# bmds-lab/Crackling

Hardware: AMD Instinct MI355X
Metric: guides/sec (whole node) + achieved HBM GB/s, 20bp/<=4mm ISSL scan (higher is better)
Workload: dtype u32

## Files before the change

crackling_amd/csrc/issl_bin.hip:

```cpp
#include <hip/hip_runtime.h>

#include <algorithm>
#include <type_traits>

#include "issl_kernels.hpp"

namespace issl {


__global__ __launch_bounds__(256) void k_pack_scan_stream(ImageView v, uint32_t *__restrict__ scan_out,
                                                          uint64_t *__restrict__ esig_out,
                                                          uint8_t *__restrict__ occ8_out,
                                                          uint32_t *__restrict__ error_flag, uint32_t *__restrict__ seen,
                                                          uint32_t tile_begin, uint32_t tile_end)
{
    for (uint32_t t = tile_begin + blockIdx.x; t < tile_end; t += gridDim.x) {
        uint32_t lo = 0, hi = v.n_buckets;
        while (hi - lo > 1) {
            const uint32_t mid = (lo + hi) >> 1;
            if (v.tile_first[mid] <= t) lo = mid; else hi = mid;
        }
        const uint32_t b = lo;
        const uint32_t slice = b >> v.slice_width;
        const uint64_t start = v.bucket_start[b];
// ... 71 lines not shown
    if (g < n) {
        const uint64_t sig = guides[g];
        const uint32_t low = (1u << slice_width) - 1u;
        for (uint32_t s = 0; s < n_slices; ++s) {
            const uint32_t key = static_cast<uint32_t>(sig >> (slice_width * s)) & low;
            atomicAdd(&hist[(s << slice_width) + key], 1u);
        }
    }
    const uint32_t stride = gridDim.x * 256;
    for (uint32_t k = g; k < n_slots; k += stride) { ws.gidx[k] = kNoGuide; ws.gword[k] = kPadGuideWord; }
    for (uint32_t k = g; k <= n; k += stride) ws.gcount[k] = 0;
    for (uint32_t k = g; k <= ws.cap_chunks; k += stride) ws.raw_used[k] = 0;
    if (g == 0) {
        Counters c{};
        c.raw_chunks = n_scan_waves;
        *ws.counters = c;
        ws.scan_span[2u * ws.span_slot] = ~0ull;
        ws.scan_span[2u * ws.span_slot + 1u] = 0ull;
    }
    __syncthreads();
    if (blockIdx.x * 256 < n)
        for (uint32_t b = threadIdx.x; b < n_buckets; b += 256)
            if (hist[b]) atomicAdd(&ws.ng[b], hist[b]);
}

template <bool COOP = false>
__device__ __forceinline__ RangeStart range_start_of(const ScanItem *__restrict__ items, uint32_t n_items, uint64_t total,
                                                     uint32_t n_ranges, uint32_t r)
{
    RangeStart out;
    out.item = n_items;
    out.tile = 0;
    out.goff = 0;
    out.pad = 0;
    if (r < n_ranges) {
        const uint64_t lo = total / n_ranges * r + (total % n_ranges) * r / n_ranges;
        uint32_t a = 0, z = n_items;
        if (COOP) {
            const uint32_t lane = threadIdx.x & 63u;
            while (z - a > 1) {
                const uint32_t step = (z - a + 63u) / 64u;
                const uint64_t pos = static_cast<uint64_t>(a) + static_cast<uint64_t>(lane + 1u) * step;
                const bool le = pos < z && items[pos].cost0 <= lo;
                const uint32_t k = static_cast<uint32_t>(__popcll(__ballot(le)));
                const uint64_t na = static_cast<uint64_t>(a) + static_cast<uint64_t>(k) * step, nz = na + step;
                a = static_cast<uint32_t>(na);
                if (nz < z) z = static_cast<uint32_t>(nz);
            }
        } else
        while (z - a > 1) {
            const uint32_t mid = (a + z) >> 1;
            if (items[mid].cost0 <= lo) a = mid; else z = mid;
        }
        const ScanItem it = items[a];
        const uint32_t len = it.g1 - it.g0;
        const uint32_t per_guide = it.shape >> 3;
        const uint64_t tile_cost = static_cast<uint64_t>(len) * per_guide + kTileFixedCost;
        const uint64_t rel = lo - it.cost0;
        uint64_t k = rel / tile_cost;
        const uint64_t rem = rel % tile_cost;
        uint32_t goff = 0;
        if (rem > kTileFixedCost) {
            goff = ((static_cast<uint32_t>(rem - kTileFixedCost) + per_guide - 1u) / per_guide + kGuideGroup - 1u) & ~(kGuideGroup - 1u);
            if (goff >= len) { goff = 0; ++k; }
        }
        if (k >= it.n_tiles) { out.item = a + 1; out.tile = 0; out.goff = 0; }
        else { out.item = a; out.tile = static_cast<uint32_t>(k); out.goff = goff; }
    }
    return out;
}

__device__ __forceinline__ uint32_t ranges_for(uint64_t units, uint32_t scan_blocks)
{
    const uint64_t want = units / 64u + 1u;
    const uint32_t floor_ = scan_blocks < 64u ? scan_blocks : 64u;
    return want >= scan_blocks ? scan_blocks : want < floor_ ? floor_ : static_cast<uint32_t>(want);
}

__global__ __launch_bounds__(256) void k_plan(ImageView v, uint32_t *__restrict__ ng, uint32_t *__restrict__ gfill,
                                              uint32_t *__restrict__ gstart, ScanItem *__restrict__ items,
                                              uint32_t cap_items, PlanInfo *__restrict__ plan, uint32_t item_guides,
                                              uint32_t scan_blocks, Counters *__restrict__ counters)
{
    short_kernel_priority();
    __shared__ uint64_t lds[256];
    const uint32_t nb = v.n_buckets;
    const uint32_t per = (nb + 255u) / 256u;
    const uint32_t b0 = threadIdx.x * per;
    const uint32_t b1 = (b0 + per < nb) ? b0 + per : nb;

    uint64_t slots = 0, n_it = 0, cost = 0, cand = 0, wtiles = 0;
    for (uint32_t b = b0; b < b1; ++b) {
        const uint32_t g = ng[b];
        const uint32_t nt = v.tile_first[b + 1] - v.tile_first[b];
        slots += (g + kGuideGroup - 1u) / kGuideGroup * kGuideGroup;
        if (g && nt) {
            const uint32_t k = (g + item_guides - 1u) / item_guides;
            n_it += k;
            cost += static_cast<uint64_t>(nt) * (static_cast<uint64_t>(g) * kGuideCost + static_cast<uint64_t>(k) * kTileFixedCost);
            cand += (v.bucket_start[b + 1] - v.bucket_start[b]) * g;
            wtiles += static_cast<uint64_t>(nt) * k;
        }
    }
    uint64_t tot_slots, tot_items, tot_cost, tot_cand, tot_tiles;
    uint64_t slot_at = block_exclusive_scan(slots, lds, &tot_slots);
    uint64_t item_at = block_exclusive_scan(n_it, lds, &tot_items);
    uint64_t cost_at = block_exclusive_scan(cost, lds, &tot_cost);
    (void)block_exclusive_scan(cand, lds, &tot_cand);
    uint64_t tile_at = block_exclusive_scan(wtiles, lds, &tot_tiles);

    const bool overflow = tot_items > cap_items;
    for (uint32_t b = b0; b < b1; ++b) {
        const uint32_t g = ng[b];
        const uint32_t nt = v.tile_first[b + 1] - v.tile_first[b];
        gstart[b] = static_cast<uint32_t>(slot_at);
        if (g && nt && !overflow) {
            const uint64_t blen = v.bucket_start[b + 1] - v.bucket_start[b];
            for (uint32_t done = 0; done < g; done += item_guides) {
                const uint32_t len = (g - done < item_guides) ? g - done : item_guides;
                ScanItem it;
                it.bucket = b;
                it.g0 = static_cast<uint32_t>(slot_at) + done;
                it.g1 = it.g0 + len;
                it.n_tiles = nt;
                it.cost0 = cost_at;
                it.tile0 = static_cast<uint32_t>(tile_at);
                it.last_cands = static_cast<uint32_t>(blen - static_cast<uint64_t>(nt - 1u) * kTileCands);
                it.group_abs = v.tile_first[b] * 64u;
                it.window = it.last_cands << 16;
                it.shape = 32; it.gmid = 0;
                items[item_at++] = it;
                cost_at += static_cast<uint64_t>(nt) * (len * kGuideCost + kTileFixedCost);
                tile_at += nt;
            }
        }
        slot_at += (g + kGuideGroup - 1u) / kGuideGroup * kGuideGroup;
        ng[b] = 0;
        gfill[b] = 0;
    }
    if (threadIdx.x == 255) {
        gstart[nb] = static_cast<uint32_t>(tot_slots);
        if (!overflow) {
            ScanItem end;
            end.bucket = 0; end.g0 = 0; end.g1 = 0; end.n_tiles = 0; end.cost0 = tot_cost;
            end.tile0 = static_cast<uint32_t>(tot_tiles); end.last_cands = 0; end.group_abs = 0; end.window = 0;
            end.shape = 32; end.gmid = 0;
            items[tot_items] = end;
        }
        plan->n_items = overflow ? 0u : static_cast<uint32_t>(tot_items);
        plan->total_cost = overflow ? 0ull : tot_cost;
        plan->candidates = tot_cand;
        plan->reference_candidates = tot_cand;
        plan->fine = 0;
        plan->tiles = tot_tiles;
        plan->n_ranges = (overflow || tot_tiles == 0) ? 0u : ranges_for(tot_tiles, scan_blocks);
        counters->raw_chunks = (plan->n_ranges ? plan->n_ranges : 1u) * 16u;
        plan->error = overflow ? 2u : 0u;
    }
}

__global__ __launch_bounds__(256) void k_guide_scatter(const uint64_t *__restrict__ guides, uint32_t n,
                                                       uint32_t slice_width, uint32_t n_slices, uint32_t sorted_layout,
                                                       uint32_t n_buckets, const uint32_t *__restrict__ gstart,
                                                       uint32_t *__restrict__ gfill, uint32_t *__restrict__ gword,
                                                       uint32_t *__restrict__ gidx, uint32_t *__restrict__ gbucket,
                                                       uint64_t *__restrict__ gsig,
                                                       uint32_t guide_blocks, const PlanInfo *__restrict__ plan,
                                                       const ScanItem *__restrict__ items,
                                                       RangeStart *__restrict__ starts)
{
    short_kernel_priority();
    if (blockIdx.x >= guide_blocks) {
        const uint32_t n_ranges = plan->n_ranges;
        const uint32_t r = (blockIdx.x - guide_blocks) * 256 + threadIdx.x;
        if (r <= n_ranges && n_ranges != 0) starts[r] = range_start_of(items, plan->n_items, plan->total_cost, n_ranges, r);
        return;
    }
    __shared__ uint32_t hist[kMaxBuckets];
    __shared__ uint32_t base[kMaxBuckets];
    for (uint32_t b = threadIdx.x; b < n_buckets; b += 256) hist[b] = 0;
    __syncthreads();
    const uint32_t g = blockIdx.x * 256 + threadIdx.x;
    const uint32_t low = (1u << slice_width) - 1u;
    uint64_t sig = 0;
    uint32_t rank[kMaxSlices];
    if (g < n) {
        sig = guides[g];
#pragma unroll
        for (uint32_t s = 0; s < kMaxSlices; ++s) {
            if (s < n_slices) {
                const uint32_t key = static_cast<uint32_t>(sig >> (slice_width * s)) & low;
                rank[s] = atomicAdd(&hist[(s << slice_width) + key], 1u);
            }
        }
    }
    __syncthreads();
    for (uint32_t b = threadIdx.x; b < n_buckets; b += 256)
        base[b] = hist[b] ? atomicAdd(&gfill[b], hist[b]) : 0u;
    __syncthreads();
    if (g < n) {
#pragma unroll
        for (uint32_t s = 0; s < kMaxSlices; ++s) {
            if (s < n_slices) {
                const uint32_t key = static_cast<uint32_t>(sig >> (slice_width * s)) & low;
                const uint32_t b = (s << slice_width) + key;
                const uint32_t slot = gstart[b] + base[b] + rank[s];
                gword[slot] = image_word(sig, s, slice_width, sorted_layout != 0u);
                gidx[slot] = g;
                gbucket[slot] = b;
                gsig[slot] = sig;
            }
        }
    }
}


struct GroupUnits {
    uint32_t s0a, n_full, rest, shape, units;
};
__device__ __forceinline__ GroupUnits group_units(uint32_t s0, uint32_t s1, uint32_t tail_shapes)
{
    GroupUnits u;
    u.s0a = s0 & ~31u;
    const uint32_t span = s1 - u.s0a;
    u.n_full = span / kTileCands;
    u.rest = span - u.n_full * kTileCands;
    u.shape = (!tail_shapes || u.rest > 1024u) ? 32u : u.rest > 512u ? 16u : 8u;
    u.units = u.n_full + (u.rest ? 1u : 0u);
    return u;
}
__device__ __forceinline__ uint64_t group_cost(const GroupUnits &u, uint32_t len)
{
    return static_cast<uint64_t>(u.n_full) * (static_cast<uint64_t>(len) * kGuideCost + kTileFixedCost) +
           (u.rest ? static_cast<uint64_t>(len) * (u.shape >> 3) + kTileFixedCost : 0ull);
}

__device__ __forceinline__ uint32_t fine_way(uint32_t gj, uint32_t way)
{
    if (way == 0) return gj;
    if (way < kFineWays) {
        const uint32_t q = (way - 1u) / 3u, d = (way - 1u) % 3u + 1u;
        return gj ^ (d << (2u * q));
    }
    const uint32_t w2 = way - kFineWays, pair = w2 / 9u, d1 = (w2 % 9u) / 3u + 1u, d2 = w2 % 3u + 1u;
    const uint32_t a = pair < 3u ? 0u : pair < 5u ? 1u : 2u;
    const uint32_t b = pair < 3u ? pair + 1u : pair < 5u ? pair - 1u : 3u;
    return gj ^ (d1 << (2u * a)) ^ (d2 << (2u * b));
}
__device__ __forceinline__ uint32_t fine_class(uint32_t way) { return way == 0u ? 0u : way < kFineWays ? 1u : 2u; }

__host__ __device__ __forceinline__ uint32_t fine_word(uint32_t word, uint32_t slice, uint32_t slice_width = 8u)
{
    const uint32_t lo = word & 0xFFFFu, hi = word >> 16;
    uint32_t lo12 = 0, hi12 = 0;
    for (uint32_t j = 0; j < 3u; ++j) {
        const uint32_t q = fine_order(slice, j, slice_width);
        lo12 |= ((lo >> (4u * q)) & 0xFu) << (4u * j);
        hi12 |= ((hi >> (4u * q)) & 0xFu) << (4u * j);
    }
    return lo12 | (hi12 << 12);
}

template <uint32_t WAYS>
__global__ __launch_bounds__(256) void k_fine_count(ImageView v, const uint64_t *__restrict__ gsig,
                                                    const uint32_t *__restrict__ gstart, const uint32_t *__restrict__ gfill,
                                                    uint32_t *__restrict__ fcount,
                                                    uint32_t *__restrict__ fcount0,
                                                    FineSum *__restrict__ fsum, uint32_t item_guides, uint32_t tail_shapes)
{
    constexpr uint32_t ways = WAYS;
    short_kernel_priority();
    __shared__ uint32_t cnt[256], cnt0[256];
    __shared__ uint64_t lds[256];
    const uint32_t b = blockIdx.x, slice = b >> v.slice_width;
    cnt[threadIdx.x] = 0;
    cnt0[threadIdx.x] = 0;
    __syncthreads();
    const uint32_t g0 = gstart[b], n = gfill[b];
    for (uint32_t i = threadIdx.x; i < n; i += 256) {
        const uint32_t gj = succ_byte(gsig[g0 + i], slice, v.slice_width);
        atomicAdd(&cnt0[gj], 1u);
#pragma unroll
        for (uint32_t way = 0; way < ways; ++way) atomicAdd(&cnt[fine_way(gj, way)], 1u);
    }
    __syncthreads();
    const uint32_t w = threadIdx.x, c = cnt[w];
    const uint32_t *ss = v.sub_start + static_cast<uint64_t>(b) * 257u;
    const uint32_t s0 = ss[w], s1 = ss[w + 1];
    fcount[static_cast<uint64_t>(b) * 256u + w] = (s1 > s0) ? c : 0u;
    fcount0[static_cast<uint64_t>(b) * 256u + w] = (s1 > s0) ? cnt0[w] : 0u;
    uint64_t cost = 0, cand = 0, slots = 0, items = 0, units = 0;
    if (c && s1 > s0) {
        const GroupUnits gu = group_units(s0, s1, tail_shapes);
        const uint32_t kk = (c + item_guides - 1u) / item_guides;
        slots = (c + kGuideGroup - 1u) / kGuideGroup * kGuideGroup;
        units = static_cast<uint64_t>(gu.units) * kk;
        items = units;
        for (uint32_t done = 0; done < c; done += item_guides) cost += group_cost(gu, c - done < item_guides ? c - done : item_guides);
        cand = static_cast<uint64_t>(s1 - s0) * c;
    }
    uint64_t t_cost, t_cand, t_slots, t_items, t_units, t_places;
    (void)block_exclusive_scan(cost, lds, &t_cost);
    (void)block_exclusive_scan(cand, lds, &t_cand);
    (void)block_exclusive_scan(slots, lds, &t_slots);
    (void)block_exclusive_scan(items, lds, &t_items);
    (void)block_exclusive_scan(units, lds, &t_units);
    (void)block_exclusive_scan((c && s1 > s0) ? c : 0u, lds, &t_places);
    if (threadIdx.x == 0) {
        FineSum f;
        f.cost = t_cost; f.cand = t_cand; f.slots = static_cast<uint32_t>(t_slots); f.items = static_cast<uint32_t>(t_items);
        f.units = static_cast<uint32_t>(t_units); f.places = static_cast<uint32_t>(t_places);
        fsum[b] = f;
    }
}

__global__ __launch_bounds__(256) void k_fine_plan(FineSum *__restrict__ fsum, uint32_t nb, ScanItem *__restrict__ fitems,
                                                   uint32_t cap_items, uint32_t cap_slots, PlanInfo *__restrict__ plan,
                                                   uint32_t scan_blocks, uint32_t prune_mode, uint32_t always,
                                                   uint32_t *__restrict__ sticky, Counters *__restrict__ counters)
{
    short_kernel_priority();
    __shared__ uint64_t lds[256];
    const uint32_t per = (nb + 255u) / 256u;
    const uint32_t b0 = threadIdx.x * per, b1 = (b0 + per < nb) ? b0 + per : nb;
    uint64_t cost = 0, cand = 0, slots = 0, items = 0, units = 0, places = 0;
    for (uint32_t b = b0; b < b1; ++b) {
        cost += fsum[b].cost; cand += fsum[b].cand; slots += fsum[b].slots; items += fsum[b].items; units += fsum[b].units;
        places += fsum[b].places;
    }
    uint64_t t_cost, t_cand, t_slots, t_items, t_units, t_places;
    (void)block_exclusive_scan(places, lds, &t_places);
    uint64_t cost_at = block_exclusive_scan(cost, lds, &t_cost);
    (void)block_exclusive_scan(cand, lds, &t_cand);
    uint64_t slot_at = block_exclusive_scan(slots, lds, &t_slots);
    uint64_t item_at = block_exclusive_scan(items, lds, &t_items);
    uint64_t unit_at = block_exclusive_scan(units, lds, &t_units);
    for (uint32_t b = b0; b < b1; ++b) {
        const FineSum f = fsum[b];
        FineSum at;
        at.cost = cost_at; at.cand = 0; at.slots = static_cast<uint32_t>(slot_at); at.items = static_cast<uint32_t>(item_at);
        at.units = static_cast<uint32_t>(unit_at); at.places = 0;
        fsum[b] = at;
        cost_at += f.cost; slot_at += f.slots; item_at += f.items; unit_at += f.units;
    }
    if (threadIdx.x == 255) {
        const uint64_t fetch_cost = static_cast<uint64_t>(kFetchPairs) * kGuideCost;
        const uint64_t full_fetch = plan->tiles, full_pairs = plan->total_cost - kTileFixedCost * full_fetch;
        const uint64_t fine_pairs = t_cost - kTileFixedCost * t_units;
        const uint64_t est_full = full_pairs > fetch_cost * full_fetch ? full_pairs : fetch_cost * full_fetch;
        const uint64_t est_fine = (fine_pairs > fetch_cost * t_units ? fine_pairs : fetch_cost * t_units) + t_places * kGuideCost;
        const bool fits = t_items <= cap_items && t_slots <= cap_slots;
        if (t_items > cap_items)
            atomicMax(&sticky[3], static_cast<uint32_t>(t_items < 0xFFFFFFFFull ? t_items : 0xFFFFFFFFull));
        if (fits && plan->error == 0 && (always || est_fine < est_full)) {
            ScanItem end;
            end.bucket = 0; end.g0 = 0; end.g1 = 0; end.n_tiles = 0; end.cost0 = t_cost;
            end.tile0 = static_cast<uint32_t>(t_units); end.last_cands = 0; end.group_abs = 0; end.window = 0;
            end.shape = 32; end.gmid = 0;
            fitems[t_items] = end;
            plan->n_items = static_cast<uint32_t>(t_items);
            plan->total_cost = t_cost;
            plan->candidates = t_cand;
            plan->tiles = t_units;
            plan->n_ranges = t_units == 0 ? 0u : ranges_for(t_units, scan_blocks);
            counters->raw_chunks = (plan->n_ranges ? plan->n_ranges : 1u) * 16u;
            plan->fine = prune_mode;
            plan->fine_slots = static_cast<uint32_t>(t_slots);
        }
    }
}


struct alignas(16) FineGroup {
    uint64_t cost0, chunk_cost;
    uint32_t s0, s1, n_full, units;
    uint32_t shape, c, slot, slot0;
};
template <uint32_t THREADS> struct FineItemLds {
    uint64_t scan[THREADS / 64u];
    uint32_t item0_of[257];
    FineGroup group[256];
    alignas(16) ScanItem stage[THREADS];
};
template <uint32_t THREADS> struct FineGuideLds {
    uint64_t scan[THREADS / 64u];
    uint32_t slot_of[256], slot0_of[256], cursor[256], cursor0[256], has_cands[256];
};
static_assert(sizeof(FineItemLds<512u>) <= 40u * 1024u, "four workgroups of k_fine_scatter per CU");

template <uint32_t THREADS>
__device__ __forceinline__ void fine_scatter_items(const ImageView &v, uint32_t b, const uint32_t *__restrict__ fcount,
                                                   const uint32_t *__restrict__ fcount0, const FineSum *__restrict__ fbase,
                                                   ScanItem *__restrict__ fitems, uint32_t item_guides, uint32_t tail_shapes,
                                                   FineItemLds<THREADS> &l)
{
    const uint32_t w = threadIdx.x;
    const FineSum base = fbase[b];
    const uint64_t blen = v.bucket_start[b + 1] - v.bucket_start[b];
    const uint32_t tile_first_b = v.tile_first[b];
    uint32_t c = 0, c1 = 0, s0 = 0, s1 = 0;
    if (w < 256u) {
        c = fcount[static_cast<uint64_t>(b) * 256u + w];
        c1 = c - fcount0[static_cast<uint64_t>(b) * 256u + w];
        const uint32_t *ss = v.sub_start + static_cast<uint64_t>(b) * 257u;
        s0 = ss[w];
        s1 = ss[w + 1];
    }
    uint64_t cost = 0, slots = 0, items = 0;
    GroupUnits gu{};
    if (c) {
        gu = group_units(s0, s1, tail_shapes);
        const uint32_t kk = (c + item_guides - 1u) / item_guides;
        slots = (c + kGuideGroup - 1u) / kGuideGroup * kGuideGroup;
        items = static_cast<uint64_t>(gu.units) * kk;
        for (uint32_t done = 0; done < c; done += item_guides) cost += group_cost(gu, c - done < item_guides ? c - done : item_guides);
    }
    const uint64_t cost_at = base.cost + block_exclusive_scan(cost, l.scan, nullptr);
    const uint32_t slot_at = base.slots + static_cast<uint32_t>(block_exclusive_scan(slots, l.scan, nullptr));
    const uint32_t item_at = static_cast<uint32_t>(block_exclusive_scan(items, l.scan, nullptr));
    if (w < 256u) {
        l.item0_of[w] = item_at;
        if (w == 255u) l.item0_of[256] = item_at + static_cast<uint32_t>(items);
        FineGroup g;
        g.cost0 = cost_at; g.chunk_cost = group_cost(gu, item_guides);
        g.s0 = s0; g.s1 = s1; g.n_full = gu.n_full; g.units = gu.units;
        g.shape = gu.shape; g.c = c; g.slot = slot_at; g.slot0 = slot_at + c1;
        l.group[w] = g;
    }
    __syncthreads();
    const uint32_t total = l.item0_of[256];
    for (uint32_t i0 = 0; i0 < total; i0 += THREADS) {
        const uint32_t i = i0 + w;
        if (i < total) {
            uint32_t lo = 0, hi = 256;
            while (hi - lo > 1u) {
                const uint32_t mid = (lo + hi) >> 1;
                if (l.item0_of[mid] <= i) lo = mid; else hi = mid;
            }
            const uint32_t gw = lo;
            const FineGroup g = l.group[gw];
            const uint32_t s0a = g.s0 & ~31u;
            const uint32_t j = i - l.item0_of[gw];
            const uint32_t chunk = j / g.units, t = j - chunk * g.units;
            const uint32_t done = chunk * item_guides;
            const uint32_t len = (g.c - done < item_guides) ? g.c - done : item_guides;
            const bool full = t < g.n_full;
            const uint32_t shape = full ? 32u : g.shape, cap = 64u * shape;
            const uint32_t wstart = s0a + t * kTileCands;
            const uint64_t after = blen - wstart;
            ScanItem it;
            it.bucket = (b << 8) | gw;
            it.g0 = g.slot + done;
            it.g1 = it.g0 + len;
            it.n_tiles = 1;
            it.cost0 = g.cost0 + static_cast<uint64_t>(chunk) * g.chunk_cost +
                       static_cast<uint64_t>(t) * (static_cast<uint64_t>(len) * kGuideCost + kTileFixedCost);
            it.tile0 = base.items + i;
            it.last_cands = after < cap ? static_cast<uint32_t>(after) : cap;
            it.group_abs = tile_first_b * 64u + (wstart >> 5);
            it.window = (t == 0 ? g.s0 - s0a : 0u) | ((g.s1 - wstart < cap ? g.s1 - wstart : cap) << 16);
            it.shape = shape; it.gmid = g.slot0;
            l.stage[w] = it;
        }
        __syncthreads();
        const uint32_t n_here = total - i0 < THREADS ? total - i0 : THREADS;
        const uint4 *src4 = reinterpret_cast<const uint4 *>(l.stage);
        uint4 *dst4 = reinterpret_cast<uint4 *>(fitems + base.items + i0);
        for (uint32_t q = w; q < n_here * 3u; q += THREADS) dst4[q] = src4[q];
        __syncthreads();
    }
}

template <uint32_t WAYS, uint32_t THREADS>
__device__ __forceinline__ void fine_scatter_guides(const ImageView &v, uint32_t b, const uint32_t *__restrict__ gstart,
                                                    const uint32_t *__restrict__ gfill, const uint32_t *__restrict__ gword,
                                                    const uint32_t *__restrict__ gidx, const uint64_t *__restrict__ gsig,
                                                    const uint32_t *__restrict__ fcount, const uint32_t *__restrict__ fcount0,
                                                    const FineSum *__restrict__ fbase, FineSlot *__restrict__ fword,
                                                    FineGuideLds<THREADS> &l)
{
    constexpr uint32_t ways = WAYS;
    const uint32_t w = threadIdx.x, slice = b >> v.slice_width;
    const uint32_t g0 = gstart[b], n = gfill[b];
    const uint32_t base_slots = fbase[b].slots;
    uint32_t c = 0, c1 = 0;
    if (w < 256u) {
        c = fcount[static_cast<uint64_t>(b) * 256u + w];
        c1 = c - fcount0[static_cast<uint64_t>(b) * 256u + w];
    }
    uint32_t i = w, guide = 0, word = 0;
    uint64_t sig = 0;
    if (i < n) { guide = gidx[g0 + i]; word = gword[g0 + i]; sig = gsig[g0 + i]; }
    const uint32_t slots = (c + kGuideGroup - 1u) / kGuideGroup * kGuideGroup;
    const uint32_t slot_at = base_slots + static_cast<uint32_t>(block_exclusive_scan(slots, l.scan, nullptr));
    if (w < 256u) {
        l.slot_of[w] = slot_at;
        l.slot0_of[w] = slot_at + c1;
        l.cursor[w] = 0;
        l.cursor0[w] = 0;
        l.has_cands[w] = c ? 1u : 0u;
        for (uint32_t k2 = c; k2 < slots; ++k2) fword[slot_at + k2] = FineSlot{kPadGuideWord, kPadSlotId};
    }
    __syncthreads();
    while (i < n) {
        const uint32_t gj = succ_byte(sig, slice, v.slice_width);
        const uint32_t word12 = fine_word(word, slice, v.slice_width), id = slot_id(slice, guide);
#pragma unroll
        for (uint32_t way = 0; way < ways; ++way) {
            const uint32_t ww = fine_way(gj, way);
            if (!l.has_cands[ww]) continue;
            const uint32_t slot = way ? l.slot_of[ww] + atomicAdd(&l.cursor[ww], 1u) : l.slot0_of[ww] + atomicAdd(&l.cursor0[ww], 1u);
            fword[slot] = FineSlot{word12 | (fine_class(way) << 24), id};
        }
        i += THREADS;
        if (i < n) { guide = gidx[g0 + i]; word = gword[g0 + i]; sig = gsig[g0 + i]; }
    }
}

template <uint32_t WAYS, uint32_t THREADS>
__global__ __launch_bounds__(THREADS) void k_fine_scatter(ImageView v, const uint32_t *__restrict__ gstart,
// ... 231 lines not shown
```

crackling_amd/csrc/issl_capi.cpp:

```cpp
#include <algorithm>
#include <cerrno>
#include <cstdio>
#include <cstdlib>
#include <cstring>

#include "issl_index.hpp"

using namespace issl;

namespace issl {

int build_from_device_sites(const uint64_t *d_sigs, const uint32_t *d_occ, size_t n_sites, size_t n_lines, size_t seq_len,
                            size_t slice_width, int device, const char *options, issl_index **out)
{
    int rc = select_device(device, "the ISSL scorer");
    if (rc) return rc;
    const uint32_t n_slices = static_cast<uint32_t>((seq_len * 2) / slice_width);
    std::vector<uint64_t> sizes(size_t(n_slices) << slice_width);
    rc = launch_bucket_sizes(d_sigs, n_sites, static_cast<uint32_t>(slice_width), n_slices, sizes.data());
    if (rc) return rc;
    std::unique_ptr<HostIndex> h(new HostIndex());
    rc = h->init_from_bucket_sizes(sizes.data(), n_sites, n_lines, seq_len, slice_width);
    if (rc) return rc;
    return build_on_device(std::move(h), d_sigs, d_occ, true, device, options, out);
// ... 1 lines not shown

}

extern "C" {

const char *issl_last_error(void) { return get_error(); }
int issl_abi_version(void) { return ISSL_ABI_VERSION; }

int issl_index_open(const char *path, issl_index **out)
{
    if (!path || !out) return issl::fail(ISSL_E_ARG, "null argument");
    return abi_call([&] { return new_index([&](HostIndex &h) { return h.open_file(path); }, out); });
}

int issl_index_from_memory(const void *image, size_t len, issl_index **out)
{
    if (!image || !out) return issl::fail(ISSL_E_ARG, "null argument");
    return abi_call([&] { return new_index([&](HostIndex &h) { return h.from_memory(image, len); }, out); });
}

int issl_index_build_from_text(const char *text, size_t n_lines, size_t seq_len, size_t slice_width,
                               issl_index **out)
{
    if (!text || !out) return issl::fail(ISSL_E_ARG, "null argument");
    return abi_call([&] { return new_index([&](HostIndex &h) { return h.build_from_text(text, n_lines, seq_len, slice_width); }, out); });
}

int issl_index_build_from_sites(const uint64_t *sigs, const uint32_t *occ, size_t n_sites, size_t n_lines,
                                size_t seq_len, size_t slice_width, issl_index **out)
{
    if (!sigs || !occ || !out) return issl::fail(ISSL_E_ARG, "null argument");
    return abi_call([&] { return new_index([&](HostIndex &h) { return h.build_from_sites(sigs, occ, n_sites, n_lines, seq_len, slice_width); }, out); });
}

int issl_index_write(const issl_index *idx, const char *path)
{
    if (!idx || !path) return issl::fail(ISSL_E_ARG, "null argument");
    return abi_call([&]() -> int {
        if (!idx->host) { set_error("index was attached from a device image and has no host arrays"); return ISSL_E_STATE; }
        if (idx->host->has_arrays()) return idx->host->write_file(path);
        if (!idx->d_image) { set_error("index has neither host arrays nor a device image"); return ISSL_E_STATE; }
        HIP_TRY(hipSetDevice(idx->device));
        FILE *fp = std::fopen(path, "wb");
        if (!fp) {
            set_error(std::string("cannot write index file '") + path + "': " + std::strerror(errno));
            return ISSL_E_IO;
        }
        bool ok = idx->host->write_leading_sections(fp) == ISSL_OK;
        const uint8_t *base = static_cast<const uint8_t *>(idx->d_image);
        const uint8_t *cold = static_cast<const uint8_t *>(idx->h_cold);
        std::vector<uint8_t> stage;
        bool sig_words = false;
        auto stream_dev = [&](const uint8_t *src, uint64_t bytes) {
            stage.resize(size_t(64) << 20);
            for (uint64_t at = 0; ok && at < bytes; at += stage.size()) {
                const size_t len = static_cast<size_t>(std::min<uint64_t>(stage.size(), bytes - at));
                ok = hipMemcpy(stage.data(), src + at, len, hipMemcpyDeviceToHost) == hipSuccess;
                if (ok && sig_words) {
                    uint64_t *w = reinterpret_cast<uint64_t *>(stage.data());
                    for (size_t i = 0; i < len / 8; ++i) w[i] &= kSigMask;
                }
                ok = ok && std::fwrite(stage.data(), 1, len, fp) == len;
            }
        };
        auto stream_out = [&](uint64_t off, uint64_t bytes, bool in_host) {
            if (in_host) {
                ok = ok && std::fwrite(cold + off, 1, bytes, fp) == bytes;
                return;
            }
            stream_dev(base + off, bytes);
        };
        sig_words = idx->hdr.off_sub_start != 0;
        stream_out(idx->hdr.off_sites, 8 * idx->geo.n_sites, (idx->hdr.cold_on_host & 2u) != 0);
        sig_words = false;
        ok = ok && std::fwrite(idx->host->sizes, 8, idx->geo.n_buckets(), fp) == idx->geo.n_buckets();
        if (idx->hdr.lists_absent) {
            std::unique_ptr<void, hipError_t (*)(void *)> list_mem(nullptr, hipFree);
            const uint64_t n = idx->geo.n_sites;
            void *p = nullptr;
            if (hipMalloc(&p, std::max<uint64_t>(8 * n, 8)) != hipSuccess) {
                (void)hipGetLastError();
                std::fclose(fp);
                set_error("no device memory to rebuild the slice lists of this image (8 B per site)");
                return ISSL_E_DEVICE;
            }
            list_mem.reset(p);
            for (uint64_t sl = 0; ok && sl < idx->geo.n_slices; ++sl) {
                int brc = launch_build_entries(reinterpret_cast<const uint64_t *>(base + idx->hdr.off_sites),
                                               reinterpret_cast<const uint32_t *>(base + idx->hdr.off_site_occ), n, static_cast<uint32_t>(sl),
                                               static_cast<uint32_t>(sl + 1), static_cast<uint32_t>(idx->geo.slice_width),
                                               static_cast<uint64_t *>(list_mem.get()));
                if (brc) { std::fclose(fp); return brc; }
                stream_dev(static_cast<const uint8_t *>(list_mem.get()), 8 * n);
            }
        } else {
            stream_out(idx->hdr.off_entries, 8 * idx->geo.n_sites * idx->geo.n_slices, (idx->hdr.cold_on_host & 1u) != 0);
        }
        ok = (std::fclose(fp) == 0) && ok;
        if (!ok) {
            set_error(std::string("could not write '") + path + "' from the device image");
            return ISSL_E_IO;
        }
        return ISSL_OK;
    });
}

int issl_index_header(const issl_index *idx, issl_header *out)
{
    if (!idx || !out) return issl::fail(ISSL_E_ARG, "null argument");
    out->n_sites = idx->geo.n_sites;
    out->seq_len = idx->geo.seq_len;
    out->n_lines = idx->geo.n_lines;
    out->slice_width = idx->geo.slice_width;
    out->n_slices = idx->geo.n_slices;
    out->n_scores = idx->geo.n_scores;
    return ISSL_OK;
}

int issl_index_bucket_sizes(const issl_index *idx, uint64_t *out, size_t n)
{
    if (!idx || !out) return issl::fail(ISSL_E_ARG, "null argument");
    if (n < idx->bucket_sizes.size()) { set_error("bucket size buffer too small"); return ISSL_E_ARG; }
    std::copy(idx->bucket_sizes.begin(), idx->bucket_sizes.end(), out);
    return ISSL_OK;
}

int issl_index_close(issl_index *idx)
{
    if (!idx) return ISSL_OK;
    release_device(idx);
    delete idx;
    return ISSL_OK;
}

int issl_index_device_bytes(const issl_index *idx, size_t *out)
{
    if (!idx || !out) return issl::fail(ISSL_E_ARG, "null argument");
    if (idx->d_image) { *out = idx->hdr.total_bytes; return ISSL_OK; }
    if (!idx->host) { set_error("index has neither host arrays nor a device image"); return ISSL_E_STATE; }
    return abi_call([&] { return planned_image_bytes(idx, out); });
}

static bool workspace_option(const issl_index *idx, const char *key, long long *value)
{
    const Workspace &w = idx->lane.ws;
    const bool used = w.cap_guides != 0;
    const struct { const char *key; long long v; } keys[] = {
        {"ws_cap_guides", static_cast<long long>(w.cap_guides)},
        {"ws_slot_width", used ? static_cast<long long>(w.slot_width) : 0},
        {"ws_fine_ways", static_cast<long long>(w.fine_ways)},
        {"ws_cap_chunks", static_cast<long long>(w.cap_chunks)},
        {"ws_cap_fitems", static_cast<long long>(w.cap_fitems)},
        {"ws_lean", idx->lane.lean ? 1 : 0},
    };
    for (const auto &k : keys)
        if (std::strcmp(k.key, key) == 0) {
            if (value) *value = k.v;
            return true;
        }
    return false;
}

int issl_index_set_option(issl_index *idx, const char *key, const char *value)
{
    if (!idx || !key || !value) return issl::fail(ISSL_E_ARG, "null argument");
    if (workspace_option(idx, key, nullptr)) {
        return abi_call([&]() -> int {
            set_error(std::string("read-only option: ") + key);
            return ISSL_E_ARG;
        });
    }
    if (idx->n_pending) { set_error("issl_index_set_option: batches are in flight, call issl_score_finish first"); return ISSL_E_STATE; }
    return abi_call([&]() -> int {
        Tuning t = idx->tuning;
        if (!t.set(key, value)) {
            set_error(std::string("unknown option or value out of range: ") + key + "=" + value);
            return ISSL_E_ARG;
        }
        if (idx->d_image && t.scan_blocks != idx->tuning.scan_blocks) {
            HIP_TRY(hipSetDevice(idx->device));
            for (Lane *lp : {&idx->lane, &idx->lane2})
                if (lp->ws.cap_chunks && lp->ws.cap_chunks < size_t(scan_waves(t)) * 2) {
                    int rc = ensure_raw_capacity(lp->ws, size_t(scan_waves(t)) * 4);
                    if (rc) return rc;
                }
        }
        idx->tuning = t;
        return ISSL_OK;
    });
}

int issl_index_get_option(const issl_index *idx, const char *key, long long *value)
{
    if (!idx || !key || !value) return issl::fail(ISSL_E_ARG, "null argument");
    if (idx->tuning.get(key, value) || image_option(idx->d_image ? &idx->hdr : nullptr, key, value) || workspace_option(idx, key, value)) return ISSL_OK;
    return abi_call([&]() -> int {
        set_error(std::string("unknown option: ") + key);
        return ISSL_E_ARG;
    });
}

int issl_index_build_on_device_opt(const uint64_t *sigs, const uint32_t *occ, size_t n_sites, size_t n_lines,
                                   size_t seq_len, size_t slice_width, int device, const char *options, issl_index **out)
{
    if (!sigs || !occ || !out) return issl::fail(ISSL_E_ARG, "null argument");
    return abi_call([&]() -> int {
        std::unique_ptr<HostIndex> h(new HostIndex());
        int rc = h->init_without_arrays(sigs, n_sites, n_lines, seq_len, slice_width);
        if (rc) return rc;
        return build_on_device(std::move(h), sigs, occ, false, device, options, out);
    });
}


int issl_index_build_from_device_sites(const uint64_t *d_sigs, const uint32_t *d_occ, size_t n_sites, size_t n_lines,
                                       size_t seq_len, size_t slice_width, int device, const char *options, issl_index **out)
{
    if (!d_sigs || !d_occ || !out) return issl::fail(ISSL_E_ARG, "null argument");
    if (seq_len == 0 || seq_len > 32 || slice_width < 2 || slice_width > 8 || (seq_len * 2) / slice_width == 0 ||
        (seq_len * 2) / slice_width > kMaxSlices) {
        set_error("bad sequence length or slice width");
        return ISSL_E_ARG;
    }
    return abi_call([&] { return build_from_device_sites(d_sigs, d_occ, n_sites, n_lines, seq_len, slice_width, device, options, out); });
}

int issl_index_build_on_device(const uint64_t *sigs, const uint32_t *occ, size_t n_sites, size_t n_lines,
                               size_t seq_len, size_t slice_width, int device, issl_index **out)
{
    return issl_index_build_on_device_opt(sigs, occ, n_sites, n_lines, seq_len, slice_width, device, nullptr, out);
}

int issl_device_memory(int device, size_t *free_bytes, size_t *total_bytes)
{
    if (!free_bytes || !total_bytes) return issl::fail(ISSL_E_ARG, "null argument");
    int rc = select_device(device, "the ISSL scorer");
    if (rc) return rc;
    HIP_TRY(hipMemGetInfo(free_bytes, total_bytes));
    return ISSL_OK;
}

int issl_index_upload(issl_index *idx, int device)
{
    if (!idx) return issl::fail(ISSL_E_ARG, "null argument");
    return abi_call([&] { return upload_common(idx, device, nullptr, 0); });
}

int issl_index_upload_into(issl_index *idx, int device, void *dev_buf, size_t bytes)
{
    if (!dev_buf) { set_error("null device buffer"); return ISSL_E_ARG; }
    if (!idx) return issl::fail(ISSL_E_ARG, "null argument");
    return abi_call([&] { return upload_common(idx, device, dev_buf, bytes); });
}


int issl_index_attach_image(int device, void *dev_buf, size_t bytes, issl_index **out)
{
    return abi_call([&] { return attach_common(device, dev_buf, bytes, nullptr, 0, out); });
}

int issl_index_attach_image_cold(int device, void *dev_buf, size_t bytes, void *cold_host, size_t cold_bytes,
                                 issl_index **out)
{
    return abi_call([&] { return attach_common(device, dev_buf, bytes, cold_host, cold_bytes, out); });
}

int issl_index_cold(const issl_index *idx, void **host_ptr, size_t *bytes)
{
    if (!idx || !host_ptr || !bytes) return issl::fail(ISSL_E_ARG, "null argument");
    if (!idx->d_image) { set_error("index has no device image"); return ISSL_E_STATE; }
    *host_ptr = idx->hdr.cold_on_host ? idx->h_cold : nullptr;
    *bytes = idx->hdr.cold_on_host ? idx->hdr.cold_bytes : 0;
    return ISSL_OK;
}

int issl_index_image(const issl_index *idx, void **dev_ptr, size_t *bytes)
{
    if (!idx || !dev_ptr || !bytes) return issl::fail(ISSL_E_ARG, "null argument");
    if (!idx->d_image) { set_error("index has no device image"); return ISSL_E_STATE; }
    *dev_ptr = idx->d_image;
    *bytes = idx->hdr.total_bytes;
    return ISSL_OK;
}

int issl_index_copy_image_to(const issl_index *idx, void *dev_dst, size_t bytes)
{
    if (!idx || !dev_dst) return issl::fail(ISSL_E_ARG, "null argument");
    if (!idx->d_image) { set_error("index has no device image"); return ISSL_E_STATE; }
    if (bytes < idx->hdr.total_bytes || (reinterpret_cast<uintptr_t>(dev_dst) & 255u)) {
        set_error("destination too small or not 256-byte aligned");
        return ISSL_E_ARG;
    }
    HIP_TRY(hipSetDevice(idx->device));
    HIP_TRY(hipMemcpy(dev_dst, idx->d_image, idx->hdr.total_bytes, hipMemcpyDeviceToDevice));
    return ISSL_OK;
}


void issl_free(void *p) { std::free(p); }

int issl_score_device(issl_index *idx, const uint64_t *d_guides, size_t n, int max_dist, double threshold,
                      int method, double *d_mit, double *d_cfd, void *stream)
{
    if (!idx || (n && (!d_guides || !d_mit || !d_cfd))) return issl::fail(ISSL_E_ARG, "null argument");
    return abi_call([&]() -> int {
        return score_core(idx, d_guides, n, max_dist, threshold, method, d_mit, d_cfd, static_cast<hipStream_t>(stream), false);
// ... 109 lines not shown
```

crackling_amd/csrc/issl_device.hpp:

```cpp
#pragma once
#include <cstddef>
#include <cstdint>
#include <string>

#include "issl_host.hpp"

namespace issl {

constexpr uint64_t kImageMagic = 0x314C535349444D41ull;
constexpr uint32_t kImageVersion = 9;
constexpr uint32_t kTileCands = 2048;
constexpr uint32_t kHeaderBytes = 4096;

struct ImageHeader {
    uint64_t magic;
    uint32_t version;
    uint32_t kind;
    uint64_t n_sites, seq_len, n_lines, slice_width, n_slices, n_scores_file;
    uint64_t n_buckets;
    uint64_t n_scores_unique;
    uint64_t n_tiles;
    uint64_t tile_cands;
    uint64_t total_bytes;
    uint64_t off_bucket_start, off_tile_first, off_score_mask, off_score_val, off_sites, off_entries,
        off_scan;
    uint64_t off_mit_dense;
    uint64_t off_esig;
    uint64_t cold_on_host;
    uint64_t cold_bytes;
    uint64_t off_occ8;
    uint64_t off_sub_start;
    uint64_t off_srec;
    uint64_t off_sid;
    uint64_t off_site_occ;
    uint64_t lists_absent;
};
static_assert(sizeof(ImageHeader) <= kHeaderBytes, "header must fit its block");

constexpr uint32_t kOccSaturated = 0xFFFFFFu;
constexpr uint64_t kSigMask = (1ull << 40) - 1ull;

#if defined(__HIPCC__)
__host__ __device__
#endif
inline uint32_t succ_byte(uint64_t sig, uint32_t s, uint32_t slice_width)
{
    const uint32_t sh = (slice_width * (s + 1u)) % 40u;
    const uint64_t x = sig & kSigMask;
    return static_cast<uint32_t>(sh ? (x >> sh) | (x << (40u - sh)) : x) & 0xFFu;
}
struct alignas(16) StreamRec {
    uint64_t sig;
    uint32_t id;
    uint32_t pos;
};

struct ImageView {
    const uint64_t *bucket_start;
    const uint32_t *tile_first;
    const uint64_t *score_mask;
    const double *score_val;
    const double *mit_dense;
    const uint64_t *sites;
    const uint64_t *entries;
    const uint64_t *esig;
    const uint8_t *occ8;
    const uint32_t *sub_start;
    const StreamRec *srec;
    const uint32_t *sid;
    const uint32_t *site_occ;
    const uint32_t *scan;
    uint64_t n_sites;
    uint32_t n_buckets;
    uint32_t n_scores;
    uint32_t slice_width;
    uint32_t n_slices;
    uint32_t n_tiles;
};

struct LayoutSpec {
    bool inline_sigs = false;
    uint32_t cold = 0;
    uint32_t sorted = 0;
    bool no_lists = false;
};
void layout_image(ImageHeader &h, const Geometry &g, uint64_t n_scores_unique, uint64_t n_tiles, bool dense_mit,
                  const LayoutSpec &spec);
ImageView make_view(const ImageHeader &h, void *base, void *cold);

struct Tuning {
    uint32_t scan_blocks;
    uint32_t scan_threads;
    int upload_threads;
    size_t upload_chunk_kib, upload_ring_min_kib;
    uint32_t item_guides;
    bool scan_generic;
    int scan_events;
    bool stage_timing;
    bool upload_timing;
    size_t raw_chunks;
    int inline_sigs;
    int sorted_layout;
    int compact;
    int prune;
    int tail_shapes;
    int hit_slots;
    size_t fine_items;
    size_t expect_guides;
    int small_bin;
    int lean_tail;
    int lanes;
    int host_cold;
    int keep_lists;
    std::string stamps_path;
    static Tuning from_env();
    bool set(const char *key, const char *value);
    bool get(const char *key, long long *value) const;
    int set_list(const char *options);
};
bool image_option(const ImageHeader *h, const char *key, long long *value);

int launch_build_entries(const uint64_t *d_sites, const uint32_t *d_occ, uint64_t n_sites, uint32_t slice_begin,
                         uint32_t slice_end, uint32_t slice_width, uint64_t *d_entries);
int launch_bucket_sizes(const uint64_t *d_sites, uint64_t n_sites, uint32_t slice_width, uint32_t n_slices, uint64_t *h_sizes);

constexpr int kSortNeedsListOrder = -1000;
constexpr int kSortNoRoom = -1001;
struct SortTemp {
    uint64_t *keys = nullptr, *tmp = nullptr;
    uint32_t *hist = nullptr;
    bool keys_borrowed = false;
    int alloc(uint64_t n_sites, void *borrowed_keys = nullptr);
    void release();
    ~SortTemp() { release(); }
};
int launch_sort_slice(SortTemp &t, const uint64_t *d_sites, const uint64_t *d_list, const uint64_t *d_bucket_start,
                      const uint32_t *d_tile_first, uint64_t n_sites, uint32_t n_slices, uint32_t n_buckets, uint32_t slice_width, uint32_t slice, uint32_t *d_sub_start,
                      StreamRec *d_srec, uint32_t *d_sid, uint32_t *d_site_occ, uint32_t *d_flag);
int finish_sort(uint32_t *d_flag);
void launch_tag_sites(uint64_t *d_sites, const uint32_t *d_site_occ, uint64_t n_sites);

constexpr uint32_t kGuideGroup = 8;
constexpr uint32_t kItemGuides = 512;
constexpr uint32_t kGuideCost = 4;
constexpr uint32_t kTileFixedCost = 8 * kGuideCost;
constexpr uint32_t kNoGuide = 0xFFFFFFFFu;
constexpr uint32_t kPadGuideWord = 0xFFFFFFFFu;
constexpr uint32_t kScanGridBlocks = 256u * 4u;
constexpr uint32_t kScanMaxBlocks = 8192u;
constexpr uint32_t kScanWaves = kScanMaxBlocks * 16u;
constexpr uint32_t kMaxRanges = kScanMaxBlocks;
constexpr uint32_t kStampsScanWords = 4u * kScanWaves, kStampsPerReplay = 16u * 4096u;
constexpr uint32_t kStampsMid = kStampsScanWords, kStampsBig256 = kStampsMid + kStampsPerReplay, kStampsBig1024 = kStampsBig256 + kStampsPerReplay;
constexpr uint32_t kStampsWords = kStampsBig1024 + kStampsPerReplay;
constexpr uint32_t kSpanRing = 64;
constexpr uint32_t kChunkRecs = 128;
constexpr uint64_t kDeadKey = ~0ull;
constexpr uint32_t kKeySliceShift = 32, kKeyGuideShift = 37, kKeySliceMask = 31, kMaxSlices = 20;

struct ScanItem {
    uint32_t bucket;
    uint32_t g0, g1;
    uint32_t n_tiles;
    uint64_t cost0;
    uint32_t tile0;
    uint32_t last_cands;
    uint32_t group_abs;
    uint32_t window;
    uint32_t shape;
    uint32_t gmid;
};
static_assert(sizeof(ScanItem) == 48, "scan items are fetched with scalar loads");

struct RangeStart {
    uint32_t item;
    uint32_t tile;
    uint32_t goff;
    uint32_t pad;
};

struct PlanInfo {
    uint32_t n_items;
    uint32_t error;
    uint32_t n_ranges;
    uint32_t fine;
    uint64_t total_cost;
    uint64_t candidates;
    uint64_t reference_candidates;
    uint64_t tiles;
    uint32_t fine_slots;
    uint32_t pad;
};

struct Counters {
    uint32_t next_range;
    uint32_t n_big;
    uint32_t n_big2;
    uint32_t n_big3;
    uint32_t raw_chunks;
    uint32_t raw_overflow;
    uint32_t overflowed;
    uint32_t replay_next[3];
};

struct FineSum {
    uint64_t cost, cand;
    uint32_t slots, items, units;
    uint32_t places;
};

constexpr uint32_t kSlotHits = 512;
constexpr uint32_t kSlotHitsWide = 2048;
struct alignas(32) SlotRec {
    double mit, cfd;
    uint64_t key, pad;
};
#if defined(__HIPCC__)
__host__ __device__
#endif
inline uint64_t slot_pad(uint32_t occ, uint32_t dist) { return static_cast<uint64_t>(occ) | (static_cast<uint64_t>(dist) << 32); }
constexpr uint32_t kFineWays = 13;
constexpr uint32_t kFineWays2 = 67;
constexpr uint32_t kFetchPairs = 8;
constexpr uint32_t kPruneMaxGuides = 1u << 20;
constexpr uint32_t kPruneMaxGuides2 = 1u << 18;
inline uint32_t prune_max_guides(uint32_t prune_mode, uint32_t n_slices)
{
    const uint32_t m = prune_mode == 3 ? kPruneMaxGuides2 : kPruneMaxGuides;
    return n_slices > 10 ? m >> 2 : n_slices > 5 ? m >> 1 : m;
}

constexpr uint32_t kSlotIdBits = 27, kSlotGuideBits = 22;
constexpr uint32_t kPadSlotId = (1u << kSlotIdBits) - 1u;
#if defined(__HIPCC__)
__host__ __device__
#endif
inline uint32_t slot_id(uint32_t slice, uint32_t guide) { return (slice << kSlotGuideBits) | guide; }
#if defined(__HIPCC__)
__host__ __device__
#endif
inline void slot_id_unpack(uint32_t id, uint32_t &slice, uint32_t &guide)
{
    slice = id >> kSlotGuideBits;
    guide = id & ((1u << kSlotGuideBits) - 1u);
}
static_assert(kPruneMaxGuides <= (1u << kSlotGuideBits), "a pruned launch's guides fit the id's guide field");
static_assert(kMaxSlices <= (1u << (kSlotIdBits - kSlotGuideBits)), "an index's slices fit the id's slice field");
static_assert(((kMaxSlices - 1u) << kSlotGuideBits | (kPruneMaxGuides - 1u)) < kPadSlotId, "no slot's id is the padding id");
static_assert(kSlotIdBits + 26u + 11u == 64u, "raw record: slot id, tile, offset in tile");

struct alignas(8) FineSlot {
    uint32_t word;
    uint32_t id;
};

struct Workspace {
    uint32_t *ng = nullptr;
    uint32_t *gfill = nullptr;
    uint32_t *gstart = nullptr;
    uint32_t *gword = nullptr;
    uint32_t *gidx = nullptr;
    uint32_t *gbucket = nullptr;
    uint64_t *gsig = nullptr;
    ScanItem *items = nullptr;
    FineSlot *fword = nullptr;
    ScanItem *fitems = nullptr;
    uint32_t *fcount = nullptr;
    uint32_t *fcount0 = nullptr;
    FineSum *fsum = nullptr;
    size_t cap_fslots = 0, cap_fitems = 0;
    uint32_t fine_ways = 0;
    PlanInfo *plan = nullptr;
    RangeStart *range_start = nullptr;
    uint64_t *raw = nullptr;
    uint32_t *raw_used = nullptr;
    size_t cap_chunks = 0;
    Counters *counters = nullptr;
    unsigned long long *scan_span = nullptr;
    uint32_t span_slot = 0;
    uint64_t *scan_count = nullptr;
    unsigned long long *stamps = nullptr;
    uint32_t *sticky = nullptr;
    uint64_t *sorted = nullptr;
    uint32_t *gcount = nullptr;
    uint32_t *goff = nullptr;
    uint32_t *gcur_big = nullptr;
    uint32_t *gcur_big2 = nullptr;
    double *terms = nullptr;
    double *pay = nullptr;
    uint32_t *rank = nullptr;
    SlotRec *slots = nullptr;
    uint32_t slot_hits = 0;
    uint32_t slot_width = kSlotHits;
    uint32_t lean_tail = 0;
    size_t cap_slot_guides = 0;
    uint32_t *blocksum = nullptr;
    uint64_t *d_guides = nullptr;
    void *h_stage = nullptr;
    size_t h_stage_bytes = 0;
    double *d_mit = nullptr, *d_cfd = nullptr;
    uint32_t *d_kept = nullptr;
    issl_hit *d_hitrec = nullptr;
    size_t cap_hitrec = 0;
    size_t cap_guides = 0;
    size_t cap_hits = 0;
    size_t cap_items = 0;
    size_t cap_gslots = 0;
    uint32_t n_buckets = 0;
};

struct ScoreParams {
    int max_dist;
    int method;
    double maximum_sum;
};

void launch_pack_scan_stream(const ImageView &v, uint32_t *scan_out, uint64_t *esig_out, uint8_t *occ8_out,
                             uint32_t *error_flag, uint32_t *seen, void *stream);
void launch_pack_scan_range(const ImageView &v, uint32_t *scan_out, uint64_t *esig_out, uint8_t *occ8_out,
                            uint32_t *error_flag, uint32_t *seen, uint32_t tile_begin, uint32_t tile_end, void *stream);
inline uint32_t fine_ways_of(uint32_t prune_mode) { return prune_mode == 1 ? 1u : prune_mode == 3 ? kFineWays2 : kFineWays; }
uint32_t prune_mode_for(const ImageView &v, const Tuning &tn, uint32_t n_guides, int max_dist);
void launch_bin_guides(const ImageView &v, const Workspace &ws, const Tuning &tn, const uint64_t *d_guides, uint32_t n,
                       uint32_t prune_mode, void *stream);
void launch_scan(const ImageView &v, const Workspace &ws, const Tuning &tn, const uint64_t *d_guides, uint32_t n,
                 int max_dist, uint32_t prune_mode, void *stream);
void launch_verify(const ImageView &v, const Workspace &ws, const uint64_t *d_guides, uint32_t n, const ScoreParams &p, void *stream);
void launch_group_hits(const Workspace &ws, uint32_t n, void *stream);
void launch_replay(const ImageView &v, const Workspace &ws, const uint64_t *d_guides, uint32_t n,
                   const ScoreParams &p, double *d_mit, double *d_cfd, uint32_t *d_kept, issl_hit *d_hitrec,
                   void *stream);
void launch_profile(const ImageView &v, const Workspace &ws, const uint64_t *d_guides, uint32_t n, issl_profile *d_out,
                    void *stream);
void launch_report_offsets(const Workspace &ws, uint32_t n, uint64_t base, uint64_t *d_offsets, void *stream);
void launch_report_emit(const ImageView &v, const Workspace &ws, const uint64_t *d_guides, uint32_t n_records,
                        uint32_t guide_base, issl_offtarget *d_out, void *stream);

}
```

crackling_amd/csrc/issl_group.hip:

```cpp
#include <hip/hip_runtime.h>

#include "issl_kernels.hpp"

namespace issl {


__global__ __launch_bounds__(256) void k_prefix_block_sums(const uint32_t *__restrict__ in, uint32_t n,
                                                           uint32_t *__restrict__ sums, uint32_t slot_hits)
{
    short_kernel_priority();
    __shared__ uint64_t lds[256];
    const uint32_t base = blockIdx.x * kScanChunk + threadIdx.x * 8u;
    uint64_t s = 0;
    for (uint32_t i = 0; i < 8; ++i)
        if (base + i < n) s += grouped_hits(in[base + i], slot_hits);
    uint64_t total;
    (void)block_exclusive_scan(s, lds, &total);
    if (threadIdx.x == 0) sums[blockIdx.x] = static_cast<uint32_t>(total);
}

__global__ __launch_bounds__(256) void k_prefix_of_sums(uint32_t *__restrict__ sums, uint32_t n_blocks)
{
    short_kernel_priority();
    __shared__ uint64_t lds[256];
    uint64_t carry = 0;
    for (uint32_t base = 0; base < n_blocks; base += 256) {
        const uint32_t i = base + threadIdx.x;
        const uint64_t val = i < n_blocks ? sums[i] : 0;
        uint64_t total;
        const uint64_t ex = block_exclusive_scan(val, lds, &total);
        if (i < n_blocks) sums[i] = static_cast<uint32_t>(carry + ex);
        carry += total;
    }
}

__global__ __launch_bounds__(256) void k_prefix_apply(const uint32_t *__restrict__ in, uint32_t n,
                                                      const uint32_t *__restrict__ sums, uint32_t *__restrict__ out,
                                                      uint32_t *__restrict__ big, Counters *__restrict__ counters,
                                                      uint32_t slot_hits)
{
    short_kernel_priority();
    __shared__ uint64_t lds[256];
    const uint32_t base = blockIdx.x * kScanChunk + threadIdx.x * 8u;
    uint32_t val[8];
    uint64_t s = 0;
    uint32_t nb = 0;
    for (uint32_t i = 0; i < 8; ++i) {
        const uint32_t c = (base + i < n) ? in[base + i] : 0u;
        nb += c > kReplayLds;
        val[i] = grouped_hits(c, slot_hits);
        s += val[i];
    }
    if (nb != 0u) {
        uint32_t at = atomicAdd(&counters->n_big, nb);
        for (uint32_t i = 0; i < 8; ++i)
            if (base + i < n && in[base + i] > kReplayLds) big[at++] = base + i;
    }
    uint64_t run = block_exclusive_scan(s, lds, nullptr) + sums[blockIdx.x];
    for (uint32_t i = 0; i < 8; ++i) {
        if (base + i < n) out[base + i] = static_cast<uint32_t>(run);
        run += val[i];
    }
}

__global__ __launch_bounds__(1024) void k_prefix_single(const uint32_t *__restrict__ in, uint32_t n,
                                                        uint32_t *__restrict__ out, uint32_t *__restrict__ big,
                                                        Counters *__restrict__ counters, uint32_t slot_hits)
{
    short_kernel_priority();
    if (slot_hits >= kReplayLds && counters->overflowed == 0u) return;
    __shared__ uint32_t wave_sum[16], wave_big[16];
    const uint32_t lane = threadIdx.x & 63u, wave = threadIdx.x >> 6;
    const uint32_t per = ((n + 1023u) / 1024u + 3u) & ~3u;
    const uint32_t i0 = threadIdx.x * per;
    uint32_t s = 0, b = 0;
    for (uint32_t k = 0; k < per; k += 4) {
        const uint32_t i = i0 + k;
        uint4 q = make_uint4(0, 0, 0, 0);
        if (i + 3 < n) q = *reinterpret_cast<const uint4 *>(in + i);
        else { if (i < n) q.x = in[i]; if (i + 1 < n) q.y = in[i + 1]; if (i + 2 < n) q.z = in[i + 2]; }
        s += grouped_hits(q.x, slot_hits) + grouped_hits(q.y, slot_hits) + grouped_hits(q.z, slot_hits) + grouped_hits(q.w, slot_hits);
        b += (q.x > kReplayLds) + (q.y > kReplayLds) + (q.z > kReplayLds) + (q.w > kReplayLds);
    }
    uint32_t x = s, xb = b;
    for (uint32_t d = 1; d < 64; d <<= 1) {
        const uint32_t y = __shfl_up(x, d, 64), yb = __shfl_up(xb, d, 64);
        if (lane >= d) { x += y; xb += yb; }
    }
    if (lane == 63) { wave_sum[wave] = x; wave_big[wave] = xb; }
    __syncthreads();
    uint32_t run = x - s, brun = xb - b;
    for (uint32_t wv = 0; wv < wave; ++wv) { run += wave_sum[wv]; brun += wave_big[wv]; }
    if (threadIdx.x == 1023u) counters->n_big = brun + b;
    for (uint32_t k = 0; k < per; k += 4) {
        const uint32_t i = i0 + k;
        if (i >= n) break;
        uint4 q = make_uint4(0, 0, 0, 0);
        if (i + 3 < n) q = *reinterpret_cast<const uint4 *>(in + i);
        else { q.x = in[i]; if (i + 1 < n) q.y = in[i + 1]; if (i + 2 < n) q.z = in[i + 2]; }
        const uint32_t ex = grouped_hits(q.x, slot_hits), ey = grouped_hits(q.y, slot_hits), ez = grouped_hits(q.z, slot_hits),
                       ew = grouped_hits(q.w, slot_hits);
        const uint4 o = make_uint4(run, run + ex, run + ex + ey, run + ex + ey + ez);
        if (i + 3 < n) *reinterpret_cast<uint4 *>(out + i) = o;
        else { out[i] = o.x; if (i + 1 < n) out[i + 1] = o.y; if (i + 2 < n) out[i + 2] = o.z; }
        run += ex + ey + ez + ew;
        if (q.x > kReplayLds) big[brun++] = i;
        if (q.y > kReplayLds) big[brun++] = i + 1;
        if (q.z > kReplayLds) big[brun++] = i + 2;
        if (q.w > kReplayLds) big[brun++] = i + 3;
    }
}

__global__ __launch_bounds__(kChunkRecs) void k_group_scatter(const uint64_t *__restrict__ raw,
                                                              const uint32_t *__restrict__ raw_used,
                                                              const Counters *__restrict__ counters, uint32_t cap_chunks,
                                                              const uint32_t *__restrict__ gcount,
                                                              const uint32_t *__restrict__ goff,
                                                              const uint32_t *__restrict__ rank,
                                                              const double2 *__restrict__ pay,
                                                              uint64_t *__restrict__ sorted, double2 *__restrict__ terms,
                                                              uint32_t slot_hits)
{
    short_kernel_priority();
    if (slot_hits >= kReplayLds && counters->n_big == 0u) return;
    uint32_t n_chunks = counters->raw_chunks;
    if (n_chunks > cap_chunks) n_chunks = cap_chunks;
    for (uint32_t chunk = blockIdx.x; chunk < n_chunks; chunk += gridDim.x) {
        const uint64_t *recs = raw + static_cast<uint64_t>(chunk) * kChunkRecs;
        const uint32_t t = threadIdx.x + 1u;
        const uint64_t slot = static_cast<uint64_t>(chunk) * (kChunkRecs - 1u) + (threadIdx.x < kChunkRecs - 1u ? threadIdx.x : kChunkRecs - 2u);
        const uint64_t key = recs[t < kChunkRecs ? t : 0u];
        const uint32_t my_rank = rank[slot];
        const double2 my_pay = pay[slot];
        const uint32_t used = raw_used[chunk];
        if (t >= used || t >= kChunkRecs || key == kDeadKey) continue;
        const uint32_t guide = static_cast<uint32_t>(key >> kKeyGuideShift);
        const uint32_t to = goff[guide] + my_rank;
        sorted[to] = key;
        if (gcount[guide] <= kMidHits) terms[to] = my_pay;
    }
}

void launch_group_hits(const Workspace &ws, uint32_t n, void *stream_)
{
    if (ws.lean_tail) return;
    hipStream_t stream = static_cast<hipStream_t>(stream_);
    const uint32_t m = n + 1;
    if (m <= (1u << 18)) {
        hipLaunchKernelGGL(k_prefix_single, dim3(1), dim3(1024), 0, stream, ws.gcount, m, ws.goff, ws.gcur_big,
                           ws.counters, ws.slot_hits);
    } else {
        const uint32_t blocks = (m + kScanChunk - 1) / kScanChunk;
        hipLaunchKernelGGL(k_prefix_block_sums, dim3(blocks), dim3(256), 0, stream, ws.gcount, m, ws.blocksum, ws.slot_hits);
        hipLaunchKernelGGL(k_prefix_of_sums, dim3(1), dim3(256), 0, stream, ws.blocksum, blocks);
        hipLaunchKernelGGL(k_prefix_apply, dim3(blocks), dim3(256), 0, stream, ws.gcount, m, ws.blocksum, ws.goff,
                           ws.gcur_big, ws.counters, ws.slot_hits);
    }
    hipLaunchKernelGGL(k_group_scatter, dim3(kTailGrid), dim3(kChunkRecs), 0, stream, ws.raw, ws.raw_used, ws.counters,
                       static_cast<uint32_t>(ws.cap_chunks), ws.gcount, ws.goff, ws.rank, reinterpret_cast<const double2 *>(ws.pay),
                       ws.sorted, reinterpret_cast<double2 *>(ws.terms), ws.slot_hits);
}

}
```

crackling_amd/csrc/issl_index.hpp:

```cpp
#pragma once
#include <hip/hip_runtime_api.h>

#include <functional>
#include <memory>
#include <string>
#include <vector>

#include "issl_device.hpp"
#include "issl_hiputil.hpp"

namespace issl {

constexpr uint32_t kRing = 64;
constexpr size_t kMaxBatch = size_t(1) << 24;
constexpr size_t kSlotBytesMax = size_t(8) << 30;

struct Lane {
    Workspace ws;
    hipEvent_t ev[6] = {};
    hipEvent_t done = nullptr;
    hipStream_t stream = nullptr;
    hipStream_t tail_stream = nullptr;
    bool ready = false;
    uint32_t last_n = 0;
    uint32_t pending = 0;
    bool staged = true;
    bool done_recorded = false;
    hipStream_t last_tail = nullptr;
    int last_max_dist = 0;
    uint32_t last_prune = 0;
    bool lean = false;
};

}

struct issl_index {
    uint64_t worst_per_guide = 0;
    std::unique_ptr<issl::HostIndex> host;
    issl::Geometry geo;
    std::vector<uint64_t> bucket_sizes;
    issl::Tuning tuning = issl::Tuning::from_env();
    int device = -1;
    void *d_image = nullptr;
    bool owns_image = false;
    void *h_cold = nullptr;
    void *d_cold = nullptr;
    bool owns_cold = false;
    issl::ImageHeader hdr{};
    issl::ImageView view{};
    issl::Lane lane;
    issl::Lane lane2;
    uint32_t n_async = 0;
    issl::Lane *last_lane = nullptr;
    hipEvent_t ring[2 * issl::kRing] = {};
    uint32_t n_ring = 0;
    bool have_events = false;
    issl_stats stats{};
    uint32_t n_pending = 0;
    hipEvent_t prev_scan_end = nullptr;
    hipEvent_t prev_batch_end = nullptr;
    bool list_order_only = false;
    size_t proven_guides = 0, proven_chunks = 0;
    int proven_dist = -1;
};

namespace issl {

int new_index_from_host(std::unique_ptr<HostIndex> h, issl_index **out);
template <class Init> int new_index(Init &&init, issl_index **out)
{
    std::unique_ptr<HostIndex> h(new HostIndex());
    if (int rc = init(*h)) return rc;
    return new_index_from_host(std::move(h), out);
}
int build_on_device(std::unique_ptr<HostIndex> h, const uint64_t *sigs, const uint32_t *occ, bool on_device, int device,
                    const char *options, issl_index **out);
int build_from_device_sites(const uint64_t *d_sigs, const uint32_t *d_occ, size_t n_sites, size_t n_lines, size_t seq_len,
                            size_t slice_width, int device, const char *options, issl_index **out);
int upload_common(issl_index *idx, int device, void *buf, size_t bytes);
int attach_common(int device, void *dev_buf, size_t bytes, void *cold_host, size_t cold_bytes, issl_index **out);
int planned_image_bytes(const issl_index *idx, size_t *out);
void release_device(issl_index *ix);

int supported_geometry(const Geometry &g);
void release_lanes(issl_index *ix);
inline uint32_t scan_waves(const Tuning &tn) { return tn.scan_blocks * 16u; }
int ensure_workspace(issl_index *ix, size_t n, Lane &lane, uint32_t fine_ways = kFineWays);
int ensure_raw_capacity(Workspace &w, size_t chunks);
int finish_batches(issl_index *ix, hipStream_t stream);
int score_core(issl_index *ix, const uint64_t *d_guides, size_t n, int max_dist, double threshold, int method,
               double *d_mit, double *d_cfd, hipStream_t stream, bool dump, issl_profile *d_profile = nullptr);
int score_async(issl_index *idx, const uint64_t *d_guides, size_t n, int max_dist, double threshold, int method,
                double *d_mit, double *d_cfd, hipStream_t stream);
int wait_batches(issl_index *idx, hipStream_t stream);
int score_host(issl_index *idx, const uint64_t *guides, size_t n, int max_dist, double threshold, int method,
               double *mit, double *cfd);
int dump_hits(issl_index *idx, const uint64_t *guides, size_t n, int max_dist, double threshold, int method,
              issl_hit *hits, size_t cap, size_t *n_hits);
int profile_host(issl_index *idx, const uint64_t *guides, size_t n, int max_dist, issl_profile *out);
int profile_device(issl_index *idx, const uint64_t *d_guides, size_t n, int max_dist, issl_profile *d_out, hipStream_t stream);
int offtargets_host(issl_index *idx, const uint64_t *guides, size_t n, int max_dist, uint64_t *offsets, issl_offtarget *recs,
                    size_t cap, size_t *n_total);
int offtargets_device(issl_index *idx, const uint64_t *d_guides, size_t n, int max_dist, uint64_t *d_offsets,
                      issl_offtarget *d_recs, size_t cap, size_t *n_total, hipStream_t stream);

struct CallBuffer : DevBuf {
    size_t bytes = 0;
    int reserve(size_t want)
    {
        if (want <= bytes) return ISSL_OK;
        release();
        bytes = 0;
        HIP_TRY(hipMalloc(&p, want));
        bytes = want;
        return ISSL_OK;
    }
};

struct RecordBatch {
    const uint64_t *d_guides = nullptr;
    size_t n_guides = 0, guide_base = 0;
    const issl_offtarget *d_recs = nullptr;
    uint32_t n_recs = 0;
    const uint32_t *d_rec_off = nullptr;
};
int records_device(issl_index *idx, const uint64_t *d_guides, size_t n, int max_dist, CallBuffer &buf, RecordBatch &out, hipStream_t stream);
int records_host(issl_index *idx, const uint64_t *guides, size_t n, int max_dist, CallBuffer &buf,
                 const std::function<int(const RecordBatch &)> &use);

}
```

crackling_amd/csrc/issl_kernels.hip:

```cpp
#include <hip/hip_runtime.h>

#include <type_traits>

#include "issl_kernels.hpp"

namespace issl {


struct alignas(4 * kGuideGroup) GuideGroup {
    uint32_t w[kGuideGroup];
};


__device__ __forceinline__ uint64_t raw_record(uint32_t gslot, uint32_t tile, uint32_t offset)
{
    return (static_cast<uint64_t>(gslot) << 37) | (static_cast<uint64_t>(tile) << 11) | offset;
}

struct RawWriter {
    uint64_t *chunk;
    uint32_t fill;
    uint32_t left;
    uint32_t reserve;
};

__device__ __forceinline__ void raw_retire(const RawWriter &w, uint32_t lane, const uint64_t *raw, uint32_t *raw_used)
{
    if (lane == 0) raw_used[(w.chunk - raw) / kChunkRecs] = w.fill;
}

__device__ __forceinline__ void raw_acquire(RawWriter &w, uint64_t *raw, uint32_t max_chunks, Counters *counters,
                                            uint32_t lane)
{
    w.fill = 1;
    if (w.left != 0u) {
        w.chunk += kChunkRecs;
        w.left -= 1u;
        return;
    }
    const uint32_t take = w.reserve;
    uint32_t idx = 0;
    if (lane == 0) idx = atomicAdd(&counters->raw_chunks, take);
    idx = __builtin_amdgcn_readfirstlane(idx);
    if (idx + take > max_chunks) {
        idx = max_chunks;
        if (lane == 0) counters->raw_overflow = 1u;
        w.chunk = raw + static_cast<uint64_t>(idx) * kChunkRecs;
        return;
    }
    w.chunk = raw + static_cast<uint64_t>(idx) * kChunkRecs;
    w.left = take - 1u;
    if (take < 16u) w.reserve = take * 2u;
}

__device__ __forceinline__ void full_add(uint32_t a, uint32_t b, uint32_t c, uint32_t &sum, uint32_t &carry)
{
    sum = __builtin_amdgcn_bitop3_b32(a, b, c, 0x96);
    carry = __builtin_amdgcn_bitop3_b32(a, b, c, 0xE8);
}
__device__ __forceinline__ void half_add(uint32_t a, uint32_t b, uint32_t &sum, uint32_t &carry)
{
    sum = a ^ b;
    carry = a & b;
}

template <int THR>
__device__ __forceinline__ uint32_t count_near(const uint32_t (&m)[16], uint32_t thr, uint32_t keep);

template <int THR>
__device__ __forceinline__ uint32_t near_plane(const uint32_t (&c)[kPlanes], uint32_t gw, uint32_t thr, uint32_t keep)
{
    uint32_t m[16];
#pragma unroll
    for (int p = 0; p < 16; ++p) {
        const uint32_t g0 = 0u - ((gw >> p) & 1u);
        const uint32_t g1 = 0u - ((gw >> (16 + p)) & 1u);
        m[p] = (c[p] ^ g0) | (c[16 + p] ^ g1);
    }
    return count_near<THR>(m, thr, keep);
}

template <int THR>
__device__ __forceinline__ uint32_t near_plane_masks(const uint32_t (&c)[kPlanes], const uint4 *gm ,
                                                     uint32_t thr, uint32_t keep)
{
    uint32_t m[16];
#pragma unroll
    for (int q = 0; q < 4; ++q) {
        const uint4 lo = gm[q], hi = gm[4 + q];
        asm volatile("" ::: "memory");
        m[4 * q + 0] = (c[4 * q + 0] ^ lo.x) | (c[16 + 4 * q + 0] ^ hi.x);
        m[4 * q + 1] = (c[4 * q + 1] ^ lo.y) | (c[16 + 4 * q + 1] ^ hi.y);
        m[4 * q + 2] = (c[4 * q + 2] ^ lo.z) | (c[16 + 4 * q + 2] ^ hi.z);
        m[4 * q + 3] = (c[4 * q + 3] ^ lo.w) | (c[16 + 4 * q + 3] ^ hi.w);
    }
    return count_near<THR>(m, thr, keep);
}

constexpr uint32_t kPassIds = 28;
typedef uint32_t SlotPair __attribute__((ext_vector_type(4)));
__device__ __forceinline__ void short_unit_masks(const FineSlot *__restrict__ slots, uint32_t g0, bool wide,
                                                 uint32_t lane, uint4 *lds_masks)
{
    const uint32_t i = lane >> 3, q = lane & 7u;
    uint32_t m[4];
    if (wide) {
        const SlotPair gw = *reinterpret_cast<const SlotPair *>(slots + g0 + 2u * i);
        const uint32_t a = gw.x >> (4u * q), b = gw.z >> (4u * q);
#pragma unroll
        for (uint32_t r = 0; r < 4; ++r)
            m[r] = ((0u - ((a >> r) & 1u)) & 0xFFFFu) | ((0u - ((b >> r) & 1u)) << 16);
        if (q == 7u) { m[0] = gw.y; m[1] = gw.w; }
    } else {
        const SlotPair *src = reinterpret_cast<const SlotPair *>(slots + g0 + 4u * i);
        const SlotPair ga = src[0], gb = src[1];
        const uint32_t t[4] = {ga.x >> (4u * q), ga.z >> (4u * q), gb.x >> (4u * q), gb.z >> (4u * q)};
#pragma unroll
        for (uint32_t r = 0; r < 4; ++r) {
            const uint32_t bits = ((t[0] >> r) & 1u) | (((t[1] >> r) & 1u) << 8) | (((t[2] >> r) & 1u) << 16) | (((t[3] >> r) & 1u) << 24);
            m[r] = bits * 255u;
        }
        if (q == 7u) { m[0] = ga.y; m[1] = ga.w; m[2] = gb.y; m[3] = gb.w; }
    }
    lds_masks[i * 8u + q] = make_uint4(m[0], m[1], m[2], m[3]);
}

template <int THR>
__device__ __forceinline__ uint32_t count_near(const uint32_t (&m)[16], uint32_t thr, uint32_t keep)
{
    uint32_t s0, s1, s2, s3, s4, t, u, n0, n1, n2;
    uint32_t k2[8], k4[4], k8a, k8b;
    full_add(m[0], m[1], m[2], s0, k2[0]);
    full_add(m[3], m[4], m[5], s1, k2[1]);
    full_add(m[6], m[7], m[8], s2, k2[2]);
    full_add(m[9], m[10], m[11], s3, k2[3]);
    full_add(m[12], m[13], m[14], s4, k2[4]);
    full_add(s0, s1, s2, t, k2[5]);
    full_add(s3, s4, m[15], u, k2[6]);
    half_add(t, u, n0, k2[7]);
    uint32_t a2, b2, c2;
    full_add(k2[0], k2[1], k2[2], a2, k4[0]);
    full_add(k2[3], k2[4], k2[5], b2, k4[1]);
    full_add(k2[6], k2[7], a2, c2, k4[2]);
    half_add(b2, c2, n1, k4[3]);
    if (THR >= 0 && THR <= 4) {
        const uint32_t o = __builtin_amdgcn_bitop3_b32(k4[0], k4[1], k4[2], 0xFE);
        if (THR == 0) return __builtin_amdgcn_bitop3_b32(o, __builtin_amdgcn_bitop3_b32(k4[3], n1, n0, 0xFE), keep, 0x02);
        if (THR == 1) return __builtin_amdgcn_bitop3_b32(o, k4[3], n1, 0x01) & keep;
        if (THR == 2) return __builtin_amdgcn_bitop3_b32(o, __builtin_amdgcn_bitop3_b32(k4[3], n1, n0, 0xF8), keep, 0x02);
        if (THR == 3) return __builtin_amdgcn_bitop3_b32(o, k4[3], keep, 0x02);
        const uint32_t p = __builtin_amdgcn_bitop3_b32(k4[0], k4[1], k4[2], 0xE8);
        const uint32_t z = __builtin_amdgcn_bitop3_b32(o, k4[3], n1 | n0, 0xE8);
        return __builtin_amdgcn_bitop3_b32(p, z, keep, 0x02);
    }
    uint32_t a4;
    full_add(k4[0], k4[1], k4[2], a4, k8a);
    half_add(a4, k4[3], n2, k8b);
    const uint32_t n[5] = {n0, n1, n2, k8a ^ k8b, k8a & k8b};
    uint32_t gt = 0u, eq = ~0u;
#pragma unroll
    for (int b = 4; b >= 0; --b) {
        if ((thr >> b) & 1u) {
            eq &= n[b];
        } else {
            gt |= eq & n[b];
            eq &= ~n[b];
        }
    }
    return keep & ~gt;
}

struct PrevSlice {
    uint32_t a, b, c;
};
template <int B, bool EXTRA>
__device__ __forceinline__ uint32_t count_near12(const uint32_t (&m)[12], uint32_t f, uint32_t thr, uint32_t keep, PrevSlice &prev)
{
    uint32_t s0, s1, s2, s3, t, n0, a2, b2, k2[6], k40, k41;
    full_add(m[0], m[1], m[2], s0, k2[0]);
    prev.a = s0; prev.b = k2[0]; prev.c = m[3];
    full_add(m[3], m[4], m[5], s1, k2[1]);
    full_add(m[6], m[7], m[8], s2, k2[2]);
    full_add(m[9], m[10], m[11], s3, k2[3]);
    full_add(s0, s1, s2, t, k2[4]);
    if (EXTRA) full_add(t, s3, f, n0, k2[5]);
    else half_add(t, s3, n0, k2[5]);
    full_add(k2[0], k2[1], k2[2], a2, k40);
    full_add(k2[3], k2[4], k2[5], b2, k41);
    if (B >= 0 && B <= 3) {
        const uint32_t r1 = __builtin_amdgcn_bitop3_b32(k40, k41, keep, 0x02);
        if (B == 3) return __builtin_amdgcn_bitop3_b32(r1, a2, b2, 0x70);
        if (B == 1) return __builtin_amdgcn_bitop3_b32(r1, a2, b2, 0x10);
        if (B == 0) return __builtin_amdgcn_bitop3_b32(__builtin_amdgcn_bitop3_b32(r1, a2, b2, 0x10), n0, n0, 0x30);
        const uint32_t r2 = __builtin_amdgcn_bitop3_b32(r1, a2, b2, 0x70);
        return __builtin_amdgcn_bitop3_b32(r2, a2 ^ b2, n0, 0x70);
    }
    const uint32_t k42 = a2 & b2;
    if (B == 4) {
        const uint32_t w = __builtin_amdgcn_bitop3_b32(a2, b2, n0, 0xBE);
        const uint32_t p = __builtin_amdgcn_bitop3_b32(k40, k41, k42, 0xE8);
        const uint32_t o = __builtin_amdgcn_bitop3_b32(k40, k41, k42, 0xFE);
        const uint32_t x = __builtin_amdgcn_bitop3_b32(o, w, keep, 0x2A);
        return __builtin_amdgcn_bitop3_b32(x, p, p, 0x30);
    }
    uint32_t n2, n3;
    full_add(k40, k41, k42, n2, n3);
    const uint32_t n[4] = {n0, a2 ^ b2, n2, n3};
    uint32_t gt = 0u, eq = ~0u;
#pragma unroll
    for (int b = 3; b >= 0; --b) {
        if ((thr >> b) & 1u) {
            eq &= n[b];
        } else {
            gt |= eq & n[b];
            eq &= ~n[b];
        }
    }
    return keep & ~gt;
}

template <int B>
__device__ __forceinline__ uint32_t near_plane12(const uint32_t (&c)[24], uint32_t gw, uint32_t thr, uint32_t keep, PrevSlice &prev)
{
    uint32_t m[12];
#pragma unroll
    for (int p = 0; p < 12; ++p) {
        const uint32_t g0 = 0u - ((gw >> p) & 1u);
        const uint32_t g1 = 0u - ((gw >> (12 + p)) & 1u);
        m[p] = (c[p] ^ g0) | (c[12 + p] ^ g1);
    }
    return count_near12<B, false>(m, 0u, thr, keep, prev);
}

template <int B>
__device__ __forceinline__ uint32_t near_plane12_masks(const uint32_t (&c)[24], const uint4 *gm ,
                                                       uint32_t thr, uint32_t keep, PrevSlice &prev)
{
    uint32_t m[12];
#pragma unroll
    for (int q = 0; q < 3; ++q) {
        const uint4 lo = gm[q], hi = gm[3 + q];
        asm volatile("" ::: "memory");
        m[4 * q + 0] = (c[4 * q + 0] ^ lo.x) | (c[12 + 4 * q + 0] ^ hi.x);
        m[4 * q + 1] = (c[4 * q + 1] ^ lo.y) | (c[12 + 4 * q + 1] ^ hi.y);
        m[4 * q + 2] = (c[4 * q + 2] ^ lo.z) | (c[12 + 4 * q + 2] ^ hi.z);
        m[4 * q + 3] = (c[4 * q + 3] ^ lo.w) | (c[12 + 4 * q + 3] ^ hi.w);
    }
    const uint32_t f = reinterpret_cast<const uint32_t *>(gm)[24];
    return count_near12<B, true>(m, f, thr, keep, prev);
}

__device__ __forceinline__ uint32_t fine_dup(uint32_t ok, const PrevSlice &prev, uint32_t dup_filter)
{
    const uint32_t prev_mismatch = __builtin_amdgcn_bitop3_b32(prev.a, prev.b, prev.c, 0xFE);
    return ok & (prev_mismatch | ~dup_filter);
}

struct alignas(4) GuideGroupAny {
    uint32_t w[kGuideGroup];
};
struct alignas(8) FineSlotGroup {
    FineSlot s[kGuideGroup];
};

constexpr uint32_t fine_order_code(uint32_t slice, uint32_t slice_width)
{
    return fine_order(slice, 0u, slice_width) | (fine_order(slice, 1u, slice_width) << 2) | (fine_order(slice, 2u, slice_width) << 4);
}
constexpr uint32_t kFineOrders = fine_order_code(0u, 8u) | (fine_order_code(1u, 8u) << 6) | (fine_order_code(2u, 8u) << 12) |
                                 (fine_order_code(3u, 8u) << 18) | (fine_order_code(4u, 8u) << 24);
constexpr uint32_t kFineOrderNarrow = fine_order_code(0u, 4u);
static_assert(fine_order_code(0u, 2u) == kFineOrderNarrow && fine_order_code(7u, 4u) == kFineOrderNarrow && (kFineOrders & 63u) == kFineOrderNarrow,
              "narrow slices: one order, that of slice 0 of the 8-bit ones");

struct RecLane {
    uint32_t lo, hi;
};
__device__ __forceinline__ RecLane rec_lane(uint32_t tile, uint32_t off0)
{
    return {(tile << 11) | off0, tile >> 21};
}
__device__ __forceinline__ RecLane rec_lane_at(uint32_t group_abs, uint32_t cand)
{
    const uint64_t at = (static_cast<uint64_t>(group_abs) << 5) + cand;
    return {static_cast<uint32_t>(at), static_cast<uint32_t>(at >> 32)};
}

__device__ __forceinline__ void note_candidates(uint32_t ok, uint32_t gslot, const uint32_t *pass_ids, uint32_t w_log, const RecLane &rl,
                                                uint32_t lane, RawWriter &w, uint64_t *raw, uint32_t *raw_used,
                                                uint32_t max_chunks, Counters *counters)
{
    uint64_t who = __ballot(ok != 0u);
    if (who == 0ull) return;
    do {
        const uint32_t n = static_cast<uint32_t>(__builtin_popcountll(who));
        if (__builtin_expect(w.fill + n > kChunkRecs, 0)) {
            raw_retire(w, lane, raw, raw_used);
            raw_acquire(w, raw, max_chunks, counters, lane);
        }
        if (ok != 0u) {
            const uint32_t q = static_cast<uint32_t>(__builtin_ctz(ok));
            ok &= ok - 1u;
            const uint32_t rank = __builtin_amdgcn_mbcnt_hi(static_cast<uint32_t>(who >> 32),
                                                            __builtin_amdgcn_mbcnt_lo(static_cast<uint32_t>(who), 0u));
            const uint32_t slot = pass_ids ? pass_ids[q >> w_log] : gslot + (q >> w_log);
            const uint32_t lo = rl.lo | (q & ((1u << w_log) - 1u)), hi = rl.hi | (slot << 5);
            w.chunk[w.fill + rank] = (static_cast<uint64_t>(hi) << 32) | lo;
        }
        w.fill += n;
        who = __ballot(ok != 0u);
    } while (__builtin_expect(who != 0ull, 0));
}

template <int THR, bool FINE>
__device__ __forceinline__ void scan_range(const uint32_t *__restrict__ scan_stream, const ScanItem *__restrict__ items,
                                           const PlanInfo *__restrict__ plan, const RangeStart *__restrict__ range_start,
                                           const std::conditional_t<FINE, FineSlot, uint32_t> *__restrict__ gword_stream, uint4 *wave_masks,
                                           uint64_t *raw, uint32_t *raw_used, uint32_t max_chunks,
                                           Counters *counters, uint32_t thr, unsigned long long *stamps,
                                           uint64_t *__restrict__ scan_count, uint32_t *next_unit_p, uint32_t *waves_done_p,
                                           unsigned long long *wg_compared_p, unsigned long long t_start,
                                           unsigned long long *span, uint32_t n_tiles, uint32_t slice_bits)
{
    uint32_t &next_unit = *next_unit_p;
    uint32_t &waves_done = *waves_done_p;
    unsigned long long &wg_compared = *wg_compared_p;
    constexpr bool fine = FINE;
    uint32_t units_done = 0;
    unsigned long long plane_wait = 0ull;
    const uint32_t lane = threadIdx.x & 63u;
    const uint32_t wave_id = __builtin_amdgcn_readfirstlane(blockIdx.x * (blockDim.x >> 6) + (threadIdx.x >> 6));
    RawWriter w;
    const bool no_own_chunk = wave_id >= max_chunks;
    w.chunk = raw + static_cast<uint64_t>(no_own_chunk ? max_chunks : wave_id) * kChunkRecs;
    w.fill = 1;
    w.left = 0;
    w.reserve = 1;
    bool own_chunk = false;
    unsigned long long compared = 0ull;

    const RangeStart first = range_start[blockIdx.x];
    const RangeStart last = range_start[blockIdx.x + 1];
    const uint32_t tile_begin = items[first.item].tile0 + first.tile;
    const uint32_t tile_last = items[last.item].tile0 + last.tile;
    const uint32_t n_units = tile_last - tile_begin + (last.goff ? 1u : 0u);
    uint32_t it = first.item;
    ScanItem cur = items[it];

    const uint32_t order_step = slice_bits == 8u ? 6u : 0u;
    while (true) {
        uint32_t u = 0;
        if (lane == 0) u = atomicAdd(&next_unit, 1u);
        u = __builtin_amdgcn_readfirstlane(u);
        if (u >= n_units) break;
        ++units_done;
        const uint32_t gt = tile_begin + u;
        if (fine) { it = gt; cur = items[gt]; }
        else while (gt >= cur.tile0 + cur.n_tiles) cur = items[++it];
        const uint32_t k = gt - cur.tile0;
        const uint32_t g_begin = cur.g0 + (u == 0 ? first.goff : 0u);
        const uint32_t g_end = (gt == tile_last) ? cur.g0 + last.goff : cur.g1;

        if constexpr (FINE) {
            const uint32_t slice_of = cur.bucket >> (8u + slice_bits);
            const uint32_t order = (kFineOrders >> (slice_of * order_step)) & 63u;
            const uint32_t dup_filter = slice_of != 0u ? ~0u : 0u;
            const uint32_t t0 = cur.group_abs >> 6, g0 = cur.group_abs & 63u;
            const uint32_t next_tile = t0 + 1u < n_tiles ? 64u * 16u : 0u;
            const char *planes = reinterpret_cast<const char *>(scan_stream) + static_cast<uint64_t>(t0) * (4u * kTileCands) + 4096u;
            const char *plane0 = planes + ((order & 3u) << 10), *plane1 = planes + (((order >> 2) & 3u) << 10), *plane2 = planes + ((order >> 4) << 10);
            const uint32_t lo = cur.window & 0xFFFFu, hi = cur.window >> 16;
            compared += static_cast<unsigned long long>(cur.last_cands) * (g_end - g_begin);
            if (cur.shape != 32u) {
                const bool wide = cur.shape == 16u;
                const uint32_t shape = wide ? 16u : 8u, w_log = wide ? 4u : 3u, per_log = wide ? 1u : 2u, per = wide ? 2u : 4u;
                const uint32_t at16 = (g0 + (lane >> per_log)) << 4, sub = lane & (per - 1u);
                const uint32_t off = (at16 & 0x3F0u) + ((at16 & next_tile) << 3);
                const uint32_t sel = (wide ? 0x01000100u : 0u) + sub * (wide ? 0x02020202u : 0x01010101u);
                uint32_t c[24];
                {
                    const uint4 a0 = *reinterpret_cast<const uint4 *>(plane0 - 4096 + off), a1 = *reinterpret_cast<const uint4 *>(plane1 - 4096 + off);
                    const uint4 a2 = *reinterpret_cast<const uint4 *>(plane2 - 4096 + off);
                    const uint4 b0 = *reinterpret_cast<const uint4 *>(plane0 + off), b1 = *reinterpret_cast<const uint4 *>(plane1 + off);
                    const uint4 b2 = *reinterpret_cast<const uint4 *>(plane2 + off);
                    const uint4 t6[6] = {a0, a1, a2, b0, b1, b2};
#pragma unroll
                    for (int q = 0; q < 6; ++q) {
                        c[4 * q + 0] = __builtin_amdgcn_perm(0u, t6[q].x, sel); c[4 * q + 1] = __builtin_amdgcn_perm(0u, t6[q].y, sel);
                        c[4 * q + 2] = __builtin_amdgcn_perm(0u, t6[q].z, sel); c[4 * q + 3] = __builtin_amdgcn_perm(0u, t6[q].w, sel);
                    }
                }
                const int mine0 = static_cast<int>(lane << w_log), width = static_cast<int>(shape);
                const int from = min(max(static_cast<int>(lo) - mine0, 0), width), to = min(max(static_cast<int>(hi) - mine0, 0), width);
                const uint32_t keep = ((1u << to) - (1u << from)) * (wide ? 0x00010001u : 0x01010101u);
                const RecLane rl = rec_lane_at(cur.group_abs, lane << w_log);
                for (uint32_t gb = g_begin; gb < g_end; gb += 8u * per) {
                    __builtin_amdgcn_wave_barrier();
                    short_unit_masks(gword_stream, gb, wide, lane, wave_masks);
                    __builtin_amdgcn_fence(__ATOMIC_RELEASE, "wavefront");
                    __builtin_amdgcn_wave_barrier();
                    const uint32_t passes = (g_end - gb + per - 1u) >> per_log;
                    for (uint32_t i = 0; i < (passes < 8u ? passes : 8u); ++i) {
                        PrevSlice prev;
                        const uint32_t ok = near_plane12_masks<THR>(c, wave_masks + i * 8u, thr, keep, prev);
                        if (__ballot(ok != 0u) != 0ull) {
                            note_candidates(fine_dup(ok, prev, dup_filter), 0u, reinterpret_cast<const uint32_t *>(wave_masks + i * 8u) + kPassIds, w_log, rl, lane, w, raw,
                                            raw_used, max_chunks, counters);
                            own_chunk = true;
                        }
                    }
                }
                continue;
            }
            const uint32_t at16 = (g0 + lane) << 4;
            const uint32_t off = (at16 & 0x3F0u) + ((at16 & next_tile) << 3);
            uint32_t c[24];
            {
                const uint4 a0 = *reinterpret_cast<const uint4 *>(plane0 - 4096 + off), a1 = *reinterpret_cast<const uint4 *>(plane1 - 4096 + off);
                const uint4 a2 = *reinterpret_cast<const uint4 *>(plane2 - 4096 + off);
                const uint4 b0 = *reinterpret_cast<const uint4 *>(plane0 + off), b1 = *reinterpret_cast<const uint4 *>(plane1 + off);
                const uint4 b2 = *reinterpret_cast<const uint4 *>(plane2 + off);
                c[0] = a0.x; c[1] = a0.y; c[2] = a0.z; c[3] = a0.w; c[4] = a1.x; c[5] = a1.y; c[6] = a1.z; c[7] = a1.w;
                c[8] = a2.x; c[9] = a2.y; c[10] = a2.z; c[11] = a2.w;
                c[12] = b0.x; c[13] = b0.y; c[14] = b0.z; c[15] = b0.w; c[16] = b1.x; c[17] = b1.y; c[18] = b1.z; c[19] = b1.w;
                c[20] = b2.x; c[21] = b2.y; c[22] = b2.z; c[23] = b2.w;
            }
            const int to = min(max(static_cast<int>(hi) - static_cast<int>(lane << 5), 0), 32);
            const uint32_t keep = static_cast<uint32_t>((0xFFFFFFFFull << to) >> 32) & (lane == 0u ? ~0u << lo : ~0u);
            const RecLane rl = rec_lane_at(cur.group_abs, lane << 5);
            if (stamps) {
                const unsigned long long t1 = __builtin_amdgcn_s_memrealtime();
                asm volatile("s_waitcnt vmcnt(0)" ::: "memory");
                plane_wait += __builtin_amdgcn_s_memrealtime() - t1;
            }
            if constexpr (THR < 0) {
                for (uint32_t g = g_begin; g < g_end; g += kGuideGroup) {
                    const FineSlotGroup gg = *reinterpret_cast<const FineSlotGroup *>(gword_stream + g);
#pragma unroll
                    for (uint32_t uu = 0; uu < kGuideGroup; ++uu) {
                        if (g + uu >= g_end) break;
                        const uint32_t cls = (gg.s[uu].word >> 24) & 3u;
                        if (cls > thr) continue;
                        PrevSlice prev;
                        const uint32_t ok = near_plane12<-1>(c, gg.s[uu].word, thr - cls, keep, prev);
                        if (__ballot(ok != 0u) != 0ull) {
                            note_candidates(fine_dup(ok, prev, dup_filter), gg.s[uu].id, nullptr, 5u, rl, lane, w, raw, raw_used, max_chunks, counters);
                            own_chunk = true;
                        }
                    }
                }
                continue;
            }
            const uint32_t gmid = cur.gmid < g_begin ? g_begin : cur.gmid > g_end ? g_end : cur.gmid;
            if constexpr (THR >= 1) {
                {
                    for (uint32_t g = g_begin; g < gmid; g += kGuideGroup) {
                        const FineSlotGroup gg = *reinterpret_cast<const FineSlotGroup *>(gword_stream + g);
#pragma unroll
                        for (uint32_t uu = 0; uu < kGuideGroup; ++uu) {
                            if (g + uu >= gmid) break;
                            PrevSlice prev;
                            const uint32_t ok = near_plane12<(THR < 1 ? 0 : THR - 1)>(c, gg.s[uu].word, thr - 1u, keep, prev);
                            if (__ballot(ok != 0u) != 0ull) {
                                note_candidates(fine_dup(ok, prev, dup_filter), gg.s[uu].id, nullptr, 5u, rl, lane, w, raw, raw_used, max_chunks, counters);
                                own_chunk = true;
                            }
                        }
                    }
                }
            }
            for (uint32_t g = gmid; g < g_end; g += kGuideGroup) {
                const FineSlotGroup gg = *reinterpret_cast<const FineSlotGroup *>(gword_stream + g);
#pragma unroll
                for (uint32_t uu = 0; uu < kGuideGroup; ++uu) {
                    if (g + uu >= g_end) break;
                    PrevSlice prev;
                    const uint32_t ok = near_plane12<THR>(c, gg.s[uu].word, thr, keep, prev);
                    if (__ballot(ok != 0u) != 0ull) {
                        note_candidates(fine_dup(ok, prev, dup_filter), gg.s[uu].id, nullptr, 5u, rl, lane, w, raw, raw_used, max_chunks, counters);
                        own_chunk = true;
                    }
                }
            }
            continue;
        }

        const uint32_t glane = cur.group_abs + (k << 6) + lane;
        const uint32_t tile = __builtin_amdgcn_readfirstlane(glane >> 6), grp = lane;
        compared += static_cast<unsigned long long>((k + 1u == cur.n_tiles) ? cur.last_cands : kTileCands) * (g_end - g_begin);
        const uint4 *__restrict__ src =
            reinterpret_cast<const uint4 *>(scan_stream + static_cast<uint64_t>(tile) * kTileCands) + grp;
        uint32_t c[kPlanes];
#pragma unroll
        for (int q = 0; q < kPlanes / 4; ++q) {
            const uint4 t4 = src[q * 64];
            c[4 * q + 0] = t4.x; c[4 * q + 1] = t4.y; c[4 * q + 2] = t4.z; c[4 * q + 3] = t4.w;
        }
        const int lo = (k == 0u) ? static_cast<int>(cur.window & 0xFFFFu) : 0;
        const int hi = (k + 1u == cur.n_tiles) ? static_cast<int>(cur.window >> 16) : static_cast<int>(kTileCands);
        const int below = lo - static_cast<int>(lane * 32u), upto = hi - static_cast<int>(lane * 32u);
        const uint32_t keep = (below <= 0 ? ~0u : below >= 32 ? 0u : ~0u << below) &
                              (upto >= 32 ? ~0u : upto <= 0 ? 0u : ~0u >> (32 - upto));
        const RecLane rl = rec_lane(tile, grp * 32u);
        if (stamps) {
            const unsigned long long t1 = __builtin_amdgcn_s_memrealtime();
            asm volatile("s_waitcnt vmcnt(0)" ::: "memory");
            plane_wait += __builtin_amdgcn_s_memrealtime() - t1;
        }
        for (uint32_t g = g_begin; g < g_end; g += kGuideGroup) {
            const GuideGroup gg = *reinterpret_cast<const GuideGroup *>(gword_stream + g);
#pragma unroll
            for (uint32_t uu = 0; uu < kGuideGroup; ++uu) {
                if (g + uu >= g_end) break;
                const uint32_t ok = near_plane<THR>(c, gg.w[uu], thr, keep);
                if (__ballot(ok != 0u) != 0ull) {
                    note_candidates(ok, g + uu, nullptr, 5u, rl, lane, w, raw, raw_used, max_chunks, counters);
                    own_chunk = true;
                }
            }
        }
    }
    if (own_chunk) {
        raw_retire(w, lane, raw, raw_used);
        if (no_own_chunk && lane == 0) counters->raw_overflow = 1u;
    }
    if (lane == 0) {
        atomicAdd(&wg_compared, compared);
        if (atomicAdd(&waves_done, 1u) == (blockDim.x >> 6) - 1u) {
            scan_count[blockIdx.x] = atomicAdd(&wg_compared, 0ull);
            atomicMax(span + 1, static_cast<unsigned long long>(__builtin_amdgcn_s_memrealtime()));
        }
    }
    if (stamps && lane == 0) {
        stamps[4 * wave_id] = t_start;
        stamps[4 * wave_id + 1] = __builtin_amdgcn_s_memrealtime();
        stamps[4 * wave_id + 2] = (static_cast<unsigned long long>(__builtin_amdgcn_s_getreg((20 << 0) | (0 << 6) | (31 << 11))) << 32) |
                                  __builtin_amdgcn_s_getreg((4 << 0) | (0 << 6) | (31 << 11));
        stamps[4 * wave_id + 3] = units_done | (plane_wait << 32);
    }
}

template <int THR>
__global__ __launch_bounds__(1024, 8) void k_scan(const uint32_t *__restrict__ scan_stream,
                                                  const ScanItem *__restrict__ items_full,
                                                  const ScanItem *__restrict__ items_fine,
                                                  const PlanInfo *__restrict__ plan,
                                                  const RangeStart *__restrict__ range_start,
                                                  const uint32_t *__restrict__ gword_full,
                                                  const FineSlot *__restrict__ gword_fine, uint64_t *raw,
                                                  uint32_t *raw_used, uint32_t max_chunks, Counters *counters, uint32_t thr,
                                                  unsigned long long *stamps, uint64_t *__restrict__ scan_count,
                                                  unsigned long long *span, uint32_t n_tiles, uint32_t slice_bits)
{
    __shared__ uint32_t next_unit;
    __shared__ uint32_t waves_done;
    __shared__ unsigned long long wg_compared;
    __shared__ uint4 tail_masks[16][64];
    const unsigned long long t_start = __builtin_amdgcn_s_memrealtime();
    if (threadIdx.x == 0) { next_unit = 0; waves_done = 0; wg_compared = 0ull; }
    __syncthreads();
    if (blockIdx.x >= plan->n_ranges) {
        if (threadIdx.x == 0) scan_count[blockIdx.x] = 0ull;
        return;
    }
    if (threadIdx.x == 0) atomicMin(span, t_start);
    if (plan->fine != 0u)
        scan_range<THR, true>(scan_stream, items_fine, plan, range_start, gword_fine, tail_masks[threadIdx.x >> 6], raw, raw_used, max_chunks, counters, thr, stamps,
                              scan_count, &next_unit, &waves_done, &wg_compared, t_start, span, n_tiles, slice_bits);
    else
        scan_range<THR, false>(scan_stream, items_full, plan, range_start, gword_full, tail_masks[threadIdx.x >> 6], raw, raw_used, max_chunks, counters, thr, stamps,
                               scan_count, &next_unit, &waves_done, &wg_compared, t_start, span, n_tiles, slice_bits);
}

template <int THR>
static void launch_scan_thr(const ImageView &v, const Workspace &ws, const Tuning &tn, uint32_t thr, uint32_t prune_mode,
                            hipStream_t stream)
{
    hipLaunchKernelGGL(k_scan<THR>, dim3(tn.scan_blocks), dim3(tn.scan_threads), 0, stream, v.scan, ws.items,
                       prune_mode ? ws.fitems : ws.items, ws.plan, ws.range_start, ws.gword, ws.fword,
                       ws.raw, ws.raw_used, static_cast<uint32_t>(ws.cap_chunks), ws.counters, thr, ws.stamps, ws.scan_count,
                       ws.scan_span + 2u * ws.span_slot, v.n_tiles, v.slice_width);
}

void launch_scan(const ImageView &v, const Workspace &ws, const Tuning &tn, const uint64_t *d_guides, uint32_t n,
                 int max_dist, uint32_t prune_mode, void *stream_)
{
    (void)n;
    (void)d_guides;
    hipStream_t stream = static_cast<hipStream_t>(stream_);
    if (max_dist < 0) {
        (void)hipMemsetAsync(ws.scan_count, 0, 8ull * tn.scan_blocks, stream);
        return;
    }
    const uint32_t thr = max_dist > 31 ? 31u : static_cast<uint32_t>(max_dist);
    if (tn.scan_generic || thr > 4) launch_scan_thr<-1>(v, ws, tn, thr, prune_mode, stream);
    else if (thr == 0) launch_scan_thr<0>(v, ws, tn, thr, prune_mode, stream);
    else if (thr == 1) launch_scan_thr<1>(v, ws, tn, thr, prune_mode, stream);
    else if (thr == 2) launch_scan_thr<2>(v, ws, tn, thr, prune_mode, stream);
    else if (thr == 3) launch_scan_thr<3>(v, ws, tn, thr, prune_mode, stream);
    else launch_scan_thr<4>(v, ws, tn, thr, prune_mode, stream);
}

}
```

crackling_amd/csrc/issl_kernels.hpp:

```cpp
#pragma once
#include <hip/hip_runtime.h>

#include "issl_device.hpp"

namespace issl {


__device__ __forceinline__ void short_kernel_priority() { __builtin_amdgcn_s_setprio(3); }

__host__ __device__ inline uint32_t gather_even16(uint32_t x)
{
    x &= 0x55555555u;
    x = (x | (x >> 1)) & 0x33333333u;
    x = (x | (x >> 2)) & 0x0F0F0F0Fu;
    x = (x | (x >> 4)) & 0x00FF00FFu;
    x = (x | (x >> 8)) & 0x0000FFFFu;
    return x;
}

__host__ __device__ inline uint32_t scan_word(uint64_t sig, uint32_t s, uint32_t width = 8u)
{
    const uint32_t sh = width * s;
    const uint64_t low = sig & ((1ull << sh) - 1ull);
    const uint64_t high = (sig >> (sh + width)) << sh;
    const uint32_t rem = static_cast<uint32_t>(low | high);
    return gather_even16(rem) | (gather_even16(rem >> 1) << 16);
}

__host__ __device__ inline uint32_t scan_word_sorted_narrow(uint64_t sig, uint32_t s, uint32_t width)
{
    const uint32_t sh = (width * (s + 1u)) % 40u;
    const uint64_t x = sig & kSigMask;
    const uint64_t a = (sh ? (x >> sh) | (x << (40u - sh)) : x) & kSigMask;
    const uint64_t prev = (a >> (40u - 2u * width)) & ((1ull << width) - 1ull);
    const uint64_t mid = (a >> 8) & ((1ull << (24u - width)) - 1ull);
    const uint32_t rem = static_cast<uint32_t>((a & 0xFFull) | (prev << 8) | (mid << (8u + width)));
    return gather_even16(rem) | (gather_even16(rem >> 1) << 16);
}
__host__ __device__ inline uint32_t image_word(uint64_t sig, uint32_t s, uint32_t width, bool sorted_layout)
{
    return (sorted_layout && width < 8u) ? scan_word_sorted_narrow(sig, s, width) : scan_word(sig, s, width);
}

__host__ __device__ inline uint64_t mismatch_mask(uint64_t a, uint64_t b)
{
    const uint64_t x = a ^ b;
    return ((x & 0xAAAAAAAAAAAAAAAAull) >> 1) | (x & 0x5555555555555555ull);
}

constexpr int kPlanes = 32;

__host__ __device__ inline uint32_t plane_word(uint32_t r, uint32_t group)
{
    return ((r >> 2) * 64u + group) * 4u + (r & 3u);
}

__device__ inline uint64_t candidate_signature(const ImageView &v, uint32_t bucket, uint32_t tile, uint32_t offset)
{
    const uint4 *src = reinterpret_cast<const uint4 *>(v.scan + static_cast<uint64_t>(tile) * kTileCands);
    const uint32_t group = offset >> 5, bit = offset & 31u;
    uint32_t w = 0;
#pragma unroll
    for (uint32_t q = 0; q < kPlanes / 4; ++q) {
        const uint4 t4 = src[q * 64u + group];
        w |= ((t4.x >> bit) & 1u) << (4 * q) | ((t4.y >> bit) & 1u) << (4 * q + 1) | ((t4.z >> bit) & 1u) << (4 * q + 2) |
             ((t4.w >> bit) & 1u) << (4 * q + 3);
    }
    uint64_t rem = 0;
#pragma unroll
    for (uint32_t p = 0; p < 16; ++p)
        rem |= static_cast<uint64_t>(((w >> p) & 1u) | (((w >> (16 + p)) & 1u) << 1)) << (2 * p);
    const uint32_t slice = bucket >> v.slice_width;
    const uint32_t sh = v.slice_width * slice;
    const uint64_t key = bucket & ((1u << v.slice_width) - 1u);
    return (rem & ((1ull << sh) - 1ull)) | (key << sh) | ((rem >> sh) << (sh + v.slice_width));
}

__device__ inline uint64_t wave_inclusive_scan_u64(uint64_t x)
{
    const uint32_t lane = threadIdx.x & 63u;
    for (uint32_t d = 1; d < 64; d <<= 1) {
        const uint32_t lo = __shfl_up(static_cast<uint32_t>(x), d, 64);
        const uint32_t hi = __shfl_up(static_cast<uint32_t>(x >> 32), d, 64);
        if (lane >= d) x += (static_cast<uint64_t>(hi) << 32) | lo;
    }
    return x;
}

__device__ inline uint64_t block_exclusive_scan(uint64_t v, uint64_t *lds , uint64_t *total)
{
    const uint32_t lane = threadIdx.x & 63u, wave = threadIdx.x >> 6;
    const uint64_t incl = wave_inclusive_scan_u64(v);
    if (lane == 63) lds[wave] = incl;
    __syncthreads();
    uint64_t before = 0, all = 0;
    for (uint32_t w = 0; w < 4; ++w) {
        const uint64_t s = lds[w];
        if (w < wave) before += s;
        all += s;
    }
    if (total) *total = all;
    __syncthreads();
    return before + incl - v;
}

__host__ __device__ __forceinline__ constexpr uint32_t fine_quad(uint32_t slice) { return slice < 4u ? slice : 0u; }
__host__ __device__ __forceinline__ constexpr uint32_t fine_order(uint32_t slice, uint32_t j, uint32_t slice_width = 8u)
{
    if (slice_width != 8u) return j + 1u;
    const uint32_t sq = fine_quad(slice);
    if (slice == 0u) return j + 1u;
    const uint32_t prev = slice - 1u;
    if (j == 0u) return prev;
    uint32_t q = 0, seen = 0;
    for (; q < 4u; ++q) {
        if (q == sq || q == prev) continue;
        if (++seen == j) break;
    }
    return q;
}

constexpr uint32_t kTailGrid = 16384;
constexpr uint32_t kReplayLds = 512;
static_assert(kReplayLds <= 512, "k_replay sorts (key, 9-bit index) pairs");
constexpr uint32_t kMidHits = 2048;

constexpr uint32_t kScanChunk = 2048;
constexpr uint32_t kBigLds = 7680;

__device__ __forceinline__ uint32_t grouped_hits(uint32_t count, uint32_t slot_hits)
{
    return count <= (slot_hits ? kSlotHits : 0u) ? 0u : count;
}

#define ISSL_CFD_QUAL inline __constant__
#include "cfd_tables.inc"

__device__ inline double mit_lookup(const ImageView &v, uint64_t mask)
{
    if (v.mit_dense) {
        if (mask >> 40) return 0.0;
        const uint32_t idx = gather_even16(static_cast<uint32_t>(mask)) |
                             (gather_even16(static_cast<uint32_t>(mask >> 32)) << 16);
        return v.mit_dense[idx];
    }
    uint32_t lo = 0, hi = v.n_scores;
    while (lo < hi) {
        const uint32_t mid = (lo + hi) >> 1;
        const uint64_t m = v.score_mask[mid];
        if (m == mask) return v.score_val[mid];
        if (m < mask) lo = mid + 1; else hi = mid;
    }
    return 0.0;
}

__device__ inline void score_terms(const ImageView &v, uint64_t gsig, uint64_t ot, uint32_t occ, bool calc_mit, bool calc_cfd,
                                   double &mit_term, double &cfd_term, int &dist_out)
{
    mit_term = 0.0;
    cfd_term = 0.0;
    const uint64_t mm = mismatch_mask(gsig, ot);
    const int dist = __builtin_popcountll(mm);
    dist_out = dist;
    if (calc_mit && dist > 0) mit_term = mit_lookup(v, mm) * static_cast<double>(occ);
    if (calc_cfd) {
        double cfd;
        if (dist == 0) {
            cfd = 1.0;
        } else {
            cfd = issl_cfd_pam[10];
            for (uint64_t left = mm; left != 0ull; left &= left - 1ull) {
                const uint32_t q = static_cast<uint32_t>(__builtin_ctzll(left)) >> 1;
                const uint32_t gb = static_cast<uint32_t>(gsig >> (2 * q)) & 3u;
                const uint32_t ob = static_cast<uint32_t>(ot >> (2 * q)) & 3u;
                cfd *= issl_cfd_pos[(q << 4) | (gb << 2) | (ob ^ 3u)];
            }
        }
        cfd_term = cfd * static_cast<double>(occ);
    }
}

struct HitTerms {
    double mit, cfd;
    issl_hit rec;
};

__device__ inline HitTerms hit_terms(const ImageView &v, uint64_t gsig, uint32_t g, uint64_t key, bool calc_mit,
                                     bool calc_cfd, bool want_id)
{
    HitTerms t;
    t.mit = 0.0;
    t.cfd = 0.0;
    const uint64_t low = (1ull << v.slice_width) - 1ull;
    const uint32_t slice = static_cast<uint32_t>(key >> kKeySliceShift) & kKeySliceMask;
    uint32_t pos = static_cast<uint32_t>(key);
    const uint32_t bucket = (slice << v.slice_width) + static_cast<uint32_t>((gsig >> (v.slice_width * slice)) & low);
    const uint64_t at = v.bucket_start[bucket] + pos;
    uint32_t id = 0, occ;
    uint64_t ot;
    if (v.srec || v.sid) {
        id = pos;
        const uint64_t site = v.sites[id];
        ot = site & kSigMask;
        occ = static_cast<uint32_t>(site >> 40);
        if (occ == kOccSaturated) occ = v.site_occ[id];
        pos = 0;
        if (want_id && v.entries) {
            const uint64_t *list = v.entries + v.bucket_start[bucket];
            uint64_t lo = 0, hi = v.bucket_start[bucket + 1] - v.bucket_start[bucket];
            while (lo < hi) {
                const uint64_t mid = (lo + hi) >> 1;
                if (static_cast<uint32_t>(list[mid]) < id) lo = mid + 1; else hi = mid;
            }
            pos = static_cast<uint32_t>(lo);
        } else if (want_id) {
            const uint32_t *ss = v.sub_start + static_cast<uint64_t>(bucket) * 257u;
            const uint64_t first = static_cast<uint64_t>(v.tile_first[bucket]) * kTileCands;
            for (uint32_t w = 0; w < 256u; ++w) {
                uint32_t lo = ss[w], hi = ss[w + 1];
                const uint32_t s0 = lo;
                while (lo < hi) {
                    const uint32_t mid = (lo + hi) >> 1;
                    const uint32_t there = v.srec ? v.srec[first + mid].id : v.sid[first + mid];
                    if (there < id) lo = mid + 1; else hi = mid;
                }
                pos += lo - s0;
            }
        }
    } else if (v.occ8) {
        ot = candidate_signature(v, bucket, v.tile_first[bucket] + (pos >> 11), pos & (kTileCands - 1u));
        occ = v.occ8[at];
        if (occ == 255u || want_id) {
            const uint64_t e = v.entries[at];
            id = static_cast<uint32_t>(e);
            occ = static_cast<uint32_t>(e >> 32);
        }
    } else {
        const uint64_t e = v.entries[at];
        id = static_cast<uint32_t>(e);
        occ = static_cast<uint32_t>(e >> 32);
        ot = v.esig ? v.esig[at] : v.sites[id];
    }
    int dist;
    score_terms(v, gsig, ot, occ, calc_mit, calc_cfd, t.mit, t.cfd, dist);
    t.rec.guide = g; t.rec.slice = slice; t.rec.pos = pos; t.rec.id = id;
    t.rec.dist = static_cast<uint32_t>(dist); t.rec.occ = occ;
    return t;
}

}
```

crackling_amd/csrc/issl_options.cpp:

```cpp
#include <climits>
#include <cstdlib>
#include <cstring>
#include <string>

#include "issl_device.hpp"

namespace issl {

namespace {

enum Kind { kInt, kFlag, kTri, kPath };

template <class T, T Tuning::*M> void put(Tuning &t, long long v) { t.*M = static_cast<T>(v); }
template <class T, T Tuning::*M> long long get(const Tuning &t) { return static_cast<long long>(t.*M); }
#define MEMBER(m) put<decltype(Tuning::m), &Tuning::m>, get<decltype(Tuning::m), &Tuning::m>

struct Option {
    const char *key, *env;
    Kind kind;
    long long lo, hi, def;
    void (*put)(Tuning &, long long);
    long long (*get)(const Tuning &);
    long long multiple = 1;
    long long round = 1;
};

constexpr long long kNoMax = LLONG_MAX;

const Option kOptions[] = {
    {"scan_blocks", "ISSL_SCAN_BLOCKS", kInt, 1, kScanMaxBlocks, kScanGridBlocks, MEMBER(scan_blocks)},
    {"scan_threads", "ISSL_SCAN_THREADS", kInt, 64, 1024, 1024, MEMBER(scan_threads), 64},
    {"upload_chunk_kib", "ISSL_UPLOAD_CHUNK_KIB", kInt, 4, 1 << 20, 16384, MEMBER(upload_chunk_kib)},
    {"upload_ring_min_kib", "ISSL_UPLOAD_RING_MIN_KIB", kInt, 0, kNoMax, 65536, MEMBER(upload_ring_min_kib)},
    {"upload_threads", "ISSL_UPLOAD_THREADS", kInt, 1, 32, 8, MEMBER(upload_threads)},
    {"item_guides", "ISSL_ITEM_GUIDES", kInt, 8, kItemGuides, kItemGuides, MEMBER(item_guides), 1, 8},
    {"scan_generic", "ISSL_SCAN_GENERIC", kFlag, 0, 1, 0, MEMBER(scan_generic)},
    {"stage_timing", "ISSL_STAGE_TIMING", kFlag, 0, 1, 0, MEMBER(stage_timing)},
    {"scan_events", "ISSL_SCAN_EVENTS", kInt, 0, 2, 2, MEMBER(scan_events)},
    {"raw_chunks", "ISSL_RAW_CHUNKS", kInt, 0, kNoMax, 0, MEMBER(raw_chunks)},
    {"inline_sigs", "ISSL_INLINE_SIGS", kTri, -1, 1, -1, MEMBER(inline_sigs)},
    {"host_cold", "ISSL_FORCE_HOST_COLD", kTri, -1, 1, -1, MEMBER(host_cold)},
    {"scan_stamps", "ISSL_SCAN_STAMPS", kPath, 0, 0, 0, nullptr, nullptr},
    {"sorted_layout", "ISSL_SORTED_LAYOUT", kTri, -1, 1, -1, MEMBER(sorted_layout)},
    {"prune", "ISSL_PRUNE", kTri, -1, 1, -1, MEMBER(prune)},
    {"lanes", "ISSL_LANES", kInt, 1, 3, 1, MEMBER(lanes)},
    {"compact", "ISSL_COMPACT", kTri, -1, 1, -1, MEMBER(compact)},
    {"tail_shapes", "ISSL_TAIL_SHAPES", kFlag, 0, 1, 1, MEMBER(tail_shapes)},
    {"hit_slots", "ISSL_HIT_SLOTS", kInt, 0, 2, 1, MEMBER(hit_slots)},
    {"lean_tail", "ISSL_LEAN_TAIL", kFlag, 0, 1, 1, MEMBER(lean_tail)},
    {"small_bin", "ISSL_SMALL_BIN", kFlag, 0, 1, 1, MEMBER(small_bin)},
    {"expect_guides", "ISSL_EXPECT_GUIDES", kInt, 0, kNoMax, 0, MEMBER(expect_guides)},
    {"fine_items", "ISSL_FINE_ITEMS", kInt, 0, kNoMax, 0, MEMBER(fine_items)},
    {"keep_lists", "ISSL_KEEP_LISTS", kTri, -1, 1, -1, MEMBER(keep_lists)},
};
#undef MEMBER

const Option *find(const char *key)
{
    for (const Option &o : kOptions)
        if (std::strcmp(o.key, key) == 0) return &o;
    return nullptr;
}

struct ImageKey {
    const char *key;
    long long (*get)(const ImageHeader &h);
};

const ImageKey kImageKeys[] = {
    {"is_sorted", [](const ImageHeader &h) -> long long { return (h.off_srec || h.off_sid) ? 1 : 0; }},
    {"is_compact", [](const ImageHeader &h) -> long long { return h.off_sid ? 1 : 0; }},
    {"cold_on_host", [](const ImageHeader &h) -> long long { return h.cold_on_host ? 1 : 0; }},
    {"cold_sections", [](const ImageHeader &h) -> long long { return h.cold_on_host; }},
    {"lists_absent", [](const ImageHeader &h) -> long long { return h.lists_absent; }},
    {"dense_mit", [](const ImageHeader &h) -> long long { return h.off_mit_dense ? 1 : 0; }},
    {"has_inline_sigs", [](const ImageHeader &h) -> long long { return h.off_esig ? 1 : 0; }},
};

}

Tuning Tuning::from_env()
{
    Tuning t;
    for (const Option &o : kOptions)
        if (o.put) o.put(t, o.def);
    const char *timing = std::getenv("ISSL_UPLOAD_TIMING");
    t.upload_timing = timing && timing[0] == '1';
    for (const Option &o : kOptions)
        if (const char *e = std::getenv(o.env)) (void)t.set(o.key, e);
    return t;
}

bool Tuning::set(const char *key, const char *value)
{
    const Option *o = key && value ? find(key) : nullptr;
    if (!o) return false;
    if (o->kind == kPath) {
        stamps_path = value;
        return true;
    }
    char *end = nullptr;
    const long long n = std::strtoll(value, &end, 10);
    if (end == value || *end != 0 || n < o->lo || n > o->hi || n % o->multiple) return false;
    o->put(*this, n / o->round * o->round);
    return true;
}

bool Tuning::get(const char *key, long long *value) const
{
    const Option *o = find(key);
    if (!o || o->kind == kPath) return false;
    *value = o->get(*this);
    return true;
}

int Tuning::set_list(const char *options)
{
    for (std::string rest = options ? options : ""; !rest.empty();) {
        const size_t comma = rest.find(',');
        const std::string item = rest.substr(0, comma);
        rest = comma == std::string::npos ? std::string() : rest.substr(comma + 1);
        const size_t eq = item.find('=');
        if (eq == std::string::npos || !set(item.substr(0, eq).c_str(), item.substr(eq + 1).c_str())) {
            set_error("unknown option or value out of range: " + item);
            return ISSL_E_ARG;
        }
    }
    return ISSL_OK;
}

bool image_option(const ImageHeader *h, const char *key, long long *value)
{
    for (const ImageKey &k : kImageKeys)
        if (std::strcmp(k.key, key) == 0) {
            *value = h ? k.get(*h) : -1;
            return true;
        }
    return false;
}

}
```

crackling_amd/csrc/issl_pipeline.cpp:

```cpp
#include <algorithm>
#include <cstdio>
#include <cstring>
#include <vector>

#include "issl_index.hpp"

namespace issl {

int supported_geometry(const Geometry &g)
{
    if (g.seq_len == 20 && (g.slice_width == 8 || g.slice_width == 4 || g.slice_width == 2) && g.n_slices * g.slice_width == 40) return ISSL_OK;
    set_error("unsupported index geometry: the gfx950 scan kernels implement 20 bp sequences in slices of 8, 4 or 2 bits "
              "(got seq_len=" + std::to_string(g.seq_len) + " slice_width=" +
              std::to_string(g.slice_width) + " slices=" + std::to_string(g.n_slices) + ")");
    return ISSL_E_UNSUPPORTED;
}

static void free_workspace(Workspace &w)
{
    void *ptrs[] = {w.ng, w.gfill, w.gstart, w.gword, w.gidx, w.gbucket, w.gsig, w.items, w.plan, w.range_start, w.counters, w.scan_count, w.scan_span, w.sticky, w.stamps, w.gcur_big, w.gcur_big2, w.terms, w.sorted, w.gcount,
                    w.goff, w.blocksum, w.d_guides, w.d_mit, w.d_cfd, w.d_kept, w.d_hitrec, w.pay, w.rank, w.fword,
                    w.fitems, w.fcount, w.fcount0, w.fsum, w.slots};
    for (void *p : ptrs)
        if (p) (void)hipFree(p);
    if (w.raw) (void)hipFree(w.raw);
    if (w.raw_used) (void)hipFree(w.raw_used);
    if (w.h_stage) (void)hipHostFree(w.h_stage);
    w = Workspace{};
}

void release_lanes(issl_index *ix)
{
    for (Lane *lp : {&ix->lane, &ix->lane2}) {
        Lane &lane = *lp;
        if (lane.ready) {
            (void)hipStreamSynchronize(lane.stream);
            (void)hipStreamSynchronize(lane.tail_stream);
            for (auto &e : lane.ev) (void)hipEventDestroy(e);
            (void)hipEventDestroy(lane.done);
            (void)hipStreamDestroy(lane.stream);
            (void)hipStreamDestroy(lane.tail_stream);
            lane.ready = false;
        }
        free_workspace(lane.ws);
        lane.lean = false;
        lane.last_n = 0;
        lane.pending = 0;
    }
    ix->last_lane = nullptr;
    if (ix->have_events) {
        for (auto &e : ix->ring) (void)hipEventDestroy(e);
        ix->have_events = false;
    }
    ix->n_pending = 0;
    ix->n_ring = 0;
    ix->proven_guides = 0;
    ix->proven_chunks = 0;
    ix->proven_dist = -1;
    ix->prev_scan_end = nullptr;
    ix->prev_batch_end = nullptr;
}

static bool ensure_stage(Workspace &w, size_t bytes)
{
    if (w.h_stage_bytes >= bytes) return true;
    if (w.h_stage) (void)hipHostFree(w.h_stage);
    w.h_stage = nullptr;
    w.h_stage_bytes = 0;
    const size_t want = bytes + bytes / 4;
    if (hipHostMalloc(&w.h_stage, want, hipHostMallocDefault) != hipSuccess) { (void)hipGetLastError(); w.h_stage = nullptr; return false; }
    w.h_stage_bytes = want;
    return true;
}

template <typename T> static int dev_alloc(T *&p, size_t count)
{
    if (p) {
        (void)hipFree(p);
        p = nullptr;
    }
    HIP_TRY(hipMalloc(reinterpret_cast<void **>(&p), std::max<size_t>(count, 1) * sizeof(T)));
    return ISSL_OK;
}

static int ensure_hit_capacity(Workspace &w, size_t want)
{
    if (want <= w.cap_hits) return ISSL_OK;
    int rc;
    if ((rc = dev_alloc(w.sorted, want))) return rc;
    if ((rc = dev_alloc(w.terms, 2 * want))) return rc;
    if ((rc = dev_alloc(w.pay, 2 * want))) return rc;
    if ((rc = dev_alloc(w.rank, want))) return rc;
    w.cap_hits = want;
    return ISSL_OK;
}

int ensure_raw_capacity(Workspace &w, size_t chunks)
{
    if (chunks <= w.cap_chunks) return ISSL_OK;
    int rc = dev_alloc(w.raw, (chunks + 1) * kChunkRecs);
    if (rc) return rc;
    if ((rc = dev_alloc(w.raw_used, chunks + 1))) return rc;
    w.cap_chunks = chunks;
    return ISSL_OK;
}

int ensure_workspace(issl_index *ix, size_t n, Lane &lane, uint32_t fine_ways)
{
    Workspace &w = lane.ws;
    const Tuning &tn = ix->tuning;
    const size_t nb = ix->hdr.n_buckets;
    int rc;
    if (w.n_buckets != nb) {
        if ((rc = dev_alloc(w.ng, nb))) return rc;
        if ((rc = dev_alloc(w.gfill, nb))) return rc;
        HIP_TRY(hipMemset(w.ng, 0, 4 * nb));
        HIP_TRY(hipMemset(w.gfill, 0, 4 * nb));
        if ((rc = dev_alloc(w.gstart, nb + 1))) return rc;
        if ((rc = dev_alloc(w.counters, 1))) return rc;
        if ((rc = dev_alloc(w.plan, 1))) return rc;
        if ((rc = dev_alloc(w.range_start, kMaxRanges + 2))) return rc;
        if ((rc = dev_alloc(w.scan_count, kScanMaxBlocks))) return rc;
        if ((rc = dev_alloc(w.scan_span, 2 * kSpanRing))) return rc;
        HIP_TRY(hipMemset(w.scan_span, 0, 16 * kSpanRing));
        HIP_TRY(hipMemset(w.scan_count, 0, 8 * kScanMaxBlocks));
        w.n_buckets = static_cast<uint32_t>(nb);
    }
    bool grew = false;
    const bool force_wide = tn.hit_slots == 2 && w.slot_width != kSlotHitsWide &&
                            std::max<size_t>(std::max<size_t>(n, w.cap_guides), 1024) * kSlotHitsWide * sizeof(SlotRec) <= kSlotBytesMax;
    if (force_wide) w.slot_width = kSlotHitsWide;
    if (n > w.cap_guides || (force_wide && w.slots)) {
        grew = true;
        const size_t cap = std::max<size_t>(std::max<size_t>(n, w.cap_guides), 1024);
        const size_t slots = cap * ix->hdr.n_slices + kGuideGroup * nb;
        const size_t items = nb + cap * ix->hdr.n_slices / 8 + 2;
        if ((rc = dev_alloc(w.gword, slots))) return rc;
        if ((rc = dev_alloc(w.gidx, slots))) return rc;
        if ((rc = dev_alloc(w.gbucket, slots))) return rc;
        if ((rc = dev_alloc(w.gsig, slots))) return rc;
        if ((rc = dev_alloc(w.items, items + 1))) return rc;
        if ((rc = dev_alloc(w.gcount, cap + 1))) return rc;
        if ((rc = dev_alloc(w.goff, cap + 1))) return rc;
        if ((rc = dev_alloc(w.gcur_big, cap + 1))) return rc;
        if ((rc = dev_alloc(w.gcur_big2, cap + 1))) return rc;
        if ((rc = dev_alloc(w.blocksum, (cap + 1) / 2048 + 2))) return rc;
        if ((rc = dev_alloc(w.d_guides, cap))) return rc;
        if ((rc = dev_alloc(w.d_mit, cap))) return rc;
        if ((rc = dev_alloc(w.d_cfd, cap))) return rc;
        if ((rc = dev_alloc(w.d_kept, cap))) return rc;
        if (w.slots) { (void)hipFree(w.slots); w.slots = nullptr; }
        w.cap_slot_guides = 0;
        if (cap * w.slot_width * sizeof(SlotRec) > kSlotBytesMax) w.slot_width = kSlotHits;
        if (cap * w.slot_width * sizeof(SlotRec) <= kSlotBytesMax) {
            if (hipMalloc(reinterpret_cast<void **>(&w.slots), cap * w.slot_width * sizeof(SlotRec)) == hipSuccess) w.cap_slot_guides = cap;
            else { (void)hipGetLastError(); w.slots = nullptr; }
        }
        w.cap_guides = cap;
        w.cap_gslots = slots;
        w.cap_items = items;
    }
    if (ix->hdr.off_sub_start && (grew || fine_ways > w.fine_ways)) {
        const size_t cap = w.cap_guides;
        const uint32_t ways = std::max(fine_ways, w.fine_ways);
        const size_t m = std::min<size_t>(cap, prune_max_guides(ways > kFineWays ? 3u : 2u, ix->hdr.n_slices));
        const size_t places = m * ix->hdr.n_slices * ways;
        const size_t groups = std::min<size_t>(nb * 256, places);
        const size_t fslots = places + kGuideGroup * groups;
        const size_t tiles_per_group = static_cast<size_t>(ix->hdr.n_sites * ix->hdr.n_slices / (static_cast<uint64_t>(nb) * 256ull * kTileCands)) + 4;
        const size_t fitems = std::max<size_t>(tn.fine_items ? tn.fine_items : tiles_per_group * (groups + places / 64) + 2, w.cap_fitems);
        if ((rc = dev_alloc(w.fword, fslots + 64))) return rc;
        if ((rc = dev_alloc(w.fitems, fitems + 1))) return rc;
        if ((rc = dev_alloc(w.fcount, nb * 256))) return rc;
        if ((rc = dev_alloc(w.fcount0, nb * 256))) return rc;
        if ((rc = dev_alloc(w.fsum, nb))) return rc;
        w.cap_fslots = fslots;
        w.cap_fitems = fitems;
        w.fine_ways = ways;
    }

    if (w.cap_chunks == 0) {
        const size_t want = tn.raw_chunks ? tn.raw_chunks : std::max<size_t>(size_t(scan_waves(tn)) * 6, n);
        if ((rc = ensure_raw_capacity(w, want))) return rc;
    }
    if (!ix->have_events) {
        for (auto &e : ix->ring) HIP_TRY(hipEventCreate(&e));
        ix->have_events = true;
    }
    if (!lane.ready) {
        for (auto &e : lane.ev) HIP_TRY(hipEventCreate(&e));
        HIP_TRY(hipEventCreate(&lane.done));
        int prio_low = 0, prio_high = 0;
        HIP_TRY(hipDeviceGetStreamPriorityRange(&prio_low, &prio_high));
        HIP_TRY(hipStreamCreateWithPriority(&lane.stream, hipStreamNonBlocking, prio_low));
        HIP_TRY(hipStreamCreateWithPriority(&lane.tail_stream, hipStreamNonBlocking, prio_high));
        lane.ready = true;
    }
    if (!w.stamps && !tn.stamps_path.empty()) {
        if ((rc = dev_alloc(w.stamps, kStampsWords))) return rc;
        HIP_TRY(hipMemset(w.stamps, 0, 8ull * kStampsWords));
    }
    if (!w.sticky) {
        if ((rc = dev_alloc(w.sticky, 4))) return rc;
        HIP_TRY(hipMemset(w.sticky, 0, 16));
    }
    return ISSL_OK;
}

static int enqueue_batch(issl_index *ix, Lane &lane, hipStream_t stream, const uint64_t *d_guides, size_t n, int max_dist,
                         double threshold, int method, double *d_mit, double *d_cfd, bool dump, bool staged,
                         int lanes_mode = 1, issl_profile *d_profile = nullptr)
{
    const bool pipelined = lanes_mode == 2, bin_ahead = lanes_mode == 3;
    if (!ix->d_image) {
        set_error("index has no device image: call issl_index_upload first");
        return ISSL_E_STATE;
    }
    const size_t max_batch = std::min<size_t>(kMaxBatch, ((size_t(1) << 27) - kGuideGroup * ix->hdr.n_buckets) / std::max<uint64_t>(ix->hdr.n_slices, 1));
    if (n > max_batch) {
        set_error("at most " + std::to_string(max_batch) + " guides per device batch on this index (issl_score splits larger batches itself)");
        return ISSL_E_ARG;
    }
    HIP_TRY(hipSetDevice(ix->device));
    if (n == 0) return ISSL_OK;
    const uint32_t prune_mode = prune_mode_for(ix->view, ix->tuning, static_cast<uint32_t>(n), max_dist);
    int rc = ensure_workspace(ix, n, lane, fine_ways_of(prune_mode ? prune_mode : 2u));
    if (rc) return rc;
    Workspace &ws = lane.ws;
    const Tuning &tn = ix->tuning;
    rc = ensure_hit_capacity(ws, ws.cap_chunks * (kChunkRecs - 1));
    if (rc) return rc;
    if (dump && ws.cap_hitrec < ws.cap_hits) {
        rc = dev_alloc(ws.d_hitrec, ws.cap_hits);
        if (rc) return rc;
        ws.cap_hitrec = ws.cap_hits;
    }
    ws.slot_hits = (!dump && tn.hit_slots && ws.cap_slot_guides >= n) ? ws.slot_width : 0u;
    ws.lean_tail = (lane.lean && ws.slot_hits >= kSlotHits && tn.lean_tail) ? 1u : 0u;
    ScoreParams p;
    p.max_dist = max_dist;
    p.method = method;
    p.maximum_sum = (10000.0 - threshold * 100) / threshold;
    const uint32_t n32 = static_cast<uint32_t>(n);
    const bool scan_pair = staged || pipelined || tn.scan_events == 1 || (tn.scan_events == 2 && ix->n_ring == 0);
    const uint32_t slot = ix->n_ring % kRing;
    lane.staged = staged;
    if (pipelined && lane.pending) HIP_TRY(hipStreamWaitEvent(stream, lane.done, 0));
    if (staged) HIP_TRY(hipEventRecord(lane.ev[0], stream));
    ws.span_slot = lane.pending % kSpanRing;
    launch_bin_guides(ix->view, ws, tn, d_guides, n32, prune_mode, stream);
    if (staged) HIP_TRY(hipEventRecord(lane.ev[1], stream));
    if (pipelined && ix->prev_scan_end) HIP_TRY(hipStreamWaitEvent(stream, ix->prev_scan_end, 0));
    if (bin_ahead && ix->prev_batch_end) HIP_TRY(hipStreamWaitEvent(stream, ix->prev_batch_end, 0));
    if (scan_pair) HIP_TRY(hipEventRecord(ix->ring[2 * slot], stream));
    launch_scan(ix->view, ws, tn, d_guides, n32, max_dist, prune_mode, stream);
    if (scan_pair) HIP_TRY(hipEventRecord(ix->ring[2 * slot + 1], stream));
    if (scan_pair) ix->n_ring += 1;
    if (staged) HIP_TRY(hipEventRecord(lane.ev[2], stream));
    hipStream_t tail = stream;
    if (pipelined) {
        tail = lane.tail_stream;
        HIP_TRY(hipStreamWaitEvent(tail, ix->ring[2 * slot + 1], 0));
        ix->prev_scan_end = ix->ring[2 * slot + 1];
    }
    launch_verify(ix->view, ws, d_guides, static_cast<uint32_t>(n), p, tail);
    if (staged) HIP_TRY(hipEventRecord(lane.ev[3], tail));
    launch_group_hits(ws, n32, tail);
    if (staged) HIP_TRY(hipEventRecord(lane.ev[4], tail));
    if (d_profile) launch_profile(ix->view, ws, d_guides, n32, d_profile, tail);
    else launch_replay(ix->view, ws, d_guides, n32, p, d_mit, d_cfd, dump ? ws.d_kept : nullptr,
                       dump ? ws.d_hitrec : nullptr, tail);
    if (staged) HIP_TRY(hipEventRecord(lane.ev[5], tail));
    if (pipelined || bin_ahead) HIP_TRY(hipEventRecord(lane.done, tail));
    lane.done_recorded = pipelined || bin_ahead;
    lane.last_tail = tail;
    if (bin_ahead) ix->prev_batch_end = lane.done;
    ix->n_pending += 1;
    lane.pending += 1;
    lane.last_n = n32;
    lane.last_max_dist = max_dist;
    lane.last_prune = prune_mode;
    ix->last_lane = &lane;
    return ISSL_OK;
}

int finish_batches(issl_index *ix, hipStream_t stream)
{
    if (!ix->d_image || ix->n_pending == 0) return ISSL_OK;
    HIP_TRY(hipSetDevice(ix->device));
    HIP_TRY(hipStreamSynchronize(stream));
    for (Lane *lp : {&ix->lane, &ix->lane2})
        if (lp->ready && lp->pending) {
            HIP_TRY(hipStreamSynchronize(lp->stream));
            HIP_TRY(hipStreamSynchronize(lp->tail_stream));
        }
    ix->prev_scan_end = nullptr;
    ix->prev_batch_end = nullptr;
    HIP_TRY(hipGetLastError());
    const uint32_t batches = ix->n_pending;
    const uint32_t ring_pairs = ix->n_ring;
    ix->n_pending = 0;
    ix->n_ring = 0;
    bool retry = false;
    uint32_t max_chunks = 0;
    Lane &lane = ix->last_lane ? *ix->last_lane : ix->lane;
    double span_sum = 0.0;
    uint32_t span_count = 0;
    for (Lane *lp : {&ix->lane, &ix->lane2}) {
        if (!lp->pending) continue;
        {
            const uint32_t have = lp->pending < kSpanRing ? lp->pending : kSpanRing;
            unsigned long long spans[2 * kSpanRing];
            HIP_TRY(hipMemcpy(spans, lp->ws.scan_span, 16 * have, hipMemcpyDeviceToHost));
            for (uint32_t i = 0; i < have; ++i)
                if (spans[2 * i + 1] > spans[2 * i]) { span_sum += static_cast<double>(spans[2 * i + 1] - spans[2 * i]); ++span_count; }
        }
        lp->pending = 0;
        uint32_t sticky[4] = {0, 0, 0, 0};
        HIP_TRY(hipMemcpy(sticky, lp->ws.sticky, sizeof sticky, hipMemcpyDeviceToHost));
        if (lp == &lane) max_chunks = sticky[1];
        if (sticky[2] & 2u) {
            HIP_TRY(hipMemset(lp->ws.sticky, 0, 16));
            set_error("internal error: scan item list overflow");
            return ISSL_E_DEVICE;
        }
        if (sticky[3] > lp->ws.cap_fitems && lp->ws.fitems) {
            const size_t want = static_cast<size_t>(sticky[3]) + sticky[3] / 4 + 2;
            uint32_t zero = 0;
            HIP_TRY(hipMemcpy(lp->ws.sticky + 3, &zero, 4, hipMemcpyHostToDevice));
            int rc = dev_alloc(lp->ws.fitems, want + 1);
            if (rc) return rc;
            lp->ws.cap_fitems = want;
        }
        if (lp->ws.slots && lp->ws.slot_width == kSlotHits && ix->tuning.hit_slots && lp->last_n) {
            Counters c{};
            HIP_TRY(hipMemcpy(&c, lp->ws.counters, sizeof c, hipMemcpyDeviceToHost));
            const size_t want = lp->ws.cap_slot_guides * size_t(kSlotHitsWide) * sizeof(SlotRec);
            size_t free_b = 0, total_b = 0;
            if (c.overflowed > lp->last_n / 8 && want <= kSlotBytesMax && hipMemGetInfo(&free_b, &total_b) == hipSuccess &&
                free_b > want + (size_t(4) << 30)) {
                SlotRec *wide = nullptr;
                if (hipMalloc(reinterpret_cast<void **>(&wide), want) == hipSuccess) {
                    (void)hipFree(lp->ws.slots);
                    lp->ws.slots = wide;
                    lp->ws.slot_width = kSlotHitsWide;
                } else {
                    (void)hipGetLastError();
                }
            }
        }
        lp->lean = (sticky[0] & 6u) == 0u && lp->ws.slot_hits >= kSlotHits;
        if (sticky[0] & 2u) retry = true;
        if (sticky[0] & 1u) {
            int rc = ensure_raw_capacity(lp->ws, static_cast<size_t>(sticky[1]) + sticky[1] / 8 + 1024);
            if (rc) return rc;
            retry = true;
        }
        if (sticky[0]) HIP_TRY(hipMemset(lp->ws.sticky, 0, 16));
    }
    if (retry) {
        ix->lane.lean = false;
        ix->lane2.lean = false;
        set_error("a batch has to be scored again: its raw record buffer was too small (it has been enlarged), or it was enqueued "
                  "without the many-hit part of the pipeline and met a guide that needs it");
        return ISSL_E_RETRY;
    }
    PlanInfo pl{};
    uint32_t total_hits = 0;
    HIP_TRY(hipMemcpy(&pl, lane.ws.plan, sizeof pl, hipMemcpyDeviceToHost));
    {
        std::vector<uint32_t> counts(lane.last_n);
        if (lane.last_n) HIP_TRY(hipMemcpy(counts.data(), lane.ws.gcount, 4 * counts.size(), hipMemcpyDeviceToHost));
        for (uint32_t c : counts) total_hits += c;
    }
    std::vector<uint64_t> counted(ix->tuning.scan_blocks);
    HIP_TRY(hipMemcpy(counted.data(), lane.ws.scan_count, 8 * counted.size(), hipMemcpyDeviceToHost));
    uint64_t compared = 0;
    for (uint64_t c : counted) compared += c;
    float ms[5] = {0, 0, 0, 0, 0};
    if (lane.staged)
        for (int i = 0; i < 5; ++i) (void)hipEventElapsedTime(&ms[i], lane.ev[i], lane.ev[i + 1]);
    double scan_sum = 0.0;
    const uint32_t have = ring_pairs < kRing ? ring_pairs : kRing;
    for (uint32_t i = 0; i < have; ++i) {
        float t = 0;
        (void)hipEventElapsedTime(&t, ix->ring[2 * i], ix->ring[2 * i + 1]);
        scan_sum += t;
    }
    ix->stats = issl_stats{};
    ix->stats.n_guides = lane.last_n;
    ix->stats.ms_bin = ms[0];
    ix->stats.ms_scan_events = have ? scan_sum / have : ms[1];
    ix->stats.ms_scan = span_count ? span_sum / span_count * 1e-5 : 0.0;
    ix->stats.ms_verify = ms[2];
    ix->stats.ms_group = ms[3];
    ix->stats.ms_replay = ms[4];
    ix->stats.ms_total = ms[0] + ms[1] + ms[2] + ms[3] + ms[4];
    ix->stats.raw_records = static_cast<uint64_t>(max_chunks) * (kChunkRecs - 1);
    ix->stats.candidates = compared;
    ix->stats.planned_comparisons = lane.last_max_dist < 0 ? 0 : pl.candidates;
    ix->stats.reference_comparisons = pl.reference_candidates;
    ix->stats.pruned = lane.last_prune ? pl.fine : 0;
    ix->stats.hits = total_hits;
    ix->stats.scan_tiles = pl.tiles;
    ix->stats.n_batches = batches;
    if (lane.ws.stamps) {
        std::vector<unsigned long long> st(kStampsWords);
        HIP_TRY(hipMemcpy(st.data(), lane.ws.stamps, 8ull * kStampsWords, hipMemcpyDeviceToHost));
        if (FILE *f = std::fopen(ix->tuning.stamps_path.c_str(), "wb")) {
            std::fwrite(st.data(), 8, st.size(), f);
            std::fclose(f);
        }
    }
    return ISSL_OK;
}

int score_core(issl_index *ix, const uint64_t *d_guides, size_t n, int max_dist, double threshold, int method,
               double *d_mit, double *d_cfd, hipStream_t stream, bool dump, issl_profile *d_profile)
{
    int rc = finish_batches(ix, stream);
    if (rc) return rc;
    ix->stats = issl_stats{};
    ix->stats.n_guides = n;
    if (n == 0) return ISSL_OK;
    for (int attempt = 0;; ++attempt) {
        rc = enqueue_batch(ix, ix->lane, stream, d_guides, n, max_dist, threshold, method, d_mit, d_cfd, dump, true, 1, d_profile);
        if (rc) return rc;
        rc = finish_batches(ix, stream);
        if (rc == ISSL_OK) {
            ix->stats.scan_launches = attempt + 1;
            return ISSL_OK;
        }
        if (rc != ISSL_E_RETRY) return rc;
        if (attempt >= 6) {
            set_error("internal error: raw record buffer kept overflowing");
            return ISSL_E_DEVICE;
        }
    }
}

template <class RunPiece>
static int for_each_piece(issl_index *idx, const uint64_t *guides, size_t n, int max_dist, RunPiece &&run_piece)
{
    HIP_TRY(hipSetDevice(idx->device));
    const uint32_t piece_mode = prune_mode_for(idx->view, idx->tuning, 1, max_dist);
    size_t piece = piece_mode ? size_t(prune_max_guides(piece_mode, idx->view.n_slices)) : size_t(1) << 22;
    if (idx->tuning.hit_slots) piece = std::min(piece, kSlotBytesMax / (size_t(kSlotHits) * sizeof(SlotRec)));
    {
        const size_t n_pieces = (n + piece - 1) / piece;
        piece = std::min(piece, (((n + n_pieces - 1) / n_pieces) + 7) & ~size_t(7));
    }
    const bool estimate = !idx->tuning.raw_chunks && n >= (size_t(1) << 15);
    const double records_per_comparison = 8e-5;
    double budget_slots = -1.0;
    const uint64_t per = idx->geo.buckets_per_slice();
    if (estimate && !idx->worst_per_guide)
        for (uint64_t sl = 0; sl < idx->geo.n_slices; ++sl)
            idx->worst_per_guide += *std::max_element(idx->bucket_sizes.begin() + sl * per, idx->bucket_sizes.begin() + (sl + 1) * per);
    const size_t wave_chunks = size_t(scan_waves(idx->tuning)) * 10;
    issl_stats total{};
    for (size_t at = 0; at < n;) {
        uint64_t cand = 0;
        size_t cnt = 0;
        const size_t most = std::min(piece, n - at);
        const size_t cap_chunks = idx->lane.ws.cap_chunks;
        const double have_slots = static_cast<double>(cap_chunks > wave_chunks ? cap_chunks - wave_chunks : 0) * (kChunkRecs - 1);
        const bool covered = static_cast<double>(most) * static_cast<double>(idx->worst_per_guide) * records_per_comparison <= have_slots ||
                             (most <= idx->proven_guides && cap_chunks >= idx->proven_chunks && idx->proven_chunks > 0 && max_dist <= idx->proven_dist);
        if (!estimate || covered) cnt = most;
        while (estimate && !covered && at + cnt < n && cnt < piece) {
            uint64_t c = 0;
            for (uint64_t sl = 0; sl < idx->geo.n_slices; ++sl)
                c += idx->bucket_sizes[sl * per + ((guides[at + cnt] >> (idx->geo.slice_width * sl)) & (per - 1))];
            const double want = static_cast<double>(cand + c) * records_per_comparison;
            if (want > have_slots) {
                if (budget_slots < 0.0) {
                    size_t free_b = 0, total_b = 0;
                    HIP_TRY(hipMemGetInfo(&free_b, &total_b));
                    budget_slots = std::max(have_slots, static_cast<double>(std::min<size_t>(free_b / 4, size_t(32) << 30)) / 32.0);
                }
                if (cnt > 0 && want > budget_slots) break;
            }
            cand += c;
            ++cnt;
        }
        Workspace &ws = idx->lane.ws;
        int rc = finish_batches(idx, nullptr);
        if (rc) return rc;
        rc = ensure_workspace(idx, cnt, idx->lane);
        if (rc) return rc;
        if (estimate && !covered) {
            double slots = static_cast<double>(cand) * records_per_comparison;
            if (budget_slots >= 0.0) slots = std::min(slots, budget_slots);
            size_t want_chunks = static_cast<size_t>(slots / (kChunkRecs - 1)) + wave_chunks;
            if (want_chunks > ws.cap_chunks && ws.cap_chunks > 0) {
                const size_t roomy = ws.cap_chunks + ws.cap_chunks / 4;
                const size_t most_chunks = budget_slots >= 0.0 ? static_cast<size_t>(budget_slots / (kChunkRecs - 1)) + wave_chunks : roomy;
                want_chunks = std::max(want_chunks, std::min(roomy, std::max(most_chunks, want_chunks)));
            }
            rc = ensure_raw_capacity(ws, want_chunks);
            if (rc) return rc;
        }
        rc = run_piece(at, cnt);
        if (rc) return rc;
        const issl_stats &s = idx->stats;
        if (s.scan_launches == 1 && (max_dist > idx->proven_dist || (max_dist == idx->proven_dist && cnt > idx->proven_guides))) {
            idx->proven_dist = max_dist;
            idx->proven_guides = cnt;
            idx->proven_chunks = ws.cap_chunks;
        }
        total.n_guides += s.n_guides; total.candidates += s.candidates; total.hits += s.hits;
        total.planned_comparisons += s.planned_comparisons; total.reference_comparisons += s.reference_comparisons;
        total.pruned = std::max(total.pruned, s.pruned);
        total.scan_tiles += s.scan_tiles; total.ms_bin += s.ms_bin; total.ms_scan += s.ms_scan;
        total.ms_scan_events += s.ms_scan_events;
        total.ms_verify += s.ms_verify; total.ms_group += s.ms_group; total.ms_replay += s.ms_replay;
        total.ms_total += s.ms_total; total.scan_launches += s.scan_launches;
        total.raw_records = std::max(total.raw_records, s.raw_records); total.n_batches += s.n_batches;
        at += cnt;
    }
    idx->stats = total;
    return ISSL_OK;
// ... 239 lines not shown
```

crackling_amd/csrc/issl_verify.hip:

```cpp
#include <hip/hip_runtime.h>

#include <algorithm>

#include "issl_kernels.hpp"

namespace issl {

__global__ __launch_bounds__(kChunkRecs, 8) void k_verify(ImageView v, Workspace ws, const uint64_t *__restrict__ guides,
                                                       uint32_t n, ScoreParams p)
{
    short_kernel_priority();
    const int max_dist = p.max_dist;
    const bool calc_mit = p.method == ISSL_METHOD_MIT || p.method == ISSL_METHOD_AND || p.method == ISSL_METHOD_OR ||
                          p.method == ISSL_METHOD_AVG;
    const bool calc_cfd = p.method == ISSL_METHOD_CFD || p.method == ISSL_METHOD_AND || p.method == ISSL_METHOD_OR ||
                          p.method == ISSL_METHOD_AVG;
    const uint32_t prune_mode = ws.plan->fine;
    uint32_t n_chunks = ws.counters->raw_chunks;
    if (blockIdx.x == 0 && threadIdx.x == 0) {
        if (ws.counters->raw_overflow) atomicOr(&ws.sticky[0], 1u);
        atomicMax(&ws.sticky[1], n_chunks);
        if (ws.plan->error) atomicOr(&ws.sticky[2], ws.plan->error);
    }
    if (n_chunks > ws.cap_chunks) n_chunks = static_cast<uint32_t>(ws.cap_chunks);
    const uint64_t low = (1ull << v.slice_width) - 1ull;
    for (uint32_t chunk = blockIdx.x; chunk < n_chunks; chunk += gridDim.x) {
        uint64_t *recs = ws.raw + static_cast<uint64_t>(chunk) * kChunkRecs;
        const uint32_t t = threadIdx.x + 1u;
        const uint64_t rec_any = recs[t < kChunkRecs ? t : 0u];
        const uint32_t used = ws.raw_used[chunk];
        const bool in_use = t < used && t < kChunkRecs;
        const uint64_t rec = in_use ? rec_any : 0ull;
        uint64_t key = kDeadKey;
        double mit_term = 0.0, cfd_term = 0.0;
        uint64_t hit_gsig = 0, hit_ot = 0;
        uint32_t hit_occ = 0;
        const uint32_t offset = static_cast<uint32_t>(rec) & (kTileCands - 1u);
        const uint32_t tile = static_cast<uint32_t>(rec >> 11) & 0x3FFFFFFu;
        const uint32_t gslot = static_cast<uint32_t>(rec >> 37);
        const bool by_id = v.srec || v.sid;
        StreamRec sr_early{};
        if (in_use && v.srec) sr_early = v.srec[static_cast<uint64_t>(tile) * kTileCands + offset];
        else if (in_use && v.sid) sr_early.id = v.sid[static_cast<uint64_t>(tile) * kTileCands + offset];
        uint32_t guide = kNoGuide, bucket = 0, slice = 0;
        uint64_t gsig = 0;
        if (in_use) {
            if (prune_mode) {
                if (gslot != kPadSlotId) slot_id_unpack(gslot, slice, guide);
                if (guide >= n || slice >= v.n_slices) guide = kNoGuide;
                else {
                    gsig = guides[guide];
                    bucket = (slice << v.slice_width) + (static_cast<uint32_t>(gsig >> (v.slice_width * slice)) & static_cast<uint32_t>(low));
                }
            } else {
                guide = ws.gidx[gslot];
                bucket = ws.gbucket[gslot];
                slice = bucket >> v.slice_width;
            }
        }
        if (guide != kNoGuide) {
            uint64_t start = 0, pos = 0;
            bool mine = true;
            if (!by_id) {
                start = v.bucket_start[bucket];
                pos = static_cast<uint64_t>(tile - v.tile_first[bucket]) * kTileCands + offset;
                mine = pos < v.bucket_start[bucket + 1] - start;
            }
            if (mine) {
                if (!prune_mode) gsig = guides[guide];
                StreamRec sr = sr_early;
                if (v.sid) sr.sig = v.sites[sr.id];
                const uint64_t ot = by_id    ? sr.sig & kSigMask
                                    : v.esig ? v.esig[start + pos]
                                    : v.occ8 ? candidate_signature(v, bucket, tile, offset)
                                             : v.sites[v.entries[start + pos] & 0xFFFFFFFFull];
                if (__builtin_popcountll(mismatch_mask(gsig, ot)) <= max_dist) {
                    const uint64_t x = gsig ^ ot;
                    if (!prune_mode) {
                        bool earlier = false;
                        for (uint32_t j = 0; j < slice; ++j)
                            if (((x >> (v.slice_width * j)) & low) == 0) earlier = true;
                        if (!earlier) {
                            const uint64_t lp = by_id ? sr.id : pos;
                            key = (static_cast<uint64_t>(guide) << kKeyGuideShift) | (static_cast<uint64_t>(slice) << kKeySliceShift) | lp;
                        }
                    } else {
                        const uint32_t tol = prune_mode - 1u;
                        const uint64_t mm = mismatch_mask(gsig, ot);
                        uint32_t first = slice, reporter = slice;
                        for (uint32_t j = slice; j-- > 0;) {
                            if (((x >> (v.slice_width * j)) & low) != 0) continue;
                            first = j;
                            if (static_cast<uint32_t>(__builtin_popcount(succ_byte(mm, j, v.slice_width))) <= tol) reporter = j;
                        }
                        if (reporter == slice)
                            key = (static_cast<uint64_t>(guide) << kKeyGuideShift) | (static_cast<uint64_t>(first) << kKeySliceShift) | sr.id;
                    }
                    if (key != kDeadKey) {
                        uint32_t occ;
                        if (by_id) {
                            occ = static_cast<uint32_t>(sr.sig >> 40);
                            if (occ == kOccSaturated) occ = v.site_occ[sr.id];
                        } else if (v.occ8) {
                            occ = v.occ8[start + pos];
                            if (occ == 255u) occ = static_cast<uint32_t>(v.entries[start + pos] >> 32);
                        } else {
                            occ = static_cast<uint32_t>(v.entries[start + pos] >> 32);
                        }
                        hit_gsig = gsig; hit_ot = ot; hit_occ = occ;
                    }
                }
            }
        }
        const bool live = key != kDeadKey;
        const uint32_t lane = threadIdx.x & 63u;
        const uint32_t prev_guide = static_cast<uint32_t>(__shfl_up(static_cast<int>(live ? guide : kNoGuide), 1, 64));
        const bool continues = live && lane != 0u && prev_guide == guide;
        const uint64_t starts = __ballot(!continues);
        uint32_t rank = 0;
        if (starts == ~0ull) {
            if (live) rank = atomicAdd(&ws.gcount[guide], 1u);
        } else {
            const uint64_t upto = (lane == 63u ? 0ull : (~0ull << (lane + 1u)));
            const uint32_t head = 63u - static_cast<uint32_t>(__builtin_clzll(starts & ~upto));
            const uint64_t later = starts & upto;
            const uint32_t next = later ? static_cast<uint32_t>(__builtin_ctzll(later)) : 64u;
            uint32_t base = 0;
            if (live && !continues) base = atomicAdd(&ws.gcount[guide], next - lane);
            rank = static_cast<uint32_t>(__shfl(static_cast<int>(base), static_cast<int>(head), 64)) + (lane - head);
        }
        if (live && rank == kReplayLds) atomicAdd(&ws.counters->overflowed, 1u);
        if (live && rank < ws.slot_hits) {
            int dist;
            score_terms(v, hit_gsig, hit_ot, hit_occ, calc_mit, calc_cfd, mit_term, cfd_term, dist);
            const uint64_t at = static_cast<uint64_t>(guide) * ws.slot_hits + rank;
            SlotRec r;
            r.mit = mit_term; r.cfd = cfd_term; r.key = key;
            r.pad = slot_pad(hit_occ, static_cast<uint32_t>(dist));
            ws.slots[at] = r;
            key = kDeadKey;
        } else if (live) {
            const uint64_t slot = static_cast<uint64_t>(chunk) * (kChunkRecs - 1u) + (t - 1u);
            ws.rank[slot] = rank;
            if (rank < kMidHits) {
                int dist;
                score_terms(v, hit_gsig, hit_ot, hit_occ, calc_mit, calc_cfd, mit_term, cfd_term, dist);
                reinterpret_cast<double2 *>(ws.pay)[slot] = make_double2(mit_term, cfd_term);
            }
        }
        if (!in_use) continue;
        if (!ws.lean_tail) recs[t] = key;
    }
}

void launch_verify(const ImageView &v, const Workspace &ws, const uint64_t *d_guides, uint32_t n, const ScoreParams &p, void *stream)
{
    if (p.max_dist < 0) return;
    const uint32_t grid = n < 256u ? std::max<uint32_t>(2048u, 64u * n) : kTailGrid;
    hipLaunchKernelGGL(k_verify, dim3(std::min(grid, kTailGrid)), dim3(kChunkRecs), 0, static_cast<hipStream_t>(stream), v, ws, d_guides, n, p);
}

}
```

Measured before the change: 48.74 million.

## Verify raw candidate chunks inside the scan kernel's tail instead of separately

Adds an optional in-scan verification path: each scan wave records the raw chunks it fills and, once a chunk is retired, verifies and scores its records within the scan kernel, marking the chunk with a verified bit so the later verify and group kernels can skip it. A plan flag enables the path only when the candidate count per range is large enough. This aims to overlap verification with scanning and cut the separate verify pass's re-read of raw chunks. In exchange it adds LDS state, kernarg pointer tricks and extra registers and branches in the scan kernel, which may hurt occupancy.

```diff
diff --git a/crackling_amd/csrc/issl_bin.hip b/crackling_amd/csrc/issl_bin.hip
--- a/crackling_amd/csrc/issl_bin.hip
+++ b/crackling_amd/csrc/issl_bin.hip
@@ -247,6 +247,7 @@
         plan->candidates = tot_cand;
         plan->reference_candidates = tot_cand;
         plan->fine = 0;
+        plan->scan_tail = 0;
         plan->tiles = tot_tiles;
         plan->n_ranges = (overflow || tot_tiles == 0) ? 0u : ranges_for(tot_tiles, scan_blocks);
         counters->raw_chunks = (plan->n_ranges ? plan->n_ranges : 1u) * 16u;
@@ -461,6 +462,7 @@
             counters->raw_chunks = (plan->n_ranges ? plan->n_ranges : 1u) * 16u;
             plan->fine = prune_mode;
             plan->fine_slots = static_cast<uint32_t>(t_slots);
+            plan->scan_tail = t_cand >= kScanTailCands * 16ull * plan->n_ranges ? 1u : 0u;
         }
     }
 }
diff --git a/crackling_amd/csrc/issl_capi.cpp b/crackling_amd/csrc/issl_capi.cpp
--- a/crackling_amd/csrc/issl_capi.cpp
+++ b/crackling_amd/csrc/issl_capi.cpp
@@ -177,6 +177,7 @@
         {"ws_cap_chunks", static_cast<long long>(w.cap_chunks)},
         {"ws_cap_fitems", static_cast<long long>(w.cap_fitems)},
         {"ws_lean", idx->lane.lean ? 1 : 0},
+        {"ws_scan_verified", static_cast<long long>(idx->lane.scan_verified)},
     };
     for (const auto &k : keys)
         if (std::strcmp(k.key, key) == 0) {
diff --git a/crackling_amd/csrc/issl_device.hpp b/crackling_amd/csrc/issl_device.hpp
--- a/crackling_amd/csrc/issl_device.hpp
+++ b/crackling_amd/csrc/issl_device.hpp
@@ -98,6 +98,7 @@
     int scan_events;
     bool stage_timing;
     bool upload_timing;
+    int scan_verify;
     size_t raw_chunks;
     int inline_sigs;
     int sorted_layout;
@@ -156,6 +157,9 @@
 constexpr uint32_t kSpanRing = 64;
 constexpr uint32_t kChunkRecs = 128;
 constexpr uint64_t kDeadKey = ~0ull;
+constexpr uint32_t kChunkVerified = 1u << 31;
+constexpr uint64_t kScanTailCands = 2ull * 127ull * 2048ull;
+constexpr uint32_t kScanVerifyRuns = 8;
 constexpr uint32_t kKeySliceShift = 32, kKeyGuideShift = 37, kKeySliceMask = 31, kMaxSlices = 20;
 
 struct ScanItem {
@@ -189,7 +193,7 @@
     uint64_t reference_candidates;
     uint64_t tiles;
     uint32_t fine_slots;
-    uint32_t pad;
+    uint32_t scan_tail;
 };
 
 struct Counters {
@@ -200,6 +204,7 @@
     uint32_t raw_chunks;
     uint32_t raw_overflow;
     uint32_t overflowed;
+    uint32_t scan_verified;
     uint32_t replay_next[3];
 };
 
@@ -292,6 +297,7 @@
     SlotRec *slots = nullptr;
     uint32_t slot_hits = 0;
     uint32_t slot_width = kSlotHits;
+    uint32_t scan_verify = 0;
     uint32_t lean_tail = 0;
     size_t cap_slot_guides = 0;
     uint32_t *blocksum = nullptr;
@@ -315,6 +321,25 @@
     double maximum_sum;
 };
 
+struct VerifyCtx {
+    ImageView v;
+    const uint64_t *guides;
+    uint64_t *raw;
+    uint32_t *raw_used;
+    const uint32_t *gidx, *gbucket;
+    uint32_t *gcount;
+    SlotRec *slots;
+    uint32_t *rank;
+    double *pay;
+    Counters *counters;
+    uint32_t n;
+    uint32_t slot_hits, lean_tail;
+    int max_dist;
+    uint32_t calc_mit, calc_cfd;
+    uint32_t scan_verify;
+};
+VerifyCtx make_verify_ctx(const ImageView &v, const Workspace &ws, const Tuning &tn, const uint64_t *d_guides, uint32_t n, const ScoreParams &p);
+
 void launch_pack_scan_stream(const ImageView &v, uint32_t *scan_out, uint64_t *esig_out, uint8_t *occ8_out,
                              uint32_t *error_flag, uint32_t *seen, void *stream);
 void launch_pack_scan_range(const ImageView &v, uint32_t *scan_out, uint64_t *esig_out, uint8_t *occ8_out,
@@ -324,8 +349,8 @@
 void launch_bin_guides(const ImageView &v, const Workspace &ws, const Tuning &tn, const uint64_t *d_guides, uint32_t n,
                        uint32_t prune_mode, void *stream);
 void launch_scan(const ImageView &v, const Workspace &ws, const Tuning &tn, const uint64_t *d_guides, uint32_t n,
-                 int max_dist, uint32_t prune_mode, void *stream);
-void launch_verify(const ImageView &v, const Workspace &ws, const uint64_t *d_guides, uint32_t n, const ScoreParams &p, void *stream);
+                 const ScoreParams &p, uint32_t prune_mode, void *stream);
+void launch_verify(const ImageView &v, const Workspace &ws, const Tuning &tn, const uint64_t *d_guides, uint32_t n, const ScoreParams &p, void *stream);
 void launch_group_hits(const Workspace &ws, uint32_t n, void *stream);
 void launch_replay(const ImageView &v, const Workspace &ws, const uint64_t *d_guides, uint32_t n,
                    const ScoreParams &p, double *d_mit, double *d_cfd, uint32_t *d_kept, issl_hit *d_hitrec,
diff --git a/crackling_amd/csrc/issl_group.hip b/crackling_amd/csrc/issl_group.hip
--- a/crackling_amd/csrc/issl_group.hip
+++ b/crackling_amd/csrc/issl_group.hip
@@ -132,7 +132,7 @@
         const uint64_t key = recs[t < kChunkRecs ? t : 0u];
         const uint32_t my_rank = rank[slot];
         const double2 my_pay = pay[slot];
-        const uint32_t used = raw_used[chunk];
+        const uint32_t used = raw_used[chunk] & ~kChunkVerified;
         if (t >= used || t >= kChunkRecs || key == kDeadKey) continue;
         const uint32_t guide = static_cast<uint32_t>(key >> kKeyGuideShift);
         const uint32_t to = goff[guide] + my_rank;
diff --git a/crackling_amd/csrc/issl_index.hpp b/crackling_amd/csrc/issl_index.hpp
--- a/crackling_amd/csrc/issl_index.hpp
+++ b/crackling_amd/csrc/issl_index.hpp
@@ -29,6 +29,7 @@
     hipStream_t last_tail = nullptr;
     int last_max_dist = 0;
     uint32_t last_prune = 0;
+    uint32_t scan_verified = 0;
     bool lean = false;
 };
 
@@ -62,6 +63,8 @@
     bool list_order_only = false;
     size_t proven_guides = 0, proven_chunks = 0;
     int proven_dist = -1;
+    double plan_cands_per_guide = 0.0;
+    uint32_t plan_cands_prune = 0;
 };
 
 namespace issl {
diff --git a/crackling_amd/csrc/issl_kernels.hip b/crackling_amd/csrc/issl_kernels.hip
--- a/crackling_amd/csrc/issl_kernels.hip
+++ b/crackling_amd/csrc/issl_kernels.hip
@@ -22,7 +22,16 @@
     uint32_t fill;
     uint32_t left;
     uint32_t reserve;
+    uint32_t tail;
 };
+constexpr uint32_t kTailOn = 4u, kTailPending = 1u, kTailRangeDone = 2u, kTailLast = 8u;
+constexpr uint32_t kRunCursor = 1u + kScanVerifyRuns, kRunWords = kRunCursor + 3u;
+__device__ __forceinline__ uint32_t *wave_runs()
+{
+    __shared__ uint32_t runs[16][kRunWords];
+    return runs[threadIdx.x >> 6];
+}
+__device__ __forceinline__ uint32_t run_chunks(uint32_t k) { return k == 0u ? 1u : k > 4u ? 16u : 1u << (k - 1u); }
 
 __device__ __forceinline__ void raw_retire(const RawWriter &w, uint32_t lane, const uint64_t *raw, uint32_t *raw_used)
 {
@@ -33,6 +42,7 @@
                                             uint32_t lane)
 {
     w.fill = 1;
+    if ((w.tail & kTailOn) != 0u) w.tail |= kTailPending | kTailLast;
     if (w.left != 0u) {
         w.chunk += kChunkRecs;
         w.left -= 1u;
@@ -51,6 +61,14 @@
     w.chunk = raw + static_cast<uint64_t>(idx) * kChunkRecs;
     w.left = take - 1u;
     if (take < 16u) w.reserve = take * 2u;
+    if ((w.tail & kTailOn) != 0u && lane == 0) {
+        uint32_t *runs = wave_runs();
+        const uint32_t listed = runs[0];
+        if (listed < kScanVerifyRuns) {
+            runs[1u + listed] = idx;
+            runs[0] = listed + 1u;
+        }
+    }
 }
 
 __device__ __forceinline__ void full_add(uint32_t a, uint32_t b, uint32_t c, uint32_t &sum, uint32_t &carry)
@@ -312,7 +330,37 @@
     } while (__builtin_expect(who != 0ull, 0));
 }
 
-template <int THR, bool FINE>
+__device__ __forceinline__ void scan_tail(uint32_t prune_mode, uint32_t lane, const uint64_t *raw, const uint32_t *raw_used)
+{
+    uint64_t kernarg = reinterpret_cast<uint64_t>(__builtin_amdgcn_kernarg_segment_ptr());
+    asm volatile("" : "+s"(kernarg));
+    KernargCtx &vc = *(KernargCtx *)kernarg;
+    if (vc.raw != raw || vc.raw_used != raw_used) return;
+    uint32_t *runs = wave_runs();
+    asm volatile("s_waitcnt vmcnt(0)" ::: "memory");
+    asm volatile("" : "+v"(lane));
+    const uint32_t listed = __builtin_amdgcn_readfirstlane(runs[0]);
+    uint32_t k = __builtin_amdgcn_readfirstlane(runs[kRunCursor]), j = __builtin_amdgcn_readfirstlane(runs[kRunCursor + 1u]);
+    uint32_t verified = 0;
+    while (k < listed) {
+        const uint32_t chunk = __builtin_amdgcn_readfirstlane(runs[1u + k]) + j;
+        const uint32_t used = __builtin_amdgcn_readfirstlane(__hip_atomic_load(vc.raw_used + chunk, __ATOMIC_RELAXED, __HIP_MEMORY_SCOPE_AGENT));
+        if (used <= 1u) break;
+        const uint64_t *recs = vc.raw + static_cast<uint64_t>(chunk) * kChunkRecs;
+        const uint32_t t0 = lane + 1u, t1 = lane + 65u;
+        const bool use0 = t0 < used, use1 = t1 < used && t1 < kChunkRecs;
+        const uint64_t rec0 = use0 ? __hip_atomic_load(recs + t0, __ATOMIC_RELAXED, __HIP_MEMORY_SCOPE_AGENT) : 0ull;
+        const uint64_t rec1 = use1 ? __hip_atomic_load(recs + t1, __ATOMIC_RELAXED, __HIP_MEMORY_SCOPE_AGENT) : 0ull;
+        verify_record<true>(vc, prune_mode, rec0, use0, chunk, t0, lane);
+        verify_record<true>(vc, prune_mode, rec1, use1, chunk, t1, lane);
+        if (lane == 0) vc.raw_used[chunk] = used | kChunkVerified;
+        verified += (used < kChunkRecs ? used : kChunkRecs) - 1u;
+        if (++j == run_chunks(k)) { j = 0u; ++k; }
+    }
+    if (lane == 0) { runs[kRunCursor] = k; runs[kRunCursor + 1u] = j; runs[kRunCursor + 2u] += verified; }
+}
+
+template <int THR, bool FINE, bool TAIL>
 __device__ __forceinline__ void scan_range(const uint32_t *__restrict__ scan_stream, const ScanItem *__restrict__ items,
                                            const PlanInfo *__restrict__ plan, const RangeStart *__restrict__ range_start,
                                            const std::conditional_t<FINE, FineSlot, uint32_t> *__restrict__ gword_stream, uint4 *wave_masks,
@@ -320,7 +368,8 @@
                                            Counters *counters, uint32_t thr, unsigned long long *stamps,
                                            uint64_t *__restrict__ scan_count, uint32_t *next_unit_p, uint32_t *waves_done_p,
                                            unsigned long long *wg_compared_p, unsigned long long t_start,
-                                           unsigned long long *span, uint32_t n_tiles, uint32_t slice_bits)
+                                           unsigned long long *span, uint32_t n_tiles, uint32_t slice_bits,
+                                           const VerifyCtx &vc, uint32_t *tails_done_p)
 {
     uint32_t &next_unit = *next_unit_p;
     uint32_t &waves_done = *waves_done_p;
@@ -336,6 +385,13 @@
     w.fill = 1;
     w.left = 0;
     w.reserve = 1;
+    const bool tail_launch = TAIL && FINE && (vc.scan_verify > 1u || (vc.scan_verify != 0u && plan->scan_tail != 0u));
+    const bool tail = tail_launch && !no_own_chunk;
+    w.tail = tail ? kTailOn | (vc.scan_verify > 1u ? kTailLast : 0u) : 0u;
+    if (tail && lane == 0) {
+        uint32_t *runs = wave_runs();
+        runs[0] = 1u; runs[1] = wave_id; runs[kRunCursor] = 0u; runs[kRunCursor + 1u] = 0u; runs[kRunCursor + 2u] = 0u;
+    }
     bool own_chunk = false;
     unsigned long long compared = 0ull;
 
@@ -349,10 +405,31 @@
 
     const uint32_t order_step = slice_bits == 8u ? 6u : 0u;
     while (true) {
+        if constexpr (FINE && TAIL) {
+            if ((w.tail & kTailPending) != 0u) {
+                scan_tail(plan->fine, lane, raw, raw_used);
+                w.tail &= ~kTailPending;
+            }
+        }
+        if ((w.tail & kTailRangeDone) != 0u) break;
         uint32_t u = 0;
         if (lane == 0) u = atomicAdd(&next_unit, 1u);
         u = __builtin_amdgcn_readfirstlane(u);
-        if (u >= n_units) break;
+        if (u >= n_units) {
+            if (own_chunk) {
+                raw_retire(w, lane, raw, raw_used);
+                if (no_own_chunk && lane == 0) counters->raw_overflow = 1u;
+            }
+            if (lane == 0) {
+                atomicAdd(&wg_compared, compared);
+                if (atomicAdd(&waves_done, 1u) == (blockDim.x >> 6) - 1u) {
+                    scan_count[blockIdx.x] = atomicAdd(&wg_compared, 0ull);
+                    if (!tail_launch) atomicMax(span + 1, static_cast<unsigned long long>(__builtin_amdgcn_s_memrealtime()));
+                }
+            }
+            w.tail |= kTailRangeDone | ((own_chunk && (w.tail & kTailLast) != 0u) ? kTailPending : 0u);
+            continue;
+        }
         ++units_done;
         const uint32_t gt = tile_begin + u;
         if (fine) { it = gt; cur = items[gt]; }
@@ -520,17 +597,11 @@
             }
         }
     }
-    if (own_chunk) {
-        raw_retire(w, lane, raw, raw_used);
-        if (no_own_chunk && lane == 0) counters->raw_overflow = 1u;
-    }
-    if (lane == 0) {
-        atomicAdd(&wg_compared, compared);
-        if (atomicAdd(&waves_done, 1u) == (blockDim.x >> 6) - 1u) {
-            scan_count[blockIdx.x] = atomicAdd(&wg_compared, 0ull);
-            atomicMax(span + 1, static_cast<unsigned long long>(__builtin_amdgcn_s_memrealtime()));
-        }
-    }
+    if constexpr (FINE && TAIL) {
+        if ((w.tail & kTailOn) != 0u && lane == 0 && wave_runs()[kRunCursor + 2u] != 0u) atomicAdd(&vc.counters->scan_verified, wave_runs()[kRunCursor + 2u]);
+    }
+    if (tail_launch && lane == 0 && atomicAdd(tails_done_p, 1u) == (blockDim.x >> 6) - 1u)
+        atomicMax(span + 1, static_cast<unsigned long long>(__builtin_amdgcn_s_memrealtime()));
     if (stamps && lane == 0) {
         stamps[4 * wave_id] = t_start;
         stamps[4 * wave_id + 1] = __builtin_amdgcn_s_memrealtime();
@@ -540,8 +611,9 @@
     }
 }
 
-template <int THR>
-__global__ __launch_bounds__(1024, 8) void k_scan(const uint32_t *__restrict__ scan_stream,
+template <int THR, bool TAIL>
+__global__ __launch_bounds__(1024, 8) void k_scan(VerifyCtx vc,
+                                                  const uint32_t *__restrict__ scan_stream,
                                                   const ScanItem *__restrict__ items_full,
                                                   const ScanItem *__restrict__ items_fine,
                                                   const PlanInfo *__restrict__ plan,
@@ -554,10 +626,11 @@
 {
     __shared__ uint32_t next_unit;
     __shared__ uint32_t waves_done;
+    __shared__ uint32_t tails_done;
     __shared__ unsigned long long wg_compared;
     __shared__ uint4 tail_masks[16][64];
     const unsigned long long t_start = __builtin_amdgcn_s_memrealtime();
-    if (threadIdx.x == 0) { next_unit = 0; waves_done = 0; wg_compared = 0ull; }
+    if (threadIdx.x == 0) { next_unit = 0; waves_done = 0; wg_compared = 0ull; if (TAIL) tails_done = 0; }
     __syncthreads();
     if (blockIdx.x >= plan->n_ranges) {
         if (threadIdx.x == 0) scan_count[blockIdx.x] = 0ull;
@@ -565,40 +638,46 @@
     }
     if (threadIdx.x == 0) atomicMin(span, t_start);
     if (plan->fine != 0u)
-        scan_range<THR, true>(scan_stream, items_fine, plan, range_start, gword_fine, tail_masks[threadIdx.x >> 6], raw, raw_used, max_chunks, counters, thr, stamps,
-                              scan_count, &next_unit, &waves_done, &wg_compared, t_start, span, n_tiles, slice_bits);
+        scan_range<THR, true, TAIL>(scan_stream, items_fine, plan, range_start, gword_fine, tail_masks[threadIdx.x >> 6], raw, raw_used, max_chunks, counters, thr, stamps,
+                              scan_count, &next_unit, &waves_done, &wg_compared, t_start, span, n_tiles, slice_bits, vc, &tails_done);
     else
-        scan_range<THR, false>(scan_stream, items_full, plan, range_start, gword_full, tail_masks[threadIdx.x >> 6], raw, raw_used, max_chunks, counters, thr, stamps,
-                               scan_count, &next_unit, &waves_done, &wg_compared, t_start, span, n_tiles, slice_bits);
+        scan_range<THR, false, TAIL>(scan_stream, items_full, plan, range_start, gword_full, tail_masks[threadIdx.x >> 6], raw, raw_used, max_chunks, counters, thr, stamps,
+                               scan_count, &next_unit, &waves_done, &wg_compared, t_start, span, n_tiles, slice_bits, vc, &tails_done);
 }
 
 template <int THR>
 static void launch_scan_thr(const ImageView &v, const Workspace &ws, const Tuning &tn, uint32_t thr, uint32_t prune_mode,
-                            hipStream_t stream)
-{
-    hipLaunchKernelGGL(k_scan<THR>, dim3(tn.scan_blocks), dim3(tn.scan_threads), 0, stream, v.scan, ws.items,
-                       prune_mode ? ws.fitems : ws.items, ws.plan, ws.range_start, ws.gword, ws.fword,
-                       ws.raw, ws.raw_used, static_cast<uint32_t>(ws.cap_chunks), ws.counters, thr, ws.stamps, ws.scan_count,
-                       ws.scan_span + 2u * ws.span_slot, v.n_tiles, v.slice_width);
+                            const VerifyCtx &vc, hipStream_t stream)
+{
+    if (vc.scan_verify != 0u)
+        hipLaunchKernelGGL((k_scan<THR, true>), dim3(tn.scan_blocks), dim3(tn.scan_threads), 0, stream, vc, v.scan, ws.items,
+                           prune_mode ? ws.fitems : ws.items, ws.plan, ws.range_start, ws.gword, ws.fword,
+                           ws.raw, ws.raw_used, static_cast<uint32_t>(ws.cap_chunks), ws.counters, thr, ws.stamps, ws.scan_count,
+                           ws.scan_span + 2u * ws.span_slot, v.n_tiles, v.slice_width);
+    else
+        hipLaunchKernelGGL((k_scan<THR, false>), dim3(tn.scan_blocks), dim3(tn.scan_threads), 0, stream, vc, v.scan, ws.items,
+                           prune_mode ? ws.fitems : ws.items, ws.plan, ws.range_start, ws.gword, ws.fword,
+                           ws.raw, ws.raw_used, static_cast<uint32_t>(ws.cap_chunks), ws.counters, thr, ws.stamps, ws.scan_count,
+                           ws.scan_span + 2u * ws.span_slot, v.n_tiles, v.slice_width);
 }
 
 void launch_scan(const ImageView &v, const Workspace &ws, const Tuning &tn, const uint64_t *d_guides, uint32_t n,
-                 int max_dist, uint32_t prune_mode, void *stream_)
-{
-    (void)n;
-    (void)d_guides;
+                 const ScoreParams &p, uint32_t prune_mode, void *stream_)
+{
+    const int max_dist = p.max_dist;
     hipStream_t stream = static_cast<hipStream_t>(stream_);
     if (max_dist < 0) {
         (void)hipMemsetAsync(ws.scan_count, 0, 8ull * tn.scan_blocks, stream);
         return;
     }
     const uint32_t thr = max_dist > 31 ? 31u : static_cast<uint32_t>(max_dist);
-    if (tn.scan_generic || thr > 4) launch_scan_thr<-1>(v, ws, tn, thr, prune_mode, stream);
-    else if (thr == 0) launch_scan_thr<0>(v, ws, tn, thr, prune_mode, stream);
-    else if (thr == 1) launch_scan_thr<1>(v, ws, tn, thr, prune_mode, stream);
-    else if (thr == 2) launch_scan_thr<2>(v, ws, tn, thr, prune_mode, stream);
-    else if (thr == 3) launch_scan_thr<3>(v, ws, tn, thr, prune_mode, stream);
-    else launch_scan_thr<4>(v, ws, tn, thr, prune_mode, stream);
-}
-
-}
+    const VerifyCtx vc = make_verify_ctx(v, ws, tn, d_guides, n, p);
+    if (tn.scan_generic || thr > 4) launch_scan_thr<-1>(v, ws, tn, thr, prune_mode, vc, stream);
+    else if (thr == 0) launch_scan_thr<0>(v, ws, tn, thr, prune_mode, vc, stream);
+    else if (thr == 1) launch_scan_thr<1>(v, ws, tn, thr, prune_mode, vc, stream);
+    else if (thr == 2) launch_scan_thr<2>(v, ws, tn, thr, prune_mode, vc, stream);
+    else if (thr == 3) launch_scan_thr<3>(v, ws, tn, thr, prune_mode, vc, stream);
+    else launch_scan_thr<4>(v, ws, tn, thr, prune_mode, vc, stream);
+}
+
+}
diff --git a/crackling_amd/csrc/issl_kernels.hpp b/crackling_amd/csrc/issl_kernels.hpp
--- a/crackling_amd/csrc/issl_kernels.hpp
+++ b/crackling_amd/csrc/issl_kernels.hpp
@@ -136,7 +136,8 @@
 #define ISSL_CFD_QUAL inline __constant__
 #include "cfd_tables.inc"
 
-__device__ inline double mit_lookup(const ImageView &v, uint64_t mask)
+template <class View>
+__device__ inline double mit_lookup(const View &v, uint64_t mask)
 {
     if (v.mit_dense) {
         if (mask >> 40) return 0.0;
@@ -154,7 +155,8 @@
     return 0.0;
 }
 
-__device__ inline void score_terms(const ImageView &v, uint64_t gsig, uint64_t ot, uint32_t occ, bool calc_mit, bool calc_cfd,
+template <class View>
+__device__ inline void score_terms(const View &v, uint64_t gsig, uint64_t ot, uint32_t occ, bool calc_mit, bool calc_cfd,
                                    double &mit_term, double &cfd_term, int &dist_out)
 {
     mit_term = 0.0;
@@ -248,4 +250,160 @@
     return t;
 }
 
-}
+struct VerifyRec {
+    StreamRec sr;
+    uint64_t gsig;
+    uint32_t guide, bucket, slice, tile, offset;
+};
+
+typedef const __attribute__((address_space(4))) VerifyCtx KernargCtx;
+template <bool SORTED_PRUNED, class Ctx>
+__device__ __forceinline__ VerifyRec verify_fetch(const Ctx &c, uint32_t prune_mode, uint64_t rec, bool in_use)
+{
+    const auto &v = c.v;
+    VerifyRec r;
+    r.sr = StreamRec{};
+    r.gsig = 0;
+    r.guide = kNoGuide; r.bucket = 0; r.slice = 0;
+    r.offset = static_cast<uint32_t>(rec) & (kTileCands - 1u);
+    r.tile = static_cast<uint32_t>(rec >> 11) & 0x3FFFFFFu;
+    const uint32_t gslot = static_cast<uint32_t>(rec >> 37);
+    if (in_use && v.srec) r.sr = v.srec[static_cast<uint64_t>(r.tile) * kTileCands + r.offset];
+    else if (in_use && v.sid) r.sr.id = v.sid[static_cast<uint64_t>(r.tile) * kTileCands + r.offset];
+    if (in_use) {
+        if (SORTED_PRUNED || prune_mode) {
+            const uint64_t low = (1ull << v.slice_width) - 1ull;
+            if (gslot != kPadSlotId) slot_id_unpack(gslot, r.slice, r.guide);
+            if (r.guide >= c.n || r.slice >= v.n_slices) r.guide = kNoGuide;
+            else {
+                r.gsig = c.guides[r.guide];
+                r.bucket = (r.slice << v.slice_width) + (static_cast<uint32_t>(r.gsig >> (v.slice_width * r.slice)) & static_cast<uint32_t>(low));
+            }
+        } else if constexpr (!SORTED_PRUNED) {
+            r.guide = c.gidx[gslot];
+            r.bucket = c.gbucket[gslot];
+            r.slice = r.bucket >> v.slice_width;
+        }
+    }
+    return r;
+}
+
+template <bool SORTED_PRUNED, class Ctx>
+__device__ __forceinline__ void verify_finish(const Ctx &c, uint32_t prune_mode, const VerifyRec &r, bool in_use,
+                                              uint32_t chunk, uint32_t t, uint32_t lane)
+{
+    const auto &v = c.v;
+    const int max_dist = c.max_dist;
+    const bool calc_mit = c.calc_mit != 0u, calc_cfd = c.calc_cfd != 0u;
+    const uint64_t low = (1ull << v.slice_width) - 1ull;
+    const uint32_t guide = r.guide, bucket = r.bucket, slice = r.slice, tile = r.tile, offset = r.offset;
+    uint64_t gsig = r.gsig;
+    uint64_t key = kDeadKey;
+    double mit_term = 0.0, cfd_term = 0.0;
+    uint64_t hit_gsig = 0, hit_ot = 0;
+    uint32_t hit_occ = 0;
+    const bool by_id = SORTED_PRUNED || v.srec || v.sid;
+    if (guide != kNoGuide) {
+        uint64_t start = 0, pos = 0;
+        bool mine = true;
+        if constexpr (!SORTED_PRUNED) if (!by_id) {
+            start = v.bucket_start[bucket];
+            pos = static_cast<uint64_t>(tile - v.tile_first[bucket]) * kTileCands + offset;
+            mine = pos < v.bucket_start[bucket + 1] - start;
+        }
+        if (mine) {
+            if (!(SORTED_PRUNED || prune_mode)) gsig = c.guides[guide];
+            StreamRec sr = r.sr;
+            if (v.sid) sr.sig = v.sites[sr.id];
+            uint64_t ot = sr.sig & kSigMask;
+            if constexpr (!SORTED_PRUNED)
+                if (!by_id) ot = v.esig   ? v.esig[start + pos]
+                                 : v.occ8 ? candidate_signature(v, bucket, tile, offset)
+                                          : v.sites[v.entries[start + pos] & 0xFFFFFFFFull];
+            if (__builtin_popcountll(mismatch_mask(gsig, ot)) <= max_dist) {
+                const uint64_t x = gsig ^ ot;
+                if (!(SORTED_PRUNED || prune_mode)) {
+                    bool earlier = false;
+                    for (uint32_t j = 0; j < slice; ++j)
+                        if (((x >> (v.slice_width * j)) & low) == 0) earlier = true;
+                    if (!earlier) {
+                        const uint64_t lp = by_id ? sr.id : pos;
+                        key = (static_cast<uint64_t>(guide) << kKeyGuideShift) | (static_cast<uint64_t>(slice) << kKeySliceShift) | lp;
+                    }
+                } else {
+                    const uint32_t tol = prune_mode - 1u;
+                    const uint64_t mm = mismatch_mask(gsig, ot);
+                    uint32_t first = slice, reporter = slice;
+                    for (uint32_t j = slice; j-- > 0;) {
+                        if (((x >> (v.slice_width * j)) & low) != 0) continue;
+                        first = j;
+                        if (static_cast<uint32_t>(__builtin_popcount(succ_byte(mm, j, v.slice_width))) <= tol) reporter = j;
+                    }
+                    if (reporter == slice)
+                        key = (static_cast<uint64_t>(guide) << kKeyGuideShift) | (static_cast<uint64_t>(first) << kKeySliceShift) | sr.id;
+                }
+                if (key != kDeadKey) {
+                    uint32_t occ = 0;
+                    if (by_id) {
+                        occ = static_cast<uint32_t>(sr.sig >> 40);
+                        if (occ == kOccSaturated) occ = v.site_occ[sr.id];
+                    } else if constexpr (!SORTED_PRUNED) {
+                        if (v.occ8) {
+                            occ = v.occ8[start + pos];
+                            if (occ == 255u) occ = static_cast<uint32_t>(v.entries[start + pos] >> 32);
+                        } else {
+                            occ = static_cast<uint32_t>(v.entries[start + pos] >> 32);
+                        }
+                    }
+                    hit_gsig = gsig; hit_ot = ot; hit_occ = occ;
+                }
+            }
+        }
+    }
+    const bool live = key != kDeadKey;
+    const uint32_t prev_guide = static_cast<uint32_t>(__shfl_up(static_cast<int>(live ? guide : kNoGuide), 1, 64));
+    const bool continues = live && lane != 0u && prev_guide == guide;
+    const uint64_t starts = __ballot(!continues);
+    uint32_t rank = 0;
+    if (starts == ~0ull) {
+        if (live) rank = atomicAdd(&c.gcount[guide], 1u);
+    } else {
+        const uint64_t upto = (lane == 63u ? 0ull : (~0ull << (lane + 1u)));
+        const uint32_t head = 63u - static_cast<uint32_t>(__builtin_clzll(starts & ~upto));
+        const uint64_t later = starts & upto;
+        const uint32_t next = later ? static_cast<uint32_t>(__builtin_ctzll(later)) : 64u;
+        uint32_t base = 0;
+        if (live && !continues) base = atomicAdd(&c.gcount[guide], next - lane);
+        rank = static_cast<uint32_t>(__shfl(static_cast<int>(base), static_cast<int>(head), 64)) + (lane - head);
+    }
+    if (live && rank == kReplayLds) atomicAdd(&c.counters->overflowed, 1u);
+    if (live && rank < c.slot_hits) {
+        int dist;
+        score_terms(v, hit_gsig, hit_ot, hit_occ, calc_mit, calc_cfd, mit_term, cfd_term, dist);
+        const uint64_t at = static_cast<uint64_t>(guide) * c.slot_hits + rank;
+        SlotRec s;
+        s.mit = mit_term; s.cfd = cfd_term; s.key = key;
+        s.pad = slot_pad(hit_occ, static_cast<uint32_t>(dist));
+        c.slots[at] = s;
+        key = kDeadKey;
+    } else if (live) {
+        const uint64_t slot = static_cast<uint64_t>(chunk) * (kChunkRecs - 1u) + (t - 1u);
+        c.rank[slot] = rank;
+        if (rank < kMidHits) {
+            int dist;
+            score_terms(v, hit_gsig, hit_ot, hit_occ, calc_mit, calc_cfd, mit_term, cfd_term, dist);
+            reinterpret_cast<double2 *>(c.pay)[slot] = make_double2(mit_term, cfd_term);
+        }
+    }
+    if (in_use && !c.lean_tail) c.raw[static_cast<uint64_t>(chunk) * kChunkRecs + t] = key;
+}
+
+template <bool SORTED_PRUNED, class Ctx>
+__device__ __forceinline__ void verify_record(const Ctx &c, uint32_t prune_mode, uint64_t rec, bool in_use, uint32_t chunk,
+                                              uint32_t t, uint32_t lane)
+{
+    const VerifyRec r = verify_fetch<SORTED_PRUNED>(c, prune_mode, rec, in_use);
+    verify_finish<SORTED_PRUNED>(c, prune_mode, r, in_use, chunk, t, lane);
+}
+
+}
diff --git a/crackling_amd/csrc/issl_options.cpp b/crackling_amd/csrc/issl_options.cpp
--- a/crackling_amd/csrc/issl_options.cpp
+++ b/crackling_amd/csrc/issl_options.cpp
@@ -86,6 +86,8 @@
         if (o.put) o.put(t, o.def);
     const char *timing = std::getenv("ISSL_UPLOAD_TIMING");
     t.upload_timing = timing && timing[0] == '1';
+    const char *scan_verify = std::getenv("ISSL_SCAN_VERIFY");
+    t.scan_verify = !scan_verify ? -1 : std::strcmp(scan_verify, "0") == 0 ? 0 : std::strcmp(scan_verify, "1") == 0 ? 1 : -1;
     for (const Option &o : kOptions)
         if (const char *e = std::getenv(o.env)) (void)t.set(o.key, e);
     return t;
diff --git a/crackling_amd/csrc/issl_pipeline.cpp b/crackling_amd/csrc/issl_pipeline.cpp
--- a/crackling_amd/csrc/issl_pipeline.cpp
+++ b/crackling_amd/csrc/issl_pipeline.cpp
@@ -57,6 +57,8 @@
     ix->proven_guides = 0;
     ix->proven_chunks = 0;
     ix->proven_dist = -1;
+    ix->plan_cands_per_guide = 0.0;
+    ix->plan_cands_prune = 0;
     ix->prev_scan_end = nullptr;
     ix->prev_batch_end = nullptr;
 }
@@ -207,6 +209,19 @@
     return ISSL_OK;
 }
 
+static uint32_t tail_worth_arming(const issl_index *ix, size_t n, uint32_t prune_mode)
+{
+    const Tuning &tn = ix->tuning;
+    if (tn.scan_verify == 0 || prune_mode == 0 || !(ix->view.srec || ix->view.sid)) return 0u;
+    if (tn.scan_verify > 0) return 2u;
+    const double want = static_cast<double>(kScanTailCands) * scan_waves(tn);
+    const double slices = static_cast<double>(ix->hdr.n_slices);
+    const double mean_group = static_cast<double>(ix->hdr.n_sites) * slices / (static_cast<double>(ix->hdr.n_buckets) * 256.0);
+    const double even = static_cast<double>(n) * slices * fine_ways_of(prune_mode) * mean_group;
+    const double learnt = ix->plan_cands_prune == prune_mode ? ix->plan_cands_per_guide * static_cast<double>(n) : 0.0;
+    return (2.0 * even >= want || learnt >= want) ? 1u : 0u;
+}
+
 static int enqueue_batch(issl_index *ix, Lane &lane, hipStream_t stream, const uint64_t *d_guides, size_t n, int max_dist,
                          double threshold, int method, double *d_mit, double *d_cfd, bool dump, bool staged,
                          int lanes_mode = 1, issl_profile *d_profile = nullptr)
@@ -237,6 +252,7 @@
     }
     ws.slot_hits = (!dump && tn.hit_slots && ws.cap_slot_guides >= n) ? ws.slot_width : 0u;
     ws.lean_tail = (lane.lean && ws.slot_hits >= kSlotHits && tn.lean_tail) ? 1u : 0u;
+    ws.scan_verify = max_dist < 0 ? 0u : tail_worth_arming(ix, n, prune_mode);
     ScoreParams p;
     p.max_dist = max_dist;
     p.method = method;
@@ -253,7 +269,7 @@
     if (pipelined && ix->prev_scan_end) HIP_TRY(hipStreamWaitEvent(stream, ix->prev_scan_end, 0));
     if (bin_ahead && ix->prev_batch_end) HIP_TRY(hipStreamWaitEvent(stream, ix->prev_batch_end, 0));
     if (scan_pair) HIP_TRY(hipEventRecord(ix->ring[2 * slot], stream));
-    launch_scan(ix->view, ws, tn, d_guides, n32, max_dist, prune_mode, stream);
+    launch_scan(ix->view, ws, tn, d_guides, n32, p, prune_mode, stream);
     if (scan_pair) HIP_TRY(hipEventRecord(ix->ring[2 * slot + 1], stream));
     if (scan_pair) ix->n_ring += 1;
     if (staged) HIP_TRY(hipEventRecord(lane.ev[2], stream));
@@ -263,7 +279,7 @@
         HIP_TRY(hipStreamWaitEvent(tail, ix->ring[2 * slot + 1], 0));
         ix->prev_scan_end = ix->ring[2 * slot + 1];
     }
-    launch_verify(ix->view, ws, d_guides, static_cast<uint32_t>(n), p, tail);
+    launch_verify(ix->view, ws, tn, d_guides, static_cast<uint32_t>(n), p, tail);
     if (staged) HIP_TRY(hipEventRecord(lane.ev[3], tail));
     launch_group_hits(ws, n32, tail);
     if (staged) HIP_TRY(hipEventRecord(lane.ev[4], tail));
@@ -332,9 +348,10 @@
             if (rc) return rc;
             lp->ws.cap_fitems = want;
         }
+        Counters c{};
+        HIP_TRY(hipMemcpy(&c, lp->ws.counters, sizeof c, hipMemcpyDeviceToHost));
+        lp->scan_verified = c.scan_verified;
         if (lp->ws.slots && lp->ws.slot_width == kSlotHits && ix->tuning.hit_slots && lp->last_n) {
-            Counters c{};
-            HIP_TRY(hipMemcpy(&c, lp->ws.counters, sizeof c, hipMemcpyDeviceToHost));
             const size_t want = lp->ws.cap_slot_guides * size_t(kSlotHitsWide) * sizeof(SlotRec);
             size_t free_b = 0, total_b = 0;
             if (c.overflowed > lp->last_n / 8 && want <= kSlotBytesMax && hipMemGetInfo(&free_b, &total_b) == hipSuccess &&
@@ -368,6 +385,10 @@
     PlanInfo pl{};
     uint32_t total_hits = 0;
     HIP_TRY(hipMemcpy(&pl, lane.ws.plan, sizeof pl, hipMemcpyDeviceToHost));
+    if (pl.fine != 0u && lane.last_n != 0u && lane.last_max_dist >= 0) {
+        ix->plan_cands_per_guide = static_cast<double>(pl.candidates) / lane.last_n;
+        ix->plan_cands_prune = pl.fine;
+    }
     {
         std::vector<uint32_t> counts(lane.last_n);
         if (lane.last_n) HIP_TRY(hipMemcpy(counts.data(), lane.ws.gcount, 4 * counts.size(), hipMemcpyDeviceToHost));
diff --git a/crackling_amd/csrc/issl_verify.hip b/crackling_amd/csrc/issl_verify.hip
--- a/crackling_amd/csrc/issl_verify.hip
+++ b/crackling_amd/csrc/issl_verify.hip
@@ -6,158 +6,68 @@
 
 namespace issl {
 
-__global__ __launch_bounds__(kChunkRecs, 8) void k_verify(ImageView v, Workspace ws, const uint64_t *__restrict__ guides,
-                                                       uint32_t n, ScoreParams p)
+template <bool MARKS>
+__global__ __launch_bounds__(kChunkRecs, 8) void k_verify(VerifyCtx c, const PlanInfo *__restrict__ plan, uint32_t *sticky, uint32_t cap_chunks)
 {
     short_kernel_priority();
-    const int max_dist = p.max_dist;
-    const bool calc_mit = p.method == ISSL_METHOD_MIT || p.method == ISSL_METHOD_AND || p.method == ISSL_METHOD_OR ||
-                          p.method == ISSL_METHOD_AVG;
-    const bool calc_cfd = p.method == ISSL_METHOD_CFD || p.method == ISSL_METHOD_AND || p.method == ISSL_METHOD_OR ||
-                          p.method == ISSL_METHOD_AVG;
-    const uint32_t prune_mode = ws.plan->fine;
-    uint32_t n_chunks = ws.counters->raw_chunks;
+    const uint32_t prune_mode = plan->fine;
+    uint32_t n_chunks = c.counters->raw_chunks;
+    const bool none_marked = !MARKS || c.counters->scan_verified == 0u;
     if (blockIdx.x == 0 && threadIdx.x == 0) {
-        if (ws.counters->raw_overflow) atomicOr(&ws.sticky[0], 1u);
-        atomicMax(&ws.sticky[1], n_chunks);
-        if (ws.plan->error) atomicOr(&ws.sticky[2], ws.plan->error);
+        if (c.counters->raw_overflow) atomicOr(&sticky[0], 1u);
+        atomicMax(&sticky[1], n_chunks);
+        if (plan->error) atomicOr(&sticky[2], plan->error);
     }
-    if (n_chunks > ws.cap_chunks) n_chunks = static_cast<uint32_t>(ws.cap_chunks);
-    const uint64_t low = (1ull << v.slice_width) - 1ull;
+    if (n_chunks > cap_chunks) n_chunks = cap_chunks;
     for (uint32_t chunk = blockIdx.x; chunk < n_chunks; chunk += gridDim.x) {
-        uint64_t *recs = ws.raw + static_cast<uint64_t>(chunk) * kChunkRecs;
+        const uint64_t *recs = c.raw + static_cast<uint64_t>(chunk) * kChunkRecs;
         const uint32_t t = threadIdx.x + 1u;
-        const uint64_t rec_any = recs[t < kChunkRecs ? t : 0u];
-        const uint32_t used = ws.raw_used[chunk];
+        uint64_t rec_any = 0ull;
+        if (none_marked) rec_any = recs[t < kChunkRecs ? t : 0u];
+        const uint32_t used = c.raw_used[chunk];
+        if (MARKS && (used & kChunkVerified)) continue;
         const bool in_use = t < used && t < kChunkRecs;
-        const uint64_t rec = in_use ? rec_any : 0ull;
-        uint64_t key = kDeadKey;
-        double mit_term = 0.0, cfd_term = 0.0;
-        uint64_t hit_gsig = 0, hit_ot = 0;
-        uint32_t hit_occ = 0;
-        const uint32_t offset = static_cast<uint32_t>(rec) & (kTileCands - 1u);
-        const uint32_t tile = static_cast<uint32_t>(rec >> 11) & 0x3FFFFFFu;
-        const uint32_t gslot = static_cast<uint32_t>(rec >> 37);
-        const bool by_id = v.srec || v.sid;
-        StreamRec sr_early{};
-        if (in_use && v.srec) sr_early = v.srec[static_cast<uint64_t>(tile) * kTileCands + offset];
-        else if (in_use && v.sid) sr_early.id = v.sid[static_cast<uint64_t>(tile) * kTileCands + offset];
-        uint32_t guide = kNoGuide, bucket = 0, slice = 0;
-        uint64_t gsig = 0;
-        if (in_use) {
-            if (prune_mode) {
-                if (gslot != kPadSlotId) slot_id_unpack(gslot, slice, guide);
-                if (guide >= n || slice >= v.n_slices) guide = kNoGuide;
-                else {
-                    gsig = guides[guide];
-                    bucket = (slice << v.slice_width) + (static_cast<uint32_t>(gsig >> (v.slice_width * slice)) & static_cast<uint32_t>(low));
-                }
-            } else {
-                guide = ws.gidx[gslot];
-                bucket = ws.gbucket[gslot];
-                slice = bucket >> v.slice_width;
-            }
-        }
-        if (guide != kNoGuide) {
-            uint64_t start = 0, pos = 0;
-            bool mine = true;
-            if (!by_id) {
-                start = v.bucket_start[bucket];
-                pos = static_cast<uint64_t>(tile - v.tile_first[bucket]) * kTileCands + offset;
-                mine = pos < v.bucket_start[bucket + 1] - start;
-            }
-            if (mine) {
-                if (!prune_mode) gsig = guides[guide];
-                StreamRec sr = sr_early;
-                if (v.sid) sr.sig = v.sites[sr.id];
-                const uint64_t ot = by_id    ? sr.sig & kSigMask
-                                    : v.esig ? v.esig[start + pos]
-                                    : v.occ8 ? candidate_signature(v, bucket, tile, offset)
-                                             : v.sites[v.entries[start + pos] & 0xFFFFFFFFull];
-                if (__builtin_popcountll(mismatch_mask(gsig, ot)) <= max_dist) {
-                    const uint64_t x = gsig ^ ot;
-                    if (!prune_mode) {
-                        bool earlier = false;
-                        for (uint32_t j = 0; j < slice; ++j)
-                            if (((x >> (v.slice_width * j)) & low) == 0) earlier = true;
-                        if (!earlier) {
-                            const uint64_t lp = by_id ? sr.id : pos;
-                            key = (static_cast<uint64_t>(guide) << kKeyGuideShift) | (static_cast<uint64_t>(slice) << kKeySliceShift) | lp;
-                        }
-                    } else {
-                        const uint32_t tol = prune_mode - 1u;
-                        const uint64_t mm = mismatch_mask(gsig, ot);
-                        uint32_t first = slice, reporter = slice;
-                        for (uint32_t j = slice; j-- > 0;) {
-                            if (((x >> (v.slice_width * j)) & low) != 0) continue;
-                            first = j;
-                            if (static_cast<uint32_t>(__builtin_popcount(succ_byte(mm, j, v.slice_width))) <= tol) reporter = j;
-                        }
-                        if (reporter == slice)
-                            key = (static_cast<uint64_t>(guide) << kKeyGuideShift) | (static_cast<uint64_t>(first) << kKeySliceShift) | sr.id;
-                    }
-                    if (key != kDeadKey) {
-                        uint32_t occ;
-                        if (by_id) {
-                            occ = static_cast<uint32_t>(sr.sig >> 40);
-                            if (occ == kOccSaturated) occ = v.site_occ[sr.id];
-                        } else if (v.occ8) {
-                            occ = v.occ8[start + pos];
-                            if (occ == 255u) occ = static_cast<uint32_t>(v.entries[start + pos] >> 32);
-                        } else {
-                            occ = static_cast<uint32_t>(v.entries[start + pos] >> 32);
-                        }
-                        hit_gsig = gsig; hit_ot = ot; hit_occ = occ;
-                    }
-                }
-            }
-        }
-        const bool live = key != kDeadKey;
-        const uint32_t lane = threadIdx.x & 63u;
-        const uint32_t prev_guide = static_cast<uint32_t>(__shfl_up(static_cast<int>(live ? guide : kNoGuide), 1, 64));
-        const bool continues = live && lane != 0u && prev_guide == guide;
-        const uint64_t starts = __ballot(!continues);
-        uint32_t rank = 0;
-        if (starts == ~0ull) {
-            if (live) rank = atomicAdd(&ws.gcount[guide], 1u);
-        } else {
-            const uint64_t upto = (lane == 63u ? 0ull : (~0ull << (lane + 1u)));
-            const uint32_t head = 63u - static_cast<uint32_t>(__builtin_clzll(starts & ~upto));
-            const uint64_t later = starts & upto;
-            const uint32_t next = later ? static_cast<uint32_t>(__builtin_ctzll(later)) : 64u;
-            uint32_t base = 0;
-            if (live && !continues) base = atomicAdd(&ws.gcount[guide], next - lane);
-            rank = static_cast<uint32_t>(__shfl(static_cast<int>(base), static_cast<int>(head), 64)) + (lane - head);
-        }
-        if (live && rank == kReplayLds) atomicAdd(&ws.counters->overflowed, 1u);
-        if (live && rank < ws.slot_hits) {
-            int dist;
-            score_terms(v, hit_gsig, hit_ot, hit_occ, calc_mit, calc_cfd, mit_term, cfd_term, dist);
-            const uint64_t at = static_cast<uint64_t>(guide) * ws.slot_hits + rank;
-            SlotRec r;
-            r.mit = mit_term; r.cfd = cfd_term; r.key = key;
-            r.pad = slot_pad(hit_occ, static_cast<uint32_t>(dist));
-            ws.slots[at] = r;
-            key = kDeadKey;
-        } else if (live) {
-            const uint64_t slot = static_cast<uint64_t>(chunk) * (kChunkRecs - 1u) + (t - 1u);
-            ws.rank[slot] = rank;
-            if (rank < kMidHits) {
-                int dist;
-                score_terms(v, hit_gsig, hit_ot, hit_occ, calc_mit, calc_cfd, mit_term, cfd_term, dist);
-                reinterpret_cast<double2 *>(ws.pay)[slot] = make_double2(mit_term, cfd_term);
-            }
-        }
-        if (!in_use) continue;
-        if (!ws.lean_tail) recs[t] = key;
+        const uint64_t rec = !in_use ? 0ull : none_marked ? rec_any : recs[t];
+        verify_record<false>(c, prune_mode, rec, in_use, chunk, t, threadIdx.x & 63u);
     }
 }
 
-void launch_verify(const ImageView &v, const Workspace &ws, const uint64_t *d_guides, uint32_t n, const ScoreParams &p, void *stream)
+VerifyCtx make_verify_ctx(const ImageView &v, const Workspace &ws, const Tuning &tn, const uint64_t *d_guides, uint32_t n, const ScoreParams &p)
+{
+    VerifyCtx c;
+    c.v = v;
+    c.guides = d_guides;
+    c.raw = ws.raw;
+    c.raw_used = ws.raw_used;
+    c.gidx = ws.gidx;
+    c.gbucket = ws.gbucket;
+    c.gcount = ws.gcount;
+    c.slots = ws.slots;
+    c.rank = ws.rank;
+    c.pay = ws.pay;
+    c.counters = ws.counters;
+    c.n = n;
+    c.slot_hits = ws.slot_hits;
+    c.lean_tail = ws.lean_tail;
+    c.max_dist = p.max_dist;
+    c.calc_mit = (p.method == ISSL_METHOD_MIT || p.method == ISSL_METHOD_AND || p.method == ISSL_METHOD_OR || p.method == ISSL_METHOD_AVG) ? 1u : 0u;
+    c.calc_cfd = (p.method == ISSL_METHOD_CFD || p.method == ISSL_METHOD_AND || p.method == ISSL_METHOD_OR || p.method == ISSL_METHOD_AVG) ? 1u : 0u;
+    (void)tn;
+    c.scan_verify = (v.srec || v.sid) ? ws.scan_verify : 0u;
+    return c;
+}
+
+void launch_verify(const ImageView &v, const Workspace &ws, const Tuning &tn, const uint64_t *d_guides, uint32_t n, const ScoreParams &p, void *stream)
 {
     if (p.max_dist < 0) return;
     const uint32_t grid = n < 256u ? std::max<uint32_t>(2048u, 64u * n) : kTailGrid;
-    hipLaunchKernelGGL(k_verify, dim3(std::min(grid, kTailGrid)), dim3(kChunkRecs), 0, static_cast<hipStream_t>(stream), v, ws, d_guides, n, p);
+    const VerifyCtx c = make_verify_ctx(v, ws, tn, d_guides, n, p);
+    if (c.scan_verify != 0u)
+        hipLaunchKernelGGL(k_verify<true>, dim3(std::min(grid, kTailGrid)), dim3(kChunkRecs), 0, static_cast<hipStream_t>(stream), c, ws.plan, ws.sticky,
+                           static_cast<uint32_t>(ws.cap_chunks));
+    else
+        hipLaunchKernelGGL(k_verify<false>, dim3(std::min(grid, kTailGrid)), dim3(kChunkRecs), 0, static_cast<hipStream_t>(stream), c, ws.plan, ws.sticky,
+                           static_cast<uint32_t>(ws.cap_chunks));
 }
 
 }
```

Measured after the change: 52.11 million (median of 6 runs). 1.07x the previous value.
